# abiswas-odu/Disco

Hardware: AMD Instinct MI355X
Metric: overlaps/sec (BuildGraph stage), 150 bp reads (higher is better)
Workload: dtype u64; 1 GPU; 50000000 x 150 bp synthetic reads, 30x of 50 x 5000000 bp uniform-random contigs, both strands, error-free, min-overlap 40 (k=39), transitive reduction on, seed 42; reads=50000000, read_len=150, min_overlap=40, parallelism=1 GPU, e_pre=903537181, e_out=45314794, n_contained=4685156, cap_bind_sites=0, asymmetric_pairs=0, probes=5550000000, kmer_hits=2220071992

## Files before the change

### disco_amd/buildgraph.py

```python
from __future__ import annotations

import ctypes as C
import os

import numpy as np

_HERE = os.path.dirname(os.path.abspath(__file__))
_LIBPATH = os.environ.get("DISCO_LIB") or os.path.join(_HERE, "libdisco_hip.so")
_lib = None


class DiscoError(RuntimeError):
    pass


class Params(C.Structure):
    _fields_ = [("min_overlap", C.c_uint32), ("max_edges_per_kmer", C.c_uint32), ("flags", C.c_uint32), ("max_substitutions", C.c_uint32)]


class GenSpecABI(C.Structure):
    _fields_ = [("seed", C.c_uint64), ("n_reads", C.c_uint64), ("contig_len", C.c_uint64), ("n_contigs", C.c_uint32),
                ("len_min", C.c_uint32), ("len_max", C.c_uint32), ("skew", C.c_uint32)]


# ... 78 lines not shown
    ("disco_ingest_fasta", C.c_int, [_P, C.POINTER(C.c_char_p), C.c_int, C.c_uint32, _P, _P]),
    ("disco_ingest_fetch", C.c_int, [_P, _P, _P]),
    ("disco_inflate_bgzf", C.c_int64, [_P, _P, C.c_uint64, _P, C.c_uint64]),
    ("disco_dist_ingest_fasta", C.c_int, [_P, C.POINTER(C.c_char_p), C.c_int, C.c_uint32, _P, _P]),
    ("disco_dist_ingest_fetch", C.c_int, [_P, _P, _P]),
    ("disco_inflate_bgzf_window", C.c_int64, [_P, _P, C.c_uint64, C.c_uint64, C.c_uint64, _P]),
    ("disco_format_contained", C.c_int64, [_P, C.c_uint32, _P, _P]),
    ("disco_fetch_contained_text", C.c_int, [_P, _P, C.c_uint64]),
    ("disco_write_contained_text", C.c_int, [_P, _P, C.c_uint32, C.c_uint32]),
    ("disco_dist_format_contained", C.c_int64, [_P, C.c_uint32, _P, _P]),
    ("disco_dist_format_edges", C.c_int64, [_P, C.c_uint32, _P, _P]),
    ("disco_fetch_chain_residue", C.c_int64, [_P, _P, _P, C.c_uint64]),
    ("disco_fetch_chain_first_edges", C.c_int, [_P, _P]),
    ("disco_fetch_chain_end_links", C.c_int, [_P, _P, _P]),
    ("disco_format_par_simple", C.c_int64, [_P, C.c_uint32, _P, _P, C.c_uint64, _P, C.c_uint64, _P]),
    ("disco_fetch_par_simple_text", C.c_int, [_P, _P, C.c_uint64]),
    ("disco_write_par_simple_text", C.c_int, [_P, _P, C.c_uint32, C.c_uint32]),
    ("disco_prepare_edge_records", C.c_int64, [_P, C.c_uint32, _P, _P]),
    ("disco_fetch_edge_records", C.c_int, [_P, _P, C.c_uint64]),
    ("disco_write_edge_records", C.c_int, [_P, C.c_int, C.c_uint64, C.c_uint32]),
    ("disco_prepare_contained_records", C.c_int64, [_P, C.c_uint32, _P]),
    ("disco_fetch_contained_records", C.c_int, [_P, _P, C.c_uint64]),
    ("disco_write_contained_records", C.c_int, [_P, C.c_int, C.c_uint64, C.c_uint32]),
]

ABI_VERSION = 2
FLAG_TWO_PASS_VERIFY = 1
FLAG_SEEDED_KMER = 2
XCHG = ("reads", "index_records", "index_shards", "contain", "row_requests", "row_data", "push", "adjacency", "twins", "queries", "hits", "keys", "reads_dealt", "contain_keys")
UNIQUE_ID_BYTES = 128
DIST_GATHER_READS = 1
DIST_KEEP_INDEX_PARTITIONED = 2


CHAIN_EDGE_DTYPE = np.dtype([("a", "<u8"), ("b", "<u8"), ("offset", "<u8"), ("orient", "<u4"), ("n_links", "<u4"), ("first_link", "<u8")])
CHAIN_LINK_DTYPE = np.dtype([("to", "<u4"), ("offset", "<u4"), ("orient", "<u4")])


class PsEdge(C.Structure):
    _fields_ = [("src", C.c_uint64), ("dst", C.c_uint64), ("offset", C.c_uint64), ("orient", C.c_uint32), ("file", C.c_uint32),
                ("first_piece", C.c_uint64), ("n_pieces", C.c_uint32), ("pad", C.c_uint32)]


class PsPiece(C.Structure):
    _fields_ = [("kind", C.c_uint32), ("a", C.c_uint32), ("offset", C.c_uint32), ("orient", C.c_uint32)]


PS_EDGE_DTYPE = np.dtype([("src", "<u8"), ("dst", "<u8"), ("offset", "<u8"), ("orient", "<u4"), ("file", "<u4"), ("first_piece", "<u8"), ("n_pieces", "<u4"), ("pad", "<u4")])
PS_PIECE_DTYPE = np.dtype([("kind", "<u4"), ("a", "<u4"), ("offset", "<u4"), ("orient", "<u4")])
assert PS_EDGE_DTYPE.itemsize == C.sizeof(PsEdge) and PS_PIECE_DTYPE.itemsize == C.sizeof(PsPiece)


class IngestFile(C.Structure):
    _fields_ = [("first_index", C.c_uint64), ("last_index", C.c_uint64), ("good", C.c_uint64), ("bad", C.c_uint64)]


class IngestInfo(C.Structure):
    _fields_ = [("n_reads", C.c_uint64), ("total_records", C.c_uint64), ("too_long", C.c_uint64), ("stride_words", C.c_uint32), ("shortest", C.c_uint32),
                ("longest", C.c_uint32), ("read_s", C.c_float), ("device_s", C.c_float)]


class DistIngestInfo(C.Structure):
    _fields_ = [("n_reads", C.c_uint64), ("total_records", C.c_uint64), ("too_long", C.c_uint64), ("stride_words", C.c_uint32), ("shortest", C.c_uint32),
                ("longest", C.c_uint32), ("world", C.c_uint32), ("share_lo", C.c_uint64), ("share_hi", C.c_uint64), ("share_reads", C.c_uint64),
                ("kept_reads", C.c_uint64), ("home_lo", C.c_uint64), ("home_hi", C.c_uint64), ("read_s", C.c_float), ("device_s", C.c_float)]


class DistInfo(C.Structure):
    _fields_ = [("world", C.c_uint32), ("rank", C.c_uint32), ("n_reads", C.c_uint64), ("own_lo", C.c_uint64), ("own_hi", C.c_uint64),
                ("n_contained", C.c_uint64), ("e_pre", C.c_uint64), ("e_out", C.c_uint64), ("e_out_local", C.c_uint64),
                ("n_contained_local", C.c_uint64), ("cap_bind_sites", C.c_uint64), ("asymmetric_pairs", C.c_uint64),
                ("dropped_hits", C.c_uint64), ("probes", C.c_uint64), ("kmer_hits", C.c_uint64), ("regime", C.c_uint32),
                ("tr_rounds", C.c_uint32), ("tr_deferred", C.c_uint64), ("bytes_sent", C.c_uint64 * len(XCHG)),
                ("ms", C.c_float * len(XCHG)), ("ms_total", C.c_float), ("kernel_ms", C.c_float), ("comm_ops", C.c_uint32),
                ("host_syncs", C.c_uint32), ("device_allocs", C.c_uint32), ("device_frees", C.c_uint32), ("arena_bytes", C.c_uint64),
                ("arena_peak", C.c_uint64), ("hbm_peak", C.c_uint64), ("own_reads", C.c_uint64), ("placement", C.c_uint32), ("reserved_", C.c_uint32)]

PHASES = ("index", "probe_kernel", "verify", "contain", "select", "csr", "twin", "trmark", "emit", "order")

INSPECT_ABI = [
    ("disco_fetch_order", C.c_int, [_P, _P, _P, C.c_uint64, C.POINTER(C.c_uint64), C.POINTER(C.c_int)]),
    ("disco_fetch_survivor_layout", C.c_int, [_P, _P, C.c_uint64, C.POINTER(C.c_uint64), C.POINTER(C.c_int), C.POINTER(C.c_uint64)]),
    ("disco_set_record_piece", C.c_int, [_P, C.c_uint64]),
]
_inspect_bound = False


def _bind_inspect(L):
    global _inspect_bound
    if not _inspect_bound:
        for name, res, args in INSPECT_ABI:
            fn = getattr(L, name)
            fn.restype = res
            fn.argtypes = args
        _inspect_bound = True


def lib_path() -> str:
    return _LIBPATH


def load():
    global _lib
    if _lib is None:
        if not os.path.exists(_LIBPATH):
            raise DiscoError(f"{_LIBPATH} is missing: build it with `python -m disco_amd.build` (hipcc, gfx950). "
                             "There is no CPU fallback.")
        L = C.CDLL(_LIBPATH)
        L.disco_abi_version.restype = C.c_int
        if L.disco_abi_version() != ABI_VERSION:
            raise DiscoError(f"{_LIBPATH} speaks ABI version {L.disco_abi_version()}, this mirror was written against {ABI_VERSION}: rebuild "
                             "(`python -m disco_amd.build`)")
        for name, res, args in ABI:
            fn = getattr(L, name)
            fn.restype = res
            fn.argtypes = args
        _lib = L
    return _lib


class BuildGraph:

    def __init__(self, min_overlap: int = 40, device: int = 0, max_edges_per_kmer: int = 4, flags: int = 0, max_substitutions: int = 0):
        self.L = load()
        self.min_overlap = min_overlap
        self._h = _P()
        p = Params(min_overlap, max_edges_per_kmer, flags, max_substitutions)
        rc = self.L.disco_create(device, C.byref(p), C.byref(self._h))
        if rc != 0:
            raise DiscoError(f"disco_create failed ({rc}): {self.L.disco_last_error(None).decode()}")

    def _chk(self, rc):
        if rc < 0:
            raise DiscoError(f"libdisco_hip error {rc}: {self.L.disco_last_error(self._h).decode()}")
        return rc

    def close(self):
        if self._h:
            self.L.disco_destroy(self._h)
            self._h = _P()

    def __del__(self):
        try:
            self.close()
        except Exception:
            pass

    def __enter__(self):
        return self

    def __exit__(self, *a):
        self.close()

    def set_stream(self, stream_ptr: int | None):
        self._chk(self.L.disco_set_stream(self._h, _P(stream_ptr) if stream_ptr else None))

    def synchronize(self):
        self._chk(self.L.disco_synchronize(self._h))

    def upload_reads(self, packed: np.ndarray, lens: np.ndarray):
        packed = np.ascontiguousarray(packed, dtype=np.uint64)
        lens = np.ascontiguousarray(lens, dtype=np.uint16)
        assert packed.ndim == 2 and packed.shape[0] == lens.shape[0]
        self._keep = (packed, lens)
        self._chk(self.L.disco_upload_reads(self._h, packed.ctypes.data, packed.shape[1], lens.ctypes.data, packed.shape[0]))

# ... 238 lines not shown
        from .edgefile import EDGE

        out = np.zeros(n, dtype=EDGE)
        self._chk(self.L.disco_fetch_edge_records(self._h, out.ctypes.data if n else None, n))
        return out

    def write_edge_records(self, fd: int, file_offset: int = 32, threads: int = 8):
        self._chk(self.L.disco_write_edge_records(self._h, fd, file_offset, threads))

    def prepare_contained_records(self, n_files: int = 1, file_index=None) -> int:
        fi = None if file_index is None else np.ascontiguousarray(file_index, dtype=np.uint64)
        return self._chk(self.L.disco_prepare_contained_records(self._h, n_files, None if fi is None else fi.ctypes.data))

    def fetch_contained_records(self, n: int) -> np.ndarray:
        from .edgefile import CONTAINED

        out = np.zeros(n, dtype=CONTAINED)
        self._chk(self.L.disco_fetch_contained_records(self._h, out.ctypes.data if n else None, n))
        return out

    def write_contained_records(self, fd: int, file_offset: int = 32, threads: int = 8):
        self._chk(self.L.disco_write_contained_records(self._h, fd, file_offset, threads))

    def set_record_piece(self, records: int = 0):
        _bind_inspect(self.L)
        self._chk(self.L.disco_set_record_piece(self._h, records))

    def fetch_edge_substitutions(self) -> np.ndarray:
        n = self._chk(self.L.disco_fetch_edge_substitutions(self._h, None, 0))
        out = np.zeros(n, dtype=np.uint16)
        if n:
            self._chk(self.L.disco_fetch_edge_substitutions(self._h, out.ctypes.data, n))
        return out

    def phase_ms(self) -> dict:
        a = (C.c_float * len(PHASES))()
        self._chk(self.L.disco_phase_ms(self._h, a, len(PHASES)))
        return {n: float(a[i]) for i, n in enumerate(PHASES)}

    def fetch_edge_files(self, n_files: int):
        n = int(self.L.disco_fetch_edges(self._h, None, 0))
        out = np.zeros(max(n, 1), dtype=np.uint16)
        self._chk(self.L.disco_fetch_edge_files(self._h, n_files, out.ctypes.data, n))
        return out[:n]

    def partition_edges(self, edges: np.ndarray, n_nodes: int, n_files: int):
        edges = np.ascontiguousarray(edges, dtype=EDGE_DTYPE)
        out = np.zeros(max(len(edges), 1), dtype=np.uint16)
        self._chk(self.L.disco_partition_edges(self._h, edges.ctypes.data, len(edges), n_nodes, n_files, out.ctypes.data))
        return out[:len(edges)]

    def get_query_order(self) -> int:
        out = _P()
        self._chk(self.L.disco_get_query_order(self._h, C.byref(out)))
        return out.value or 0

    def set_query_order(self, d_order_ptr: int):
        self._chk(self.L.disco_set_query_order(self._h, _P(d_order_ptr)))

    def probe_run_words(self) -> int:
        return int(self.L.disco_probe_run_words(self._h))

    def fetch_order(self):
        _bind_inspect(self.L)
        n, bits = C.c_uint64(0), C.c_int(0)
        one = np.zeros(1, dtype=np.uint64)
        rc = self.L.disco_fetch_order(self._h, one.ctypes.data, one.ctypes.data, 0, C.byref(n), C.byref(bits))
        if n.value == 0:
            self._chk(rc)
        order, keys = np.zeros(max(n.value, 1), dtype=np.uint64), np.zeros(max(n.value, 1), dtype=np.uint32)
        self._chk(self.L.disco_fetch_order(self._h, order.ctypes.data, keys.ctypes.data, len(order), C.byref(n), C.byref(bits)))
        return order[:n.value], keys[:n.value], bits.value

    def fetch_survivor_layout(self, lengths: bool = True):
        _bind_inspect(self.L)
        n, dense, used = C.c_uint64(0), C.c_int(0), C.c_uint64(0)
        self._chk(self.L.disco_fetch_survivor_layout(self._h, None, 0, C.byref(n), C.byref(dense), C.byref(used)))
        lens = None
        if lengths:
            lens = np.zeros(max(n.value, 1), dtype=np.uint8)
            self._chk(self.L.disco_fetch_survivor_layout(self._h, lens.ctypes.data, len(lens), C.byref(n), C.byref(dense), C.byref(used)))
            lens = lens[:n.value]
        return lens, bool(dense.value), used.value

    def measure_hbm(self, nbytes: int = 4 << 30, reps: int = 5) -> float:
        out = C.c_double(0.0)
        self._chk(self.L.disco_measure_hbm(self._h, nbytes, reps, C.byref(out)))
        return out.value

    def measure_gather(self, nbytes: int = 3 << 30, reps: int = 3) -> float:
        out = C.c_double(0.0)
        self._chk(self.L.disco_measure_gather(self._h, nbytes, reps, C.byref(out)))
        return out.value

    def memcpy_d2d(self, dst_ptr: int, src_ptr: int, nbytes: int):
        self._chk(self.L.disco_memcpy_d2d(self._h, _P(dst_ptr), _P(src_ptr), nbytes))

    @staticmethod
    def comm_unique_id() -> bytes:
        buf = C.create_string_buffer(UNIQUE_ID_BYTES)
        rc = load().disco_comm_unique_id(buf, UNIQUE_ID_BYTES)
        if rc != 0:
            raise DiscoError(f"disco_comm_unique_id failed ({rc})")
        return buf.raw

    def comm_init(self, unique_id: bytes, world: int, rank: int):
        self._chk(self.L.disco_comm_init(self._h, C.c_char_p(unique_id), world, rank))

    @staticmethod
    def comm_init_local(graphs):
        arr = (_P * len(graphs))(*[g._h for g in graphs])
        rc = load().disco_comm_init_local(arr, len(graphs))
        if rc != 0:
            raise DiscoError(f"disco_comm_init_local failed ({rc})")

    @property
    def rank(self) -> int:
        return int(self.L.disco_comm_rank(self._h))

    @property
    def world(self) -> int:
        return int(self.L.disco_comm_world(self._h))

    @property
    def transport(self) -> str:
        return self.L.disco_comm_kind(self._h).decode()

    def dist_range(self, n_total: int):
        lo, hi = C.c_uint64(), C.c_uint64()
        self._chk(self.L.disco_dist_range(self._h, n_total, C.byref(lo), C.byref(hi)))
        return lo.value, hi.value

    def dist_upload_reads(self, packed_own: np.ndarray, lens_own: np.ndarray, n_total: int, stride_words: int | None = None):
        packed_own = np.ascontiguousarray(packed_own, dtype=np.uint64)
        lens_own = np.ascontiguousarray(lens_own, dtype=np.uint16)
        self._keep = (packed_own, lens_own)
        stride = int(stride_words if stride_words is not None else packed_own.shape[1])
        self._chk(self.L.disco_dist_upload_reads(self._h, packed_own.ctypes.data, stride, lens_own.ctypes.data, n_total))

    def dist_upload_ascii(self, reads):
        n = len(reads)
        lo, hi = self.dist_range(n)
        stride = int((max((len(r) for r in reads), default=1) + 31) // 32)
        packed = np.zeros((hi - lo, stride), dtype=np.uint64)
        lens = np.fromiter((len(r) for r in reads[lo:hi]), dtype=np.uint16, count=hi - lo)
        for i, r in enumerate(reads[lo:hi]):
            b = r.encode()
            if self.L.disco_pack_ascii(b, len(b), packed[i].ctypes.data) != 0:
                raise DiscoError(f"read {lo + i} contains a non-ACGT base")
        self.dist_upload_reads(packed, lens, n, stride)

    def dist_generate_reads(self, spec):
        s = GenSpecABI(spec.seed, spec.n_reads, spec.contig_len, spec.n_contigs, spec.len_min, spec.len_max, int(spec.skew_word if hasattr(spec, "skew_word") else getattr(spec, "skew", 0)))
        self._chk(self.L.disco_dist_generate_reads(self._h, C.byref(s)))

    def ingest_fasta(self, paths, threads: int = 16):
        arr = (C.c_char_p * len(paths))(*[os.fsencode(p) for p in paths])
        info, files = IngestInfo(), (IngestFile * len(paths))()
        rc = self.L.disco_ingest_fasta(self._h, arr, len(paths), threads, C.byref(info), files)
        if rc == -6:
            return None
        self._chk(rc)
        return ({n: getattr(info, n) for n, _ in IngestInfo._fields_}, [{n: getattr(f, n) for n, _ in IngestFile._fields_} for f in files])

    def inflate_bgzf(self, data: bytes):
        data = bytes(data)
# ... 110 lines not shown
```

### disco_amd/csrc/disco_hip.hip

```cpp
#include <hip/hip_runtime.h>
#include <rocprofiler-sdk-roctx/roctx.h>

#include <algorithm>
#include <atomic>
#include <chrono>
#include <cstdarg>
#include <cstdio>
#include <cstdlib>
#include <cstring>
#include <functional>
#include <fcntl.h>
#include <sys/mman.h>
#include <sys/stat.h>
#include <unistd.h>
#include <string>
#include <memory>
#include <thread>
#include <map>
#include <mutex>
#include <queue>
#include <vector>

#include "../../include/disco_hip.h"
#include "../../include/disco_hip_test.h"
// ... 79 lines not shown
                used += bytes;
                peak = std::max(peak, used);
                return base + off;
            }
        return nullptr;
    }
    void release(void *p)
    {
        const size_t off = (size_t)((char *)p - base);
        auto lv = live.find(off);
        if (lv == live.end()) return;
        size_t start = off, end = off + lv->second;
        used -= lv->second;
        live.erase(lv);
        auto nx = free_at.lower_bound(off);
        if (nx != free_at.end() && nx->first == end) {
            end += nx->second;
            nx = free_at.erase(nx);
        }
        if (nx != free_at.begin()) {
            auto pv = std::prev(nx);
            if (pv->first + pv->second == start) {
                start = pv->first;
                free_at.erase(pv);
            }
        }
        free_at[start] = end - start;
    }
    std::map<size_t, size_t> live;
};

template <typename T>
struct DevBuf {
    T *p = nullptr;
    u64 cap = 0;
    operator T *() const { return p; }
};

struct disco_ctx {
    int device = 0;
    disco_params prm{};
    DevArena arena;
    int k = 0;
    int ks = 0;
    hipStream_t own_stream = nullptr;
    hipStream_t stream = nullptr;
    int n_cu = 256;
    std::string err;
    size_t hbm_bytes = 0, hbm_peak = 0;

    u64 n = 0;
    int S = 0;
    u64 *d_reads = nullptr;
    u16 *d_len = nullptr;
    DevBuf<u64> reads_own;
    DevBuf<u16> len_own;
    bool reads_owned = false;
    std::vector<uint16_t> h_len;
    bool h_len_ok = false;
    std::mutex h_len_mu;
    u64 q_lo = 0, q_hi = 0;
    bool two_class = false;
    bool dist_two_class = false;
    u64 job_n_long = 0;
    u32 job_short_max = 0;
    int S_ext = 0;
    u64 n_long = 0;
    DevBuf<u64> d_full;
    DevBuf<u32> d_ovf, d_long_ids;
    u32 max_len_all = 0;
    int tailb = 0;
    DevBuf<u32> d_lpos, d_n_list;
    DevBuf<uint2> d_linfo;
    DevBuf<ulonglong2> d_lmeta;

    u64 T = 0;
    int bshift = 0;
    DevBuf<u32> d_bkt;
    DevBuf<u64> d_ent;
    DevBuf<ulonglong2> d_rec;
    bool binned_index = false;
    DevBuf<ulonglong2> d_rec2;
    DevBuf<u32> d_binx;

    DevBuf<u64> d_tile;
    u64 *d_total = nullptr;

    u64 *d_ctr = nullptr;
    u64 *d_wq = nullptr;
    u64 h_ctr[CTR_COUNT] = {0};

    DevBuf<u64> d_best;
    DevBuf<u64> d_hits;
    u64 hits_used = 0;
    u64 *d_bump = nullptr;
    DevBuf<u64> d_row_start;
    DevBuf<u32> d_row_cnt;
    DevBuf<u64> d_big_list;
    DevBuf<u32> d_big_cnt;
    u32 *d_n_big = nullptr;
    DevBuf<u32> d_runs;
    u64 runs_lo = 0, runs_n = 0;
    int runs_lpr = 0;
    DevBuf<u64> d_slow_list;
    u32 *d_n_slow = nullptr;
    u64 big_rows = 0, slow_rows = 0;
    const u64 *d_order = nullptr;
    const u64 *d_order_used = nullptr;
    bool order_external = false;
    DevBuf<u32> d_ocnt, d_okey, d_oslot;
    DevBuf<u64> d_order_own;
    bool order_counted = false;
    bool order_items = false;
    int order_id_bits = 0;
    bool es_big_counted = false, tr_big_counted = false;
    bool contained_count_pending = false;
    bool order_ready = false;
    hipStream_t aux_stream = nullptr;
    hipEvent_t ev_crows = nullptr;
    DevBuf<u32> d_cpos, d_crow_id;
    DevBuf<u64> d_crow_key;
    DevBuf<u64> d_tile2;
    u64 *d_total2 = nullptr;
    void *h_crows = nullptr;
    DevBuf<u32> d_crow_len;
    u64 crows_hcap = 0, crows_n = 0;
    bool crows_pending = false;
    bool crows_in_ring = false;
    DevBuf<u32> d_cgrp_cur, d_cgrp_id;
    DevBuf<u64> d_cgrp_key, d_cgrp_big;
    u64 h_cgrp_big = 0;
    bool cgrp_pending = false;
    DevBuf<u32> d_fetch_src;
    DevBuf<u64> d_fetch_ent;
    DevBuf<u32> d_rec_of_read;
    std::vector<u64> ingest_id_base, ingest_rec_base;
    u64 ingest_n = 0;
    void *h_ring = nullptr;
    std::vector<u64> text_off;
    DevBuf<char> d_ctext;
    std::vector<u64> ctext_off;
    u64 ctext_bytes = 0;
    DevBuf<u8> d_ingest;
    std::thread hits_prealloc;
    DevBuf<u64> prealloc;
    u64 prealloc_asked = 0;
    size_t ring_half = 0;
    hipEvent_t ev_ring[2] = {nullptr, nullptr};
    hipStream_t copy_stream = nullptr;
    hipEvent_t ev_copied[3] = {nullptr, nullptr, nullptr}, ev_unpacked[3] = {nullptr, nullptr, nullptr};
    bool index_counted = false;
    u64 order_counted_lo = 0, order_counted_hi = 0;
    int order_counted_bits = 0;
    DevBuf<u32> d_asked;
    u64 order_q_lo = 0, order_q_hi = 0;
    DevBuf<ulonglong2> d_meta_ord;
    u64 dropped_local = 0;
    ProbeRare h_probe_rare;
    DevBuf<ProbeRare> d_probe_rare;
    u32 max_len = 0, min_len = 0;
    bool two_pass_last = false;
    bool contained_done = false;

    DevBuf<u8> d_contained;
    DevBuf<u64> d_cbits;
    DevBuf<u64> d_dropbits;
    DevBuf<u64> d_drop_node, d_drop_key;
    u64 n_drop_items = 0;
    u64 drop_lo = 0, drop_hi = 0;
    u64 n_contained = 0;

    DevBuf<u64> d_adj_ref;
// ... 267 lines not shown
    v.long_ids = c->two_class ? c->d_long_ids : nullptr;
    v.n_long = c->two_class ? (u32)c->n_long : 0u;
    v.SL = c->two_class ? c->S_ext : 0;
    v.tailb = c->two_class ? c->tailb : 0;
    return v;
}

static OwnSet own_set(const disco_ctx *c)
{
    OwnSet o;
    o.otab = c->loci ? c->d_otab : nullptr;
    o.me = c->comm ? (u32)c->comm->rank : 0u;
    o.lo = c->q_lo;
    o.hi = c->q_hi;
    o.list = c->loci ? c->d_order_own : nullptr;
    o.n_own = c->loci ? c->n_own : 0;
    o.ids = c->loci ? c->d_own_ids : nullptr;
    return o;
}

static int settle_keys(disco_ctx *c)
{
    if (c->keys_pending) {
        c->keys_pending = false;
        HIPCHK(c, hipStreamWaitEvent(c->stream, c->ev_keys, 0));
    }
    return DISCO_OK;
}

static int env_int(const char *name, int dflt)
{
    const char *e = getenv(name);
    return e ? atoi(e) : dflt;
}

static int wave_grid(const disco_ctx *c, u64 items, int per_cu = 24)
{
    u64 g = (u64)c->n_cu * per_cu;
    if (items < g) g = items;
    return (int)std::max<u64>(g, 1);
}

template <typename K>
static int wq_grid(disco_ctx *c, K kernel, u64 items, const char *env, int cap = 32)
{
    (void)hipMemsetAsync(c->d_wq, 0, sizeof(u64) * WQ_WORDS, c->stream);
    int per_cu = 0;
    if (hipOccupancyMaxActiveBlocksPerMultiprocessor(&per_cu, kernel, 64, 0) != hipSuccess || per_cu <= 0) per_cu = 16;
    if (per_cu > cap) per_cu = cap;
    per_cu = env_int(env, per_cu);
    u64 g = (u64)c->n_cu * per_cu;
    const u64 chunks = (items + WQ_CHUNK - 1) / WQ_CHUNK;
    if (chunks < g) g = chunks;
    return (int)std::max<u64>(g, 1);
}

template <typename K, typename... A>
static void wq_launch(disco_ctx *c, K kernel, u64 items, const char *env, int cap, A... args)
{
    const int g = wq_grid(c, kernel, items, env, cap);
    hipLaunchKernelGGL(kernel, dim3(g), dim3(64), 0, c->stream, args...);
}

static int flat_grid(const disco_ctx *c, u64 items, int block = 256)
{
    u64 g = (items + block - 1) / block;
    u64 cap = (u64)c->n_cu * 16;
    return (int)std::max<u64>(std::min(g, cap), 1);
}

static int read_counters(disco_ctx *c)
{
    HIPCHK(c, hipMemcpyAsync(c->h_ctr, c->d_ctr, sizeof(c->h_ctr), hipMemcpyDeviceToHost, c->stream));
    HIPCHK(c, hipStreamSynchronize(c->stream));
    return DISCO_OK;
}

static int zero_counter(disco_ctx *c, int idx)
{
    HIPCHK(c, hipMemsetAsync(c->d_ctr + idx, 0, sizeof(u64), c->stream));
    return DISCO_OK;
}

template <typename InT, typename OutT>
static int scan_exclusive_on(disco_ctx *c, hipStream_t st, DevBuf<u64> &tile, u64 *total, const InT *in, u64 n, OutT *out, bool write_total, u64 *total_host)
{
    u64 nt = (n + SCAN_TILE - 1) / SCAN_TILE;
    if (nt == 0) nt = 1;
    CHK(ensure(c, tile, nt));
    hipLaunchKernelGGL((scan_tile_sums_kernel<InT>), dim3((unsigned)nt), dim3(SCAN_BLOCK), 0, st, in, n, tile.p);
    hipLaunchKernelGGL(scan_sums_kernel, dim3(1), dim3(1024), 0, st, tile.p, nt, total);
    hipLaunchKernelGGL((scan_apply_kernel<InT, OutT>), dim3((unsigned)nt), dim3(SCAN_BLOCK), 0, st, in, n, tile.p, out);
    if (write_total) hipLaunchKernelGGL((scan_write_total_kernel<OutT>), dim3(1), dim3(1), 0, st, total, out + n);
    HIPCHK(c, hipGetLastError());
    if (total_host) {
        HIPCHK(c, hipMemcpyAsync(total_host, total, sizeof(u64), hipMemcpyDeviceToHost, st));
        HIPCHK(c, hipStreamSynchronize(st));
    }
    return DISCO_OK;
}

template <typename InT, typename OutT>
static int scan_exclusive(disco_ctx *c, const InT *in, u64 n, OutT *out, bool write_total, u64 *total_host)
{
    return scan_exclusive_on<InT, OutT>(c, c->stream, c->d_tile, c->d_total, in, n, out, write_total, total_host);
}

static void drop_edge_records(disco_ctx *c)
{
    c->rec_e_ready = false;
    release(c, c->d_rec_efile);
    release(c, c->d_rec_subs);
    release(c, c->d_rec_efindex);
}
static void drop_contained_records(disco_ctx *c)
{
    c->rec_c_ready = false;
    c->rec_c_n = 0;
    release(c, c->d_rec_cword);
    release(c, c->d_rec_csup);
    release(c, c->d_rec_cfindex);
}

static void free_graph_state(disco_ctx *c)
{
    drop_edge_records(c);
    drop_contained_records(c);
    release(c, c->d_rec_piece[0]);
    release(c, c->d_rec_piece[1]);
    if (c->keys_pending) {
        c->keys_pending = false;
        if (c->ev_keys) (void)hipEventSynchronize(c->ev_keys);
    }
    release(c, c->d_bkt);
    release(c, c->d_ent);
    release(c, c->d_rec);
    release(c, c->d_rec2);
    release(c, c->d_binx);
    release(c, c->d_best);
    release(c, c->d_hits);
    release(c, c->d_row_start);
    release(c, c->d_row_cnt);
    release(c, c->d_big_list);
    release(c, c->d_big_cnt);
    release(c, c->d_slow_list);
    release(c, c->d_runs);
    c->runs_n = 0;
    c->runs_lpr = 0;
    release(c, c->d_contained);
    release(c, c->d_cbits);
    release(c, c->d_dropbits);
    release(c, c->d_drop_node);
    release(c, c->d_drop_key);
    release(c, c->d_adj_ref);
    release(c, c->d_adj_own);
    release(c, c->d_adj_spare);
    release(c, c->d_start_tmp);
    release(c, c->d_ocnt);
    release(c, c->d_okey);
    release(c, c->d_meta_ord);
    release(c, c->d_asked);
    release(c, c->d_oslot);
    release(c, c->d_order_own);
    c->d_order_used = nullptr;
    c->d_adj = nullptr;
    release(c, c->d_extra_cnt);
    release(c, c->d_extra_node);
    release(c, c->d_extra_key);
    release(c, c->d_half);
    release(c, c->d_hcnt);
    release(c, c->d_wide);
    release(c, c->d_n_wide);
    c->adj_total = 0;
    release(c, c->d_out_valid);
    release(c, c->d_ch_comp);
    release(c, c->d_ch_links);
    release(c, c->d_ch_dead);
    release(c, c->d_ch_first);
    release(c, c->d_ch_res_pos);
    release(c, c->d_ch_res_slot);
    c->ch_res_n = 0;
    release(c, c->d_ptext);
    c->ptext_bytes = 0;
    c->ptext_off.clear();
    release(c, c->d_text);
    c->text_bytes = 0;
    release(c, c->d_ctext);
    c->ctext_bytes = 0;
    c->ctext_off.clear();
    c->ch_ready = false;
    release(c, c->d_out_pos);
    release(c, c->d_out_src);
    release(c, c->d_out_ent);
    c->n_out = c->out_used = 0;
    c->flags_pending = false;
    c->adj_imported = false;
    c->T = 0;
    release(c, c->d_x16a);
    release(c, c->d_x16b);
    release(c, c->d_req_flat);
    release(c, c->d_req_s);
    release(c, c->d_req_r);
    release(c, c->d_rdeg_s);
    release(c, c->d_rdeg_r);
    release(c, c->d_rdata_s);
    release(c, c->d_rpos);
    release(c, c->d_nadj32_own);
    release(c, c->d_deg_tmp);
    release(c, c->d_dense);
    release(c, c->d_pq_start);
    c->nadj_used = 0;
    c->d_push_r = nullptr;
    c->n_push_r = 0;
    release(c, c->d_cb_all);
    release(c, c->d_otab);
    release(c, c->d_own_ids);
    c->n_own = 0;
    c->loci = c->runs_by_pos = false;
}

static void free_long_class(disco_ctx *c)
{
    release(c, c->d_full);
    release(c, c->d_ovf);
    release(c, c->d_long_ids);
    release(c, c->d_lpos);
    release(c, c->d_lmeta);
    release(c, c->d_linfo);
    release(c, c->d_n_list);
    c->two_class = false;
    c->n_long = 0;
    c->S_ext = 0;
    c->tailb = 0;
}

static void free_reads(disco_ctx *c)
{
    release(c, c->reads_own);
    release(c, c->len_own);
    free_long_class(c);
    c->d_reads = nullptr;
    c->d_len = nullptr;
    c->reads_owned = false;
    c->h_len.clear();
    c->n = 0;
}

static int alloc_reads(disco_ctx *c, u64 words, u64 n_len)
{
    CHK(ensure(c, c->reads_own, words));
    c->d_reads = c->reads_own;
    CHK(ensure(c, c->len_own, n_len));
    c->d_len = c->len_own;
    return DISCO_OK;
}

static u32 extra_cap(const disco_ctx *c) { return (u32)std::min<u64>(std::min(c->d_extra_node.cap, c->d_extra_key.cap), 0xFFFFFFFFull); }

static int grow_big_lists(disco_ctx *c, u64 need) { return ensure_group(c, need, need, c->d_big_list, c->d_big_cnt); }

static bool own_order_wanted(const disco_ctx *c, u64 nq, int *bits)
{
    const u64 order_min = getenv("DISCO_ORDER_MIN_READS") ? (u64)atoll(getenv("DISCO_ORDER_MIN_READS")) : 4096;
    int b = 16;
    while (b < 27 && (1ull << b) < nq) ++b;
    if (const char *e = getenv("DISCO_ORDER_BITS")) b = std::min(std::max(atoi(e), 16), 26);
    *bits = b;
    return !c->order_external && !getenv("DISCO_NO_ORDER") && nq >= order_min && nq > 0;
}

struct IndexCountPlan {
    u64 lo = 0, hi = 0;
    int lpr = 0, nf = 0;
    u32 *ocnt = nullptr, *oslot = nullptr;
    u64 *oitem = nullptr;
    u32 oidbits = 0;
    u32 oshift = 0;
    const u64 *list = nullptr;
};

static bool runs_nf_built(int nf, int m) { return (nf == 7 || nf == 12 || nf == 17 || nf == 22 || nf == 27) && m == RUNS_M; }

static int runs_lpr_for(const disco_ctx *c, int nf, u32 max_len, u64 nloc)
{
    int lpr = 0;
    const int m = view(c).m;
    const bool nf_built = runs_nf_built(nf, m);
    const bool nf_generic = nf >= 2 && nf <= 64 && m > 16 && m <= 31 && !getenv("DISCO_NO_GENERIC_RUNS");
    if ((nf_built || nf_generic) && max_len > (u32)c->ks && !getenv("DISCO_NO_RUNS")) {
        const u32 maxwin = max_len - (u32)c->ks;
        const u32 expect = 2u * maxwin / (u32)(nf + 1);
        lpr = maxwin <= 256 ? (maxwin <= 128 && expect <= 20 ? 16 : (expect <= 44 ? 32 : 0)) : 0;
        const double max_gb = getenv("DISCO_RUNS_MAX_GB") ? atof(getenv("DISCO_RUNS_MAX_GB")) : 16.0;
        if ((double)nloc * lpr * 4.0 > max_gb * 1e9) lpr = 0;
    }
    return lpr;
}

static bool two_class_ok(const disco_ctx *c, int S, u64 n, u64 n_long, u32 short_max, bool will_own = false)
{
    if (((c->comm || c->dist_reads) && !c->dist_two_class) || !(c->reads_owned || will_own) || c->prm.max_substitutions || getenv("DISCO_NO_TWO_CLASS")) return false;
    if (S <= VERIFY_SW || n_long == 0 || n_long * (u64)env_int("DISCO_TWO_CLASS_ONE_IN", 5) > n || n + n_long >= (1ull << 31)) return false;
    return runs_lpr_for(c, c->ks - view(c).m + 1, short_max, n) != 0;
}

static int two_class_alloc(disco_ctx *c, u64 n_long, int Sx, u32 short_max)
{
    c->n_long = n_long;
    c->S_ext = Sx;
    int rc = ensure(c, c->d_ovf, c->n_alloc);
    if (rc == DISCO_OK) rc = ensure(c, c->d_full, n_long * (u64)Sx);
    if (rc == DISCO_OK) rc = ensure(c, c->d_long_ids, n_long);
    if (rc == DISCO_OK) rc = ensure(c, c->d_lpos, n_long);
    if (rc == DISCO_OK) rc = ensure(c, c->d_lmeta, n_long);
    if (rc == DISCO_OK) rc = ensure(c, c->d_linfo, n_long);
    if (rc == DISCO_OK) rc = ensure(c, c->d_n_list, 1);
    if (rc != DISCO_OK) {
        free_long_class(c);
        return rc;
    }
    c->S = VERIFY_SW;
    c->tailb = short_max <= 160 ? 160 : 256;
    c->two_class = true;
    if (getenv("DISCO_VERBOSE"))
        fprintf(stderr, "[disco] two classes of rows: %llu of %llu reads are longer than 256 bases, the others up to %u: 64-byte rows + %d-word rows for those\n",
                (unsigned long long)n_long, (unsigned long long)c->n, short_max, Sx);
    return DISCO_OK;
}

static bool binned_order_wanted(disco_ctx *c, u64 n, int obits, int *id_bits)
{
    if (getenv("DISCO_NO_BINNED_ORDER") || getenv("DISCO_NO_ORDERED_FILL") || c->two_class || n != c->n || n >= 0xFFFF0000ull) return false;
    const u64 binned_min = getenv("DISCO_BINNED_ORDER_MIN_READS") ? (u64)atoll(getenv("DISCO_BINNED_ORDER_MIN_READS")) : (1ull << 21);
    if (n < binned_min) return false;
    int idb = 1, lenb = 1;
    while ((1ull << idb) < n) ++idb;
    while ((1u << lenb) <= c->max_len) ++lenb;
    if (obits + lenb + idb > 64) return false;
    if (ensure(c, c->d_rec2, n) != DISCO_OK) {
        (void)hipGetLastError();
        c->err.clear();
        return false;
    }
    *id_bits = idb;
    return true;
}

static int index_count_plan(disco_ctx *c, const DiscoView &v, u64 lo, u64 hi, IndexCountPlan *pl, const u64 *list = nullptr)
{
    const u64 nloc = hi - lo;
    *pl = IndexCountPlan();
    pl->lo = lo;
    pl->hi = hi;
    pl->list = list;
    if (!list) c->order_counted = c->order_ready = c->order_items = false;
    int obits = 0;
    if (!list && lo == c->q_lo && hi == c->q_hi && own_order_wanted(c, nloc, &obits) && !getenv("DISCO_NO_ORDER_FUSE")) {
        const u64 order_buckets = 1ull << obits;
        if (lo == 0 && binned_order_wanted(c, nloc, obits, &c->order_id_bits)) {
            pl->oitem = (u64 *)c->d_rec2.p;
            pl->oidbits = (u32)c->order_id_bits;
            c->order_items = true;
        } else {
            CHK(ensure(c, c->d_ocnt, order_buckets + 1));
            CHK(ensure(c, c->d_oslot, nloc));
            HIPCHK(c, hipMemsetAsync(c->d_ocnt, 0, (order_buckets + 1) * sizeof(u32), c->stream));
            pl->ocnt = c->d_ocnt;
            pl->oslot = c->d_oslot;
        }
        pl->oshift = 32u - (u32)obits;
        c->order_counted = true;
        c->order_counted_lo = lo;
        c->order_counted_hi = hi;
        c->order_counted_bits = obits;
    }
    c->runs_lpr = 0;
    c->runs_n = 0;
    c->runs_by_pos = false;
    const int nf = v.ks - v.m + 1;
    const int lpr = c->S == VERIFY_SW ? runs_lpr_for(c, nf, c->max_len, nloc) : 0;
    if (lpr && nloc) {
        CHK(ensure(c, c->d_runs, nloc * (u64)lpr));
        c->runs_lpr = lpr;
        c->runs_lo = lo;
        c->runs_n = nloc;
        c->runs_by_pos = list != nullptr;
        pl->lpr = lpr;
        pl->nf = nf;
    }
    return DISCO_OK;
}

typedef void (*IndexRunsFn)(DiscoView, u32 *, ulonglong2 *, u32 *, u64, u64, u32 *, u32 *, u32 *, u64 *, u32, u32, const u64 *);
typedef void (*IndexCountFn)(DiscoView, u32 *, ulonglong2 *, u32 *, u64, u64, u32 *, u32 *, u64 *, u32, u32, const u64 *);
struct IndexCountKernel {
    IndexRunsFn runs = nullptr;
    IndexCountFn plain = nullptr;
};
template <bool COUNT, int NF, int NFMAX, bool LONGK>
static IndexCountKernel index_runs_pick(int lpr)
{
    IndexCountKernel k;
    k.runs = lpr == 16 ? index_runs_kernel<COUNT, NF, 1, NFMAX, LONGK> : index_runs_kernel<COUNT, NF, 2, NFMAX, LONGK>;
    return k;
}
template <bool COUNT>
static IndexCountKernel index_count_pick(int nf, int m, int lpr, bool longk, bool long_class)
{
    if (long_class || !lpr) {
        IndexCountKernel k;
        if (long_class) k.plain = longk ? index_count_kernel<COUNT, true, true> : index_count_kernel<COUNT, false, true>;
        else k.plain = longk ? index_count_kernel<COUNT, true> : index_count_kernel<COUNT>;
        return k;
    }
    if (runs_nf_built(nf, m)) switch (nf) {
        case 7: return index_runs_pick<COUNT, 7, 7, false>(lpr);
        case 12: return index_runs_pick<COUNT, 12, 12, false>(lpr);
        case 17: return index_runs_pick<COUNT, 17, 17, false>(lpr);
        case 22: return index_runs_pick<COUNT, 22, 22, false>(lpr);
        default: return index_runs_pick<COUNT, 27, 27, false>(lpr);
        }
    if (longk) return nf <= 48 ? index_runs_pick<COUNT, 0, 48, true>(lpr) : index_runs_pick<COUNT, 0, 64, true>(lpr);
    if (nf <= 8) return index_runs_pick<COUNT, 0, 8, false>(lpr);
    if (nf <= 12) return index_runs_pick<COUNT, 0, 12, false>(lpr);
    if (nf <= 16) return index_runs_pick<COUNT, 0, 16, false>(lpr);
    if (nf <= 24) return index_runs_pick<COUNT, 0, 24, false>(lpr);
    if (nf <= 32) return index_runs_pick<COUNT, 0, 32, false>(lpr);
    if (nf <= 48) return index_runs_pick<COUNT, 0, 48, false>(lpr);
    return index_runs_pick<COUNT, 0, 64, false>(lpr);
}
static IndexCountKernel index_count_pick(bool count, int nf, int m, int lpr, bool longk, bool long_class)
{
    return count ? index_count_pick<true>(nf, m, lpr, longk, long_class) : index_count_pick<false>(nf, m, lpr, longk, long_class);
}

static int index_count_chunk(disco_ctx *c, const DiscoView &v, const IndexCountPlan &pl, bool count, ulonglong2 *rec_base, u64 a, u64 b)
{
    if (b <= a) return DISCO_OK;
    const dim3 grid((unsigned)((b - a + 255) / 256));
    ulonglong2 *rec = rec_base + 2 * (a - pl.lo);
    u32 *oslot = pl.oslot ? pl.oslot + (a - pl.lo) : nullptr;
    u64 *oitem = pl.oitem ? pl.oitem + (a - pl.lo) : nullptr;
    u32 *okey = pl.list ? nullptr : c->d_okey.p;
    const IndexCountKernel k = index_count_pick(count, pl.nf, v.m, pl.lpr, c->ks > 64, false);
    if (k.runs) hipLaunchKernelGGL(k.runs, grid, dim3(256), 0, c->stream, v, c->d_bkt, rec, okey, a, b, c->d_runs + (a - pl.lo) * (u64)pl.lpr, pl.ocnt, oslot, oitem, pl.oidbits, pl.oshift, pl.list);
    else hipLaunchKernelGGL(k.plain, grid, dim3(256), 0, c->stream, v, c->d_bkt, rec, okey, a, b, pl.ocnt, oslot, oitem, pl.oidbits, pl.oshift, pl.list);
    HIPCHK(c, hipGetLastError());
    return DISCO_OK;
}

static int index_count_long(disco_ctx *c, const DiscoView &v, const IndexCountPlan &pl, bool count, ulonglong2 *rec, u32 *oslot, u64 x_lo, u64 x_hi)
{
    const dim3 g((unsigned)((x_hi - x_lo + 255) / 256));
    hipLaunchKernelGGL(index_count_pick(count, 0, v.m, 0, c->ks > 64, true).plain, g, dim3(256), 0, c->stream, v, c->d_bkt, rec, c->d_okey, x_lo, x_hi, pl.ocnt, oslot, (u64 *)nullptr, 0u, pl.oshift,
                       (const u64 *)nullptr);
    HIPCHK(c, hipGetLastError());
    return DISCO_OK;
}

static bool binned_index_wanted(disco_ctx *c, int logT)
{
    if (getenv("DISCO_NO_BINNED_INDEX") || 2 * c->n >= 0xFFFF0000ull) return false;
    if (logT > BINX_SPAN_BITS && ensure(c, c->d_rec2, 2 * c->n) != DISCO_OK) {
        (void)hipGetLastError();
        c->err.clear();
        return false;
    }
    return true;
}

static int size_bucket_table(disco_ctx *c)
{
    u64 T = 1024;
    int logT = 10;
    double tscale = 2.0;
    if (const char *e = getenv("DISCO_BUCKET_SCALE")) tscale = atof(e);
    while ((double)T < tscale * (double)c->n && logT < 32) {
        T <<= 1;
        logT++;
    }
    c->T = T;
    c->bshift = 64 - logT;
    return logT;
}

static int index_begin(disco_ctx *c)
{
    const int logT = size_bucket_table(c);
    const u64 T = c->T;
    CHK(ensure(c, c->d_bkt, T + 1));
    CHK(ensure(c, c->d_ent, 2 * c->n));
    CHK(ensure(c, c->d_rec, 2 * c->n));
    CHK(ensure(c, c->d_okey, c->n));
    c->adj_imported = false;
    c->binned_index = binned_index_wanted(c, logT);
    if (!c->binned_index) HIPCHK(c, hipMemsetAsync(c->d_bkt, 0, (T + 1) * sizeof(u32), c->stream));
    return DISCO_OK;
}

struct BinxPlan {
    int span = 0, levels = 0, bits[3] = {0, 0, 0};
};
static BinxPlan binx_plan(int logT)
{
    BinxPlan b;
    b.span = std::min(logT, BINX_SPAN_BITS);
    const int prefix = logT - b.span;
    b.levels = (prefix + BINX_MAX_BITS - 1) / BINX_MAX_BITS;
    for (int l = 0; l < b.levels; l++) b.bits[l] = prefix / b.levels + (l < prefix % b.levels ? 1 : 0);
    return b;
}

template <typename R>
static int binx_partition(disco_ctx *c, const char *what, int bits, u32 kshift, u32 total, R *src, R *dst, const R **out, const u32 **part)
{
    const BinxPlan bp = binx_plan(bits);
    const u32 n_part = 1u << (bits - bp.span);
    const u32 tiles = (total + BINX_TILE - 1u) / BINX_TILE;
    u64 hist_len = 1;
    for (int l = 0, done = 0; l < bp.levels; done += bp.bits[l], l++) hist_len = std::max<u64>(hist_len, ((u64)tiles + (1ull << done)) * (1ull << bp.bits[l]) + 1);
    const u64 tab = ((u64)n_part + 1 + 63) & ~63ull;
    CHK(ensure(c, c->d_binx, 4 * tab + hist_len));
    u32 *seg[2] = {c->d_binx.p, c->d_binx.p + tab}, *tb[2] = {c->d_binx.p + 2 * tab, c->d_binx.p + 3 * tab}, *hist = c->d_binx.p + 4 * tab;
    if (getenv("DISCO_VERBOSE"))
        fprintf(stderr, "[disco] binned %s: 2^%d buckets, %u partitions of 2^%d, %d level(s) of %d / %d / %d bits\n", what, bits, n_part, bp.span, bp.levels, bp.bits[0], bp.bits[1], bp.bits[2]);
    u32 pseg = 1, pnb = 1;
    int cur = 0, done = 0;
    for (int l = 0; l < bp.levels; l++) {
        const u32 nseg = 1u << done, nb = 1u << bp.bits[l], shift = kshift + (u32)(bits - done - bp.bits[l]);
        const u32 grid = tiles + nseg;
        const u64 hlen = (u64)grid * nb + 1;
        hipLaunchKernelGGL(binx_segs_kernel, dim3(1), dim3(1024), 0, c->stream, l ? (const u32 *)hist : (const u32 *)nullptr, (const u32 *)tb[cur ^ 1], pseg, pnb, total, seg[cur], tb[cur]);
        HIPCHK(c, hipMemsetAsync(hist, 0, hlen * sizeof(u32), c->stream));
        hipLaunchKernelGGL(binx_hist_kernel<R>, dim3(grid), dim3(BINX_BLOCK), 0, c->stream, (const R *)src, (const u32 *)seg[cur], (const u32 *)tb[cur], nseg, shift, nb, hist);
        CHK((scan_exclusive<u32, u32>(c, hist, hlen, hist, false, nullptr)));
        hipLaunchKernelGGL(binx_scatter_kernel<R>, dim3(grid), dim3(BINX_BLOCK), 0, c->stream, (const R *)src, dst, (const u32 *)seg[cur], (const u32 *)tb[cur], nseg, shift, nb, (const u32 *)hist);
        HIPCHK(c, hipGetLastError());
        std::swap(src, dst);
        pseg = nseg;
        pnb = nb;
        done += bp.bits[l];
        cur ^= 1;
    }
    hipLaunchKernelGGL(binx_segs_kernel, dim3(1), dim3(1024), 0, c->stream, bp.levels ? (const u32 *)hist : (const u32 *)nullptr, (const u32 *)tb[cur ^ 1], pseg, pnb, total, seg[cur],
                       (u32 *)nullptr);
    HIPCHK(c, hipGetLastError());
    *out = src;
    *part = seg[cur];
    return DISCO_OK;
}

static int binned_build_index(disco_ctx *c)
{
    const int logT = 64 - c->bshift;
    const u32 total = (u32)(2 * c->n);
    const ulonglong2 *rec;
    const u32 *part;
    CHK(binx_partition(c, "index build", logT, 32u, total, c->d_rec.p, c->d_rec2.p, &rec, &part));
    const int span = std::min(logT, BINX_SPAN_BITS);
    hipLaunchKernelGGL(binx_build_kernel<ulonglong2>, dim3(1u << (logT - span)), dim3(BINX_BUILD_BLOCK), 0, c->stream, rec, part, (u32)span, 32u, 0u, total, c->T, c->d_bkt.p, c->d_ent.p);
    HIPCHK(c, hipGetLastError());
    return DISCO_OK;
}

static int binned_build_order(disco_ctx *c)
{
    const int bits = c->order_counted_bits;
    const u32 total = (u32)c->n, kshift = 64u - (u32)bits;
    u64 *items = (u64 *)c->d_rec2.p;
    const u64 *rec;
    const u32 *part;
    CHK(binx_partition(c, "grouping", bits, kshift, total, items, items + c->n, &rec, &part));
    const int span = std::min(bits, BINX_SPAN_BITS);
    hipLaunchKernelGGL(binx_build_kernel<u64>, dim3(1u << (bits - span)), dim3(BINX_BUILD_BLOCK), 0, c->stream, rec, part, (u32)span, kshift, (u32)c->order_id_bits, total, (u64)0,
                       (u32 *)nullptr, c->d_order_own.p);
    HIPCHK(c, hipGetLastError());
    return DISCO_OK;
}

static int start_contained_rows(disco_ctx *c, bool grouped)
{
    const u64 nc = c->n_contained;
    if (c->crows_pending && c->crows_n == nc && (!grouped || c->cgrp_pending)) return DISCO_OK;
    const bool have_rows = c->crows_pending && c->crows_n == nc;
    if (!have_rows) c->crows_pending = c->cgrp_pending = false;
    const u64 max_rows = getenv("DISCO_EAGER_ROWS_MAX") ? (u64)atoll(getenv("DISCO_EAGER_ROWS_MAX")) : (16ull << 20);
    if (c->comm || nc == 0 || nc > max_rows || c->n >= (1ull << 31)) return DISCO_OK;
    if (!c->aux_stream) {
        HIPCHK(c, hipStreamCreateWithFlags(&c->aux_stream, hipStreamNonBlocking));
        HIPCHK(c, hipEventCreateWithFlags(&c->ev_crows, hipEventDisableTiming));
        HIPCHK(c, hipMalloc((void **)&c->d_total2, sizeof(u64)));
    }
    CHK(ensure(c, c->d_cpos, c->n + 1));
    CHK(ensure_group(c, nc, nc + nc / 4 + 1024, c->d_crow_id, c->d_crow_key, c->d_crow_len));
    if (nc > c->crows_hcap && c->h_ring && !c->crows_in_ring && (u64)c->ring_half * 2 >= (nc + 1024) * 32) {
        if (c->h_crows) (void)hipHostFree(c->h_crows);
        c->h_crows = c->h_ring;
        c->crows_hcap = (u64)c->ring_half * 2 / 32;
        c->crows_in_ring = true;
    }
    if (nc > c->crows_hcap) {
        if (c->h_crows && !c->crows_in_ring) (void)hipHostFree(c->h_crows);
        c->crows_in_ring = false;
        c->h_crows = nullptr;
        c->crows_hcap = 0;
        const u64 want = nc + nc / 4 + 1024;
        if (hipHostMalloc(&c->h_crows, want * 32) != hipSuccess) {
            c->h_crows = nullptr;
            (void)hipGetLastError();
            return DISCO_OK;
        }
        c->crows_hcap = want;
    }
    if (!have_rows) {
    CHK((scan_exclusive_on<u8, u32>(c, c->aux_stream, c->d_tile2, c->d_total2, c->d_contained, c->n, c->d_cpos, false, nullptr)));
    hipLaunchKernelGGL(contain_rows32_kernel, dim3(flat_grid(c, c->n)), dim3(256), 0, c->aux_stream, c->d_best, c->d_contained, c->d_cpos, c->n, c->d_crow_id, c->d_crow_key);
    HIPCHK(c, hipGetLastError());
    u64 *hkey = (u64 *)c->h_crows;
    u32 *hid = (u32 *)(hkey + c->crows_hcap), *hln = hid + c->crows_hcap;
    hipLaunchKernelGGL(crow_lens_kernel, dim3(flat_grid(c, nc)), dim3(256), 0, c->aux_stream, (const u32 *)c->d_crow_id, (const u64 *)c->d_crow_key, nc, (const u16 *)c->d_len, c->d_crow_len);
    HIPCHK(c, hipGetLastError());
    HIPCHK(c, hipMemcpyAsync(hkey, c->d_crow_key, nc * 8, hipMemcpyDeviceToHost, c->aux_stream));
    HIPCHK(c, hipMemcpyAsync(hid, c->d_crow_id, nc * 4, hipMemcpyDeviceToHost, c->aux_stream));
    HIPCHK(c, hipMemcpyAsync(hln, c->d_crow_len, nc * 4, hipMemcpyDeviceToHost, c->aux_stream));
    HIPCHK(c, hipEventRecord(c->ev_crows, c->aux_stream));
    c->crows_n = nc;
    c->crows_pending = true;
    }
    if (grouped && !c->cgrp_pending) {
        CHK(ensure(c, c->d_cgrp_cur, c->n + 1));
        CHK(ensure_group(c, nc, nc + nc / 4 + 1024, c->d_cgrp_id, c->d_cgrp_key));
        CHK(ensure(c, c->d_cgrp_big, 1));
        HIPCHK(c, hipMemsetAsync(c->d_cpos, 0, (c->n + 1) * sizeof(u32), c->aux_stream));
        HIPCHK(c, hipMemsetAsync(c->d_cgrp_big, 0, sizeof(u64), c->aux_stream));
        hipLaunchKernelGGL(crow_count_kernel, dim3(flat_grid(c, nc)), dim3(256), 0, c->aux_stream, (const u64 *)c->d_crow_key, nc, c->d_cpos);
        CHK((scan_exclusive_on<u32, u32>(c, c->aux_stream, c->d_tile2, c->d_total2, c->d_cpos, c->n + 1, c->d_cgrp_cur, false, nullptr)));
        hipLaunchKernelGGL(crow_place_kernel, dim3(flat_grid(c, nc)), dim3(256), 0, c->aux_stream, (const u32 *)c->d_crow_id, (const u64 *)c->d_crow_key, nc, c->d_cgrp_cur, c->d_cgrp_id,
                           c->d_cgrp_key);
        hipLaunchKernelGGL(crow_sort_groups_kernel, dim3(flat_grid(c, nc)), dim3(256), 0, c->aux_stream, c->d_cgrp_id, c->d_cgrp_key, nc, c->d_cgrp_big);
        HIPCHK(c, hipGetLastError());
        u64 *gkey = (u64 *)((char *)c->h_crows + c->crows_hcap * 16);
        u32 *gid = (u32 *)(gkey + c->crows_hcap), *gln = gid + c->crows_hcap;
        hipLaunchKernelGGL(crow_lens_kernel, dim3(flat_grid(c, nc)), dim3(256), 0, c->aux_stream, (const u32 *)c->d_cgrp_id, (const u64 *)c->d_cgrp_key, nc, (const u16 *)c->d_len, c->d_crow_len);
        HIPCHK(c, hipMemcpyAsync(gkey, c->d_cgrp_key, nc * 8, hipMemcpyDeviceToHost, c->aux_stream));
        HIPCHK(c, hipMemcpyAsync(gid, c->d_cgrp_id, nc * 4, hipMemcpyDeviceToHost, c->aux_stream));
        HIPCHK(c, hipMemcpyAsync(gln, c->d_crow_len, nc * 4, hipMemcpyDeviceToHost, c->aux_stream));
        HIPCHK(c, hipMemcpyAsync(&c->h_cgrp_big, c->d_cgrp_big, sizeof(u64), hipMemcpyDeviceToHost, c->aux_stream));
        c->cgrp_pending = true;
    }
    return DISCO_OK;
}

static int settle_contained_rows(disco_ctx *c)
{
    if (c->crows_pending) HIPCHK(c, hipStreamSynchronize(c->aux_stream));
// ... 1483 lines not shown
    HIPCHK(c, hipGetLastError());
    HIPCHK(c, hipStreamSynchronize(c->stream));
    release(c, c->reads_own);
    c->reads_own = rows8;
    c->d_reads = c->reads_own;
    set_read_lengths(c, c->max_len, short_max, c->min_len);
    return DISCO_OK;
}

int disco_build_index(disco_ctx *c)
{
    DISCO_TRACE("disco_build_index");
    if (!c) return DISCO_E_ARG;
    if (c->phase < 1) return fail(c, DISCO_E_STATE, "disco_build_index: no reads");
    HIPCHK(c, hipSetDevice(c->device));
    ph_begin(c, DISCO_PH_INDEX);
    if (c->index_counted) {
        c->index_counted = false;
    } else {
        CHK(two_class_convert(c));
        CHK(index_begin(c));
        const DiscoView v = view(c);
        IndexCountPlan pl;
        CHK(index_count_plan(c, v, 0, c->n, &pl));
        CHK(index_count_chunk(c, v, pl, !c->binned_index, c->d_rec, 0, c->n));
        if (c->two_class) CHK(index_count_long(c, v, pl, !c->binned_index, c->d_rec, pl.oslot, 0, c->n_long));
    }
    const bool binned = c->binned_index;
    if (!binned) CHK((scan_exclusive<u32, u32>(c, c->d_bkt, c->T + 1, c->d_bkt, false, nullptr)));
    c->order_ready = false;
    if (c->order_counted && c->order_counted_lo == 0 && c->order_counted_hi == c->n && !c->two_class && !getenv("DISCO_NO_ORDERED_FILL")) {
        const u64 order_buckets = 1ull << c->order_counted_bits;
        CHK(ensure(c, c->d_order_own, c->n));
        ph_end(c, DISCO_PH_INDEX);
        ph_begin(c, DISCO_PH_ORDER);
        if (c->order_items) CHK(binned_build_order(c));
        else {
            CHK((scan_exclusive<u32, u32>(c, c->d_ocnt, order_buckets + 1, c->d_ocnt, false, nullptr)));
            hipLaunchKernelGGL(order_scatter_kernel, dim3(flat_grid(c, c->n)), dim3(256), 0, c->stream, c->d_okey, c->d_oslot, c->d_ocnt, 32u - (u32)c->order_counted_bits, (u64)0, c->n, c->d_len, c->d_order_own);
        }
        ph_end(c, DISCO_PH_ORDER);
        ph_begin(c, DISCO_PH_INDEX2);
        if (binned) CHK(binned_build_index(c));
        else hipLaunchKernelGGL(index_fill_ordered_kernel, dim3(flat_grid(c, c->n)), dim3(256), 0, c->stream, c->n, (const u64 *)c->d_order_own, (const ulonglong2 *)c->d_rec, (const u32 *)c->d_bkt, c->d_ent);
        ph_end(c, DISCO_PH_INDEX2);
        HIPCHK(c, hipGetLastError());
        c->order_ready = true;
        c->phase = 2;
        return DISCO_OK;
    }
    if (binned) CHK(binned_build_index(c));
    else if (c->n) hipLaunchKernelGGL(index_fill_kernel, dim3(flat_grid(c, 2 * c->n)), dim3(256), 0, c->stream, 2 * c->n, c->d_rec, c->d_bkt, c->d_ent);
    HIPCHK(c, hipGetLastError());
    ph_end(c, DISCO_PH_INDEX);
    c->phase = 2;
    return DISCO_OK;
}

int disco_probe(disco_ctx *c)
{
    DISCO_TRACE("disco_probe");
    if (!c) return DISCO_E_ARG;
    if (c->phase < 2) return fail(c, DISCO_E_STATE, "disco_probe: build the index first");
    HIPCHK(c, hipSetDevice(c->device));
    CHK(settle_contained_rows(c));
    CHK(settle_keys(c));
    drop_edge_records(c);
    drop_contained_records(c);
    settle_hits_prealloc(c);
    const u64 nq = c->q_hi - c->q_lo;
    CHK(ensure(c, c->d_best, c->n_alloc));
    CHK(ensure(c, c->d_row_start, c->n));
    CHK(ensure(c, c->d_row_cnt, c->n));
    if (c->n_alloc) hipLaunchKernelGGL(fill_u64_kernel, dim3(flat_grid(c, c->n_alloc)), dim3(256), 0, c->stream, c->d_best, c->n_alloc, DISCO_NOKEY);
    HIPCHK(c, hipMemsetAsync(c->d_row_cnt, 0, std::max<u64>(c->n, 1) * sizeof(u32), c->stream));
    const bool use_runs = c->runs_lpr != 0 && c->d_runs && c->q_lo >= c->runs_lo && c->q_hi <= c->runs_lo + c->runs_n;
    const ProbeKernel range_kernel = probe_pick(c, 0, use_runs);
    const int grid = range_kernel.runs ? wq_grid(c, range_kernel.runs, nq, "DISCO_PROBE_WAVES") : wq_grid(c, range_kernel.plain, nq, "DISCO_PROBE_WAVES");
    auto launch_probe = [&](const ProbeArgs &a, const ProbeKernel &k, int g) {
        if (k.runs) hipLaunchKernelGGL(k.runs, dim3(g), dim3(64), 0, c->stream, a, (const u32 *)c->d_runs, c->runs_by_pos ? ~0ull : c->runs_lo);
        else hipLaunchKernelGGL(k.plain, dim3(g), dim3(64), 0, c->stream, a);
    };
    const u64 chunk_slots = use_runs ? PR_CHUNK : PROBE_CHUNK;
    u64 want_hits = nq * 64 + (u64)grid * chunk_slots + (1u << 16);
    u32 want_slow = use_runs ? (u32)std::min<u64>(nq, nq / 64 + 1024 + (c->two_class ? c->n_long : 0)) : 1u;
    u32 want_big = (u32)std::min<u64>(nq, nq / 64 + 1024);
    for (int attempt = 0; attempt < 8; attempt++) {
        if (want_hits > c->d_hits.cap) {
            release(c, c->d_hits);
            size_t fr = 0, tot = 0;
            HIPCHK(c, hipMemGetInfo(&fr, &tot));
            if (want_hits * 8 > fr) {
                u64 can = fr / 8 / 10 * 9;
                if (can < (u64)grid * chunk_slots * 2) return fail(c, DISCO_E_NOMEM, "disco_probe: not enough HBM for the hit buffer (%llu entries wanted)", (unsigned long long)want_hits);
                want_hits = can;
            }
            CHK(ensure(c, c->d_hits, want_hits));
        }
        if (want_slow > c->d_slow_list.cap) CHK(ensure(c, c->d_slow_list, want_slow));
        CHK(grow_big_lists(c, want_big));
        HIPCHK(c, hipMemsetAsync(c->d_bump, 0, sizeof(u64), c->stream));
        HIPCHK(c, hipMemsetAsync(c->d_n_big, 0, sizeof(u32), c->stream));
        HIPCHK(c, hipMemsetAsync(c->d_n_slow, 0, sizeof(u32), c->stream));
        HIPCHK(c, hipMemsetAsync(c->d_ctr + CTR_KMER_HITS, 0, sizeof(u64) * 4, c->stream));
        CHK(zero_counter(c, CTR_MAX_ROW));
        CHK(zero_counter(c, CTR_ES_BIG));
        CHK(zero_counter(c, CTR_ES_MID));
        c->es_big_counted = c->tr_big_counted = false;
        ProbeArgs a;
        a.v = view(c);
        a.hits = c->d_hits;
        a.row_start = c->d_row_start;
        a.row_cnt = c->d_row_cnt;
        c->h_probe_rare.bump = c->d_bump;
        c->h_probe_rare.hits_cap = c->d_hits.cap;
        c->h_probe_rare.big_list = c->d_big_list;
        c->h_probe_rare.big_cnt = c->d_big_cnt;
        c->h_probe_rare.n_big = c->d_n_big;
        c->h_probe_rare.big_cap = c->d_big_list.cap;
        c->h_probe_rare.slow_cap = c->d_slow_list.cap;
        c->h_probe_rare.slow_list = c->d_slow_list;
        c->h_probe_rare.n_slow = c->d_n_slow;
        c->h_probe_rare.ctr = c->d_ctr;
        CHK(ensure(c, c->d_probe_rare, 1));
        HIPCHK(c, hipMemcpyAsync(c->d_probe_rare, &c->h_probe_rare, sizeof(ProbeRare), hipMemcpyHostToDevice, c->stream));
        a.rare = c->d_probe_rare;
        CHK(ensure(c, c->d_meta_ord, std::max<u64>(nq, 1)));
        a.meta_ord = c->d_meta_ord;
        int order_bits = 16;
        const bool own_order = own_order_wanted(c, nq, &order_bits);
        a.order = nullptr;
        const u64 order_buckets = 1ull << order_bits;
        const bool counted = c->order_counted && c->order_counted_lo == c->q_lo && c->order_counted_hi == c->q_hi && c->order_counted_bits == order_bits &&
                             (!c->order_items || c->order_ready);
        c->order_counted = false;
        if (c->loci) {
            c->d_order_used = c->d_order_own;
        } else if (own_order && c->order_ready && counted) {
            c->d_order_used = c->d_order_own;
        } else if (own_order) {
            CHK(ensure(c, c->d_ocnt, order_buckets + 1));
            CHK(ensure(c, c->d_oslot, nq));
            CHK(ensure(c, c->d_order_own, nq));
            const u32 oshift = 32u - (u32)order_bits;
            ph_begin(c, DISCO_PH_ORDER);
            if (!counted) {
                HIPCHK(c, hipMemsetAsync(c->d_ocnt, 0, (order_buckets + 1) * sizeof(u32), c->stream));
                hipLaunchKernelGGL(order_count_kernel, dim3(flat_grid(c, nq)), dim3(256), 0, c->stream, c->d_okey + c->q_lo, nq, oshift, c->d_ocnt, c->d_oslot);
            }
            CHK((scan_exclusive<u32, u32>(c, c->d_ocnt, order_buckets + 1, c->d_ocnt, false, nullptr)));
            hipLaunchKernelGGL(order_scatter_kernel, dim3(flat_grid(c, nq)), dim3(256), 0, c->stream, c->d_okey + c->q_lo, c->d_oslot, c->d_ocnt, oshift, c->q_lo, nq, c->d_len, c->d_order_own);
            ph_end(c, DISCO_PH_ORDER);
            HIPCHK(c, hipGetLastError());
            c->d_order_used = c->d_order_own;
        } else if (c->order_external && nq) {
            CHK(ensure(c, c->d_order_own, nq));
            hipLaunchKernelGGL(order_pack_kernel, dim3(flat_grid(c, nq)), dim3(256), 0, c->stream, c->d_order, nq, c->d_len, c->d_order_own);
            HIPCHK(c, hipGetLastError());
            c->d_order_used = c->d_order_own;
        } else
            c->d_order_used = nullptr;
        a.order = c->d_order_used;
        c->order_q_lo = c->q_lo;
        c->order_q_hi = c->q_hi;
        ph_begin(c, DISCO_PH_PROBE_KERNEL);
        HIPCHK(c, hipMemsetAsync(c->d_wq, 0, sizeof(u64) * WQ_WORDS, c->stream));
        const bool partitioned = c->dist_active && c->part_index;
        if (partitioned) CHK(dist_partitioned_probe(c));
        else if (nq) {
            launch_probe(a, range_kernel, grid);
        }
        ph_end(c, DISCO_PH_PROBE_KERNEL);
        HIPCHK(c, hipGetLastError());
        u32 n_big = 0, n_slow = 0;
        if (!partitioned) {
            HIPCHK(c, hipMemcpyAsync(&n_slow, c->d_n_slow, sizeof(u32), hipMemcpyDeviceToHost, c->stream));
            HIPCHK(c, hipMemcpyAsync(&n_big, c->d_n_big, sizeof(u32), hipMemcpyDeviceToHost, c->stream));
        }
        CHK(read_counters(c));
        if (partitioned) c->h_ctr[CTR_HITS_NEEDED] = c->hits_used;
        if (!c->h_ctr[CTR_OVERFLOW] && n_slow) {
            int g2 = wave_grid(c, (n_slow + WQ_CHUNK - 1) / WQ_CHUNK, 24);
            HIPCHK(c, hipMemsetAsync(c->d_wq, 0, sizeof(u64) * WQ_WORDS, c->stream));
            launch_probe(a, probe_pick(c, 2, false), g2);
            HIPCHK(c, hipGetLastError());
            HIPCHK(c, hipMemcpyAsync(&n_big, c->d_n_big, sizeof(u32), hipMemcpyDeviceToHost, c->stream));
            CHK(read_counters(c));
        }
        if (!partitioned) c->slow_rows = n_slow;
        if (!c->h_ctr[CTR_OVERFLOW] && n_big) {
            int g2 = wave_grid(c, (n_big + WQ_CHUNK - 1) / WQ_CHUNK, 8);
            HIPCHK(c, hipMemsetAsync(c->d_wq, 0, sizeof(u64) * WQ_WORDS, c->stream));
            launch_probe(a, probe_pick(c, 1, false), g2);
            HIPCHK(c, hipGetLastError());
            CHK(read_counters(c));
        }
        if (!c->h_ctr[CTR_OVERFLOW]) {
            c->big_rows = n_big;
            c->hits_used = c->h_ctr[CTR_HITS_NEEDED];
            VerifyArgs va;
            va.v = view(c);
            va.best = c->d_best;
            va.hits = c->d_hits;
            va.row_start = c->d_row_start;
            va.row_cnt = c->d_row_cnt;
            va.order = c->d_order_used;
            va.meta_ord = c->d_meta_ord;
            if (c->wait_bulk_before_verify) {
                HIPCHK(c, hipStreamWaitEvent(c->stream, c->ev_bulk, 0));
                c->wait_bulk_before_verify = false;
            }
            const bool inexact = c->prm.max_substitutions != 0;
            va.max_subs = c->prm.max_substitutions;
            const bool two_pass = !inexact && !c->two_class && (c->prm.flags & DISCO_FLAG_TWO_PASS_VERIFY) && c->S == VERIFY_SW && (nq || c->dist_active) &&
                                  (u64)c->min_len * 10 < (u64)c->max_len * 9 && !getenv("DISCO_NO_TWO_PASS");
            c->two_pass_last = two_pass;
            const bool flat = !inexact && c->S == VERIFY_SW && (c->two_class || !getenv("DISCO_NO_FLAT_VERIFY"));
            ph_begin(c, DISCO_PH_VERIFY);
            if (c->two_class && nq) {
                HIPCHK(c, hipMemsetAsync(c->d_n_list, 0, sizeof(u32), c->stream));
                hipLaunchKernelGGL(class_take_rows_kernel, dim3((unsigned)std::min<u64>((nq + TAKE_SPAN - 1) / TAKE_SPAN, (u64)c->n_cu * 8)), dim3(256), 0, c->stream, c->d_meta_ord,
                                   (const u64 *)c->d_order_used, c->q_lo, nq, (const u32 *)c->d_ovf, c->d_lpos, c->d_lmeta, c->d_linfo, c->d_n_list, (u32)c->n_long);
            }
            if (two_pass) {
                CHK(ensure(c, c->d_contained, c->n_alloc));
                CHK(ensure(c, c->d_cbits, c->n_alloc / 64 + 1));
                va.cbits = c->d_cbits;
                if (nq) verify_launch(c, va, nq, 1, flat, inexact);
                if (c->dist_active) {
                    CHK(dist_mark_contained(c));
                    c->contained_done = true;
                } else {
                    CHK(zero_counter(c, CTR_N_CONTAINED));
                    hipLaunchKernelGGL(contain_flags_kernel, dim3(flat_grid(c, c->n)), dim3(256), 0, c->stream, c->d_best, c->n, c->d_contained, c->d_cbits, c->d_ctr);
                }
                if (nq) verify_launch(c, va, nq, 2, flat, inexact);
            } else if (nq) {
                va.cbits = nullptr;
                verify_launch(c, va, nq, 0, flat, inexact);
            }
            if (c->two_class && nq)
                wq_launch(c, verify_long_kernel, c->n_long * 16, "DISCO_VL_WAVES", 32, va, (const u32 *)c->d_lpos, (const ulonglong2 *)c->d_lmeta, (const uint2 *)c->d_linfo, (const u32 *)c->d_n_list);
            ph_end(c, DISCO_PH_VERIFY);
            HIPCHK(c, hipGetLastError());
            CHK(read_counters(c));
            ph_collect(c);
            c->es_big_counted = true;
            c->phase = 3;
            return DISCO_OK;
        }
        if (getenv("DISCO_VERBOSE"))
            fprintf(stderr, "[disco] probe attempt %d overflowed: hits_cap=%llu needed=%llu n_big=%u big_cap=%u overflow=%llu\n", attempt,
                    (unsigned long long)c->d_hits.cap, (unsigned long long)c->h_ctr[CTR_HITS_NEEDED], n_big, (unsigned)c->d_big_list.cap, (unsigned long long)c->h_ctr[CTR_OVERFLOW]);
        if (n_big > c->d_big_list.cap) want_big = (u32)std::min<u64>(nq, (u64)n_big + n_big / 4 + 1024);
        if (n_slow > c->d_slow_list.cap) want_slow = (u32)std::min<u64>(nq, (u64)n_slow + n_slow / 4 + 1024);
        u64 needed = c->h_ctr[CTR_HITS_NEEDED];
        want_hits = std::max<u64>(c->d_hits.cap * 2, needed + needed / 4 + (u64)grid * chunk_slots);
    }
    return fail(c, DISCO_E_CAPACITY, "disco_probe: hit buffer could not be sized");
}


int disco_mark_contained(disco_ctx *c, uint64_t *n_contained)
{
    DISCO_TRACE("disco_mark_contained");
    if (!c) return DISCO_E_ARG;
    if (c->phase < 3) return fail(c, DISCO_E_STATE, "disco_mark_contained: run disco_probe first");
    HIPCHK(c, hipSetDevice(c->device));
    drop_contained_records(c);
    CHK(ensure(c, c->d_contained, c->n_alloc));
    CHK(ensure(c, c->d_cbits, c->n_alloc / 64 + 1));
    CHK(zero_counter(c, CTR_N_CONTAINED));
    ph_begin(c, DISCO_PH_CONTAIN);
    if (c->n) hipLaunchKernelGGL(contain_flags_kernel, dim3(flat_grid(c, c->n)), dim3(256), 0, c->stream, c->d_best, c->n, c->d_contained, c->d_cbits, c->d_ctr);
    HIPCHK(c, hipGetLastError());
    ph_end(c, DISCO_PH_CONTAIN);
    CHK(read_counters(c));
    ph_collect(c);
    c->n_contained = c->h_ctr[CTR_N_CONTAINED];
    if (n_contained) *n_contained = c->n_contained;
    c->phase = 4;
    c->crows_pending = c->cgrp_pending = false;
    return DISCO_OK;
}

static int ensure_big_cap(disco_ctx *c, const u32 *cnt, const u64 *ref, u32 thr)
{
    CHK(zero_counter(c, CTR_ES_BIG));
    const u64 ilo = c->loci ? 0 : c->q_lo, ihi = c->loci ? c->n : c->q_hi;
    if (ihi > ilo) hipLaunchKernelGGL(count_above_kernel, dim3(flat_grid(c, ihi - ilo)), dim3(256), 0, c->stream, cnt, ref, ilo, ihi, thr, c->d_ctr + CTR_ES_BIG);
    HIPCHK(c, hipGetLastError());
    CHK(read_counters(c));
    const u64 need = c->h_ctr[CTR_ES_BIG] + 1024;
    if (need > 0xFFFFFFFFull) return fail(c, DISCO_E_CAPACITY, "more than 2^32 big rows");
    return grow_big_lists(c, need);
}

static int select_edges(disco_ctx *c)
{
    DISCO_TRACE("select_edges");
    const u64 nq = c->q_hi - c->q_lo;
    CHK(ensure(c, c->d_adj_ref, c->n));
    HIPCHK(c, hipMemsetAsync(c->d_adj_ref, 0, std::max<u64>(c->n, 1) * sizeof(u64), c->stream));
    HIPCHK(c, hipMemsetAsync(c->d_n_big, 0, sizeof(u32), c->stream));
    CHK(zero_counter(c, CTR_CAP_SITES));
    CHK(zero_counter(c, CTR_DROPPED));
    CHK(zero_counter(c, CTR_ES_SLOW));
    CHK(zero_counter(c, CTR_ADJ_TOTAL));
    CHK(zero_counter(c, CTR_OVERFLOW));
    CHK(zero_counter(c, CTR_TR_BIG));
    CHK(zero_counter(c, CTR_TR_MID));
    const bool rows_counted = c->es_big_counted && !getenv("DISCO_COUNT_BIG_ROWS");
    const bool select_small = rows_counted && env_int("DISCO_SELECT_SMALL", c->h_ctr[CTR_ES_MID] * 100 <= nq ? 1 : 0) != 0;
    if (rows_counted) {
        const u64 need = c->h_ctr[select_small ? CTR_ES_MID : CTR_ES_BIG] + 1024;
        if (need > 0xFFFFFFFFull) return fail(c, DISCO_E_CAPACITY, "more than 2^32 big rows");
        CHK(grow_big_lists(c, need));
    } else
        CHK(ensure_big_cap(c, c->d_row_cnt, nullptr, ES_CAP));
    c->es_big_counted = false;
    EdgeSelArgs a;
    a.v = view(c);
    CHK(ensure(c, c->d_dropbits, c->n_alloc / 64 + 1));
    HIPCHK(c, hipMemsetAsync(c->d_dropbits, 0, (c->n_alloc / 64 + 1) * sizeof(u64), c->stream));
    c->drop_lo = c->loci ? 0 : c->q_lo;
    c->drop_hi = c->loci ? 0 : c->q_hi;
    a.dropbits = c->d_dropbits;
    a.hidden_flags = c->prm.max_substitutions != 0;
    a.drop_node = a.drop_key = nullptr;
    a.drop_cap = 0;
    CHK(zero_counter(c, CTR_DROP_ITEMS));
    if (c->prm.max_substitutions == 0 && !getenv("DISCO_NO_DROP_LIST")) {
        CHK(ensure(c, c->d_drop_node, DROP_LIST_CAP));
        CHK(ensure(c, c->d_drop_key, DROP_LIST_CAP));
        a.drop_node = c->d_drop_node;
        a.drop_key = c->d_drop_key;
        a.drop_cap = (u32)std::min<u64>(DROP_LIST_CAP, (u64)env_int("DISCO_DROP_LIST_CAP", (int)DROP_LIST_CAP));
    }
    a.contained = c->d_cbits;
    a.hits = c->d_hits;
    a.row_start = c->d_row_start;
    a.row_cnt = c->d_row_cnt;
    a.ref = c->d_adj_ref;
    a.max_per_kmer = c->prm.max_edges_per_kmer;
    a.big_list = c->d_big_list;
    a.n_big = c->d_n_big;
    a.big_cap = c->d_big_list.cap;
    a.scratch = nullptr;
    a.scratch_cap = 0;
    a.order = c->d_order_used;
    a.meta_ord = c->d_meta_ord;
    ph_begin(c, DISCO_PH_SELECT);
    const bool flat_select = c->S == VERIFY_SW && c->max_len <= 256 && !a.hidden_flags && a.max_per_kmer < 255u && !getenv("DISCO_NO_FLAT_SELECT");
    if (nq) wq_launch(c, edge_select_pick(false, flat_select, select_small), nq, "DISCO_SELECT_WAVES", 32, a);
    ph_end(c, DISCO_PH_SELECT);
    HIPCHK(c, hipGetLastError());
    u32 n_big = 0;
    HIPCHK(c, hipMemcpyAsync(&n_big, c->d_n_big, sizeof(u32), hipMemcpyDeviceToHost, c->stream));
    CHK(read_counters(c));
    ph_collect(c);
    if (c->h_ctr[CTR_OVERFLOW]) return fail(c, DISCO_E_CAPACITY, "edge selection: big-row list overflow (%u rows)", n_big);
    if (n_big) {
        if (select_small) {
            HIPCHK(c, hipMemsetAsync(c->d_wq, 0, sizeof(u64) * WQ_WORDS, c->stream));
            hipLaunchKernelGGL(edge_select_mid_kernel<ES_CAP>, dim3((int)std::min<u64>(n_big, (u64)c->n_cu * 32)), dim3(64), 0, c->stream, a, 0u);
        }
        if (!select_small || c->h_ctr[CTR_ES_BIG]) {
            HIPCHK(c, hipMemsetAsync(c->d_wq, 0, sizeof(u64) * WQ_WORDS, c->stream));
            hipLaunchKernelGGL(edge_select_mid_kernel<ES_MID>, dim3((int)std::min<u64>(n_big, (u64)c->n_cu * 8)), dim3(64), 0, c->stream, a, select_small ? (u32)ES_CAP : 0u);
        }
        HIPCHK(c, hipGetLastError());
        CHK(read_counters(c));
    }
    if (n_big && c->h_ctr[CTR_MAX_ROW] > ES_MID) {
        int g2 = (int)std::min<u64>(n_big, (u64)c->n_cu * 8);
        u64 cap = c->h_ctr[CTR_MAX_ROW] + 64;
        DevBuf<u64> scratch;
        CHK(ensure(c, scratch, (u64)g2 * 2 * cap));
        a.scratch = scratch;
        a.scratch_cap = cap;
        HIPCHK(c, hipMemsetAsync(c->d_wq, 0, sizeof(u64) * WQ_WORDS, c->stream));
        hipLaunchKernelGGL(edge_select_pick(true, false, false), dim3(g2), dim3(64), 0, c->stream, a);
        hipError_t e = hipGetLastError();
        int rc = read_counters(c);
        release(c, scratch);
        if (e != hipSuccess) return fail(c, DISCO_E_HIP, "edge_select_kernel (big rows): %s", hipGetErrorString(e));
        CHK(rc);
    }
    c->dropped = c->dropped_local = c->h_ctr[CTR_DROPPED];
    c->n_drop_items = a.drop_node ? c->h_ctr[CTR_DROP_ITEMS] : ~0ull;
    c->tr_big_counted = true;
    if (c->contained_count_pending) {
        c->n_contained = c->h_ctr[CTR_N_CONTAINED];
        c->contained_count_pending = false;
    }
    if (getenv("DISCO_VERBOSE"))
        fprintf(stderr, "[disco] edge selection%s: %llu rows in the sequential path, %u in the big-row list (%llu rows of more than 64 hits), dropped %llu\n",
                select_small ? " (five waves per SIMD)" : "", (unsigned long long)c->h_ctr[CTR_ES_SLOW], n_big, (unsigned long long)c->h_ctr[CTR_ES_MID], (unsigned long long)c->dropped);
    c->d_adj = c->d_hits;
    c->adj_total = c->h_ctr[CTR_ADJ_TOTAL];
    c->adj_imported = false;
    c->adj_span = 0;
    c->half_complete = true;
    c->ph_ms[DISCO_PH_CSR] = 0;
    c->phase = 5;
    return DISCO_OK;
}

static bool merge_is_sparse(const disco_ctx *c) { return c->d_adj == c->d_hits && c->n_extra <= 16384 && !getenv("DISCO_MERGE_REBUILD"); }

static int twin_check_search(disco_ctx *c, u64 lo, u64 hi);

static int twin_check(disco_ctx *c, u64 lo, u64 hi)
{
    CHK(twin_check_search(c, lo, hi));
    if (c->prm.max_substitutions != 0 && c->n && (c->n_extra == 0 || merge_is_sparse(c))) {
        hipLaunchKernelGGL(clear_adj_flags_kernel, dim3(flat_grid(c, c->n * 16)), dim3(256), 0, c->stream, c->d_adj_ref, c->d_adj, c->n);
        HIPCHK(c, hipGetLastError());
    }
    return DISCO_OK;
}

static int twin_check_search(disco_ctx *c, u64 lo, u64 hi)
{
    DISCO_TRACE("twin_check");
    CHK(ensure(c, c->d_extra_cnt, c->n));
    if (c->dropped == 0 && c->prm.max_substitutions == 0 && lo >= c->q_lo && hi <= c->q_hi && !getenv("DISCO_FORCE_TWIN_CHECK")) {
        c->n_extra = 0;
        c->asym_local = 0;
        c->ph_ms[DISCO_PH_TWIN] = 0;
        return DISCO_OK;
    }
    TwinArgs a;
    a.v = view(c);
    a.ref = c->d_adj_ref;
    a.adj = c->d_adj;
    a.lo = lo;
    a.hi = hi;
    a.otab = c->loci ? c->d_otab : nullptr;
    a.me = c->comm ? (u32)c->comm->rank : 0u;
    a.extra_cnt = c->d_extra_cnt;
    a.n_extra = c->d_n_extra;
    const bool by_list = c->prm.max_substitutions == 0 && c->d_drop_node && lo == 0 && hi == c->n && c->q_lo == 0 && c->q_hi == c->n && !c->adj_imported &&
                         c->n_drop_items == c->dropped && c->n_drop_items <= (u64)env_int("DISCO_DROP_LIST_CAP", (int)DROP_LIST_CAP) && !getenv("DISCO_FORCE_TWIN_CHECK");
    const bool by_bitmap = !by_list && c->d_dropbits && lo >= c->drop_lo && hi <= c->drop_hi && !getenv("DISCO_FORCE_TWIN_CHECK");
    a.dropbits = by_bitmap ? c->d_dropbits : nullptr;
    a.hidden_flags = by_bitmap && c->prm.max_substitutions != 0;
    if (!by_bitmap && !by_list && c->prm.max_substitutions == 0) {
        CHK(zero_counter(c, CTR_ASYM));
        CHK(zero_counter(c, CTR_TW_UP));
        CHK(zero_counter(c, CTR_TW_DOWN));
        a.extra_node = nullptr;
        a.extra_key = nullptr;
        a.extra_cap = 0;
// ... 150 lines not shown
    if (!c) return DISCO_E_ARG;
    CHK(disco_select_edges(c));
    CHK(disco_symmetrize(c, 1, nullptr));
    CHK(merge_extras(c));
    if (n_pre) *n_pre = c->adj_total / 2;
    return DISCO_OK;
}

int disco_adjacency_size(disco_ctx *c, uint64_t *n_entries)
{
    if (!c || !n_entries) return DISCO_E_ARG;
    if (c->phase < 5) return fail(c, DISCO_E_STATE, "disco_adjacency_size: select edges first");
    *n_entries = c->adj_total;
    return DISCO_OK;
}

int disco_export_adjacency(disco_ctx *c, void *d_deg_u32, void *d_entries_u64)
{
    if (!c || !d_deg_u32) return DISCO_E_ARG;
    if (c->phase < 5 || c->adj_imported) return fail(c, DISCO_E_STATE, "disco_export_adjacency: needs the locally selected edges");
    HIPCHK(c, hipSetDevice(c->device));
    const u64 nq = c->q_hi - c->q_lo;
    ph_begin(c, DISCO_PH_CSR);
    if (nq) hipLaunchKernelGGL(deg_from_ref_kernel, dim3(flat_grid(c, nq)), dim3(256), 0, c->stream, c->d_adj_ref, c->q_lo, c->q_hi, (u32 *)d_deg_u32);
    HIPCHK(c, hipGetLastError());
    if (nq && c->adj_total && d_entries_u64) {
        CHK(ensure(c, c->d_start_tmp, c->n + 1));
        u64 *start = c->d_start_tmp;
        u64 total = 0;
        int rc = scan_exclusive<u32, u64>(c, (const u32 *)d_deg_u32, nq, start, true, &total);
        if (rc == DISCO_OK && total != c->adj_total) rc = fail(c, DISCO_E_STATE, "disco_export_adjacency: degree sum %llu != %llu", (unsigned long long)total, (unsigned long long)c->adj_total);
        if (rc == DISCO_OK) hipLaunchKernelGGL(rows_gather_kernel, dim3(wave_grid(c, nq, 16)), dim3(64), 0, c->stream, c->d_adj, c->d_adj_ref, c->q_lo, c->q_hi, start, (u64 *)d_entries_u64,
                                              (c->phase == 5 && c->prm.max_substitutions != 0) ? 0ull : (u64)ADJ_FLAG);
        hipError_t e = hipStreamSynchronize(c->stream);
        CHK(rc);
        if (e != hipSuccess) return fail(c, DISCO_E_HIP, "disco_export_adjacency: %s", hipGetErrorString(e));
    }
    ph_end(c, DISCO_PH_CSR);
    HIPCHK(c, hipStreamSynchronize(c->stream));
    ph_collect(c);
    return DISCO_OK;
}





int disco_import_adjacency(disco_ctx *c, const void *d_deg_u32_all, const void *d_entries_u64_all, uint64_t n_entries_all)
{
    if (!c || !d_deg_u32_all) return DISCO_E_ARG;
    if (c->phase < 5) return fail(c, DISCO_E_STATE, "disco_import_adjacency: select edges first");
    HIPCHK(c, hipSetDevice(c->device));
    CHK(ensure(c, c->d_start_tmp, c->n + 1));
    u64 *start = c->d_start_tmp;
    u64 total = 0;
    CHK((scan_exclusive<u32, u64>(c, (const u32 *)d_deg_u32_all, c->n, start, true, &total)));
    if (total != n_entries_all)
        return fail(c, DISCO_E_ARG, "disco_import_adjacency: degrees sum to %llu but %llu entries were passed", (unsigned long long)total, (unsigned long long)n_entries_all);
    CHK(ensure(c, c->d_adj_own, total));
    c->d_adj = c->d_adj_own;
    c->adj_total = total;
    if (total) HIPCHK(c, hipMemcpyAsync(c->d_adj, d_entries_u64_all, total * 8, hipMemcpyDeviceToDevice, c->stream));
    if (c->n) hipLaunchKernelGGL(ref_from_start_kernel, dim3(flat_grid(c, c->n)), dim3(256), 0, c->stream, start, (const u32 *)d_deg_u32_all, c->n, c->d_adj_ref);
    HIPCHK(c, hipGetLastError());
    HIPCHK(c, hipStreamSynchronize(c->stream));
    c->adj_imported = true;
    c->tr_big_counted = false;
    c->adj_span = total;
    c->half_complete = false;
    c->phase = 5;
    return DISCO_OK;
}




int disco_transitive_mark(disco_ctx *c)
{
    DISCO_TRACE("disco_transitive_mark");
    if (!c) return DISCO_E_ARG;
    if (c->phase < 6) return fail(c, DISCO_E_STATE, "disco_transitive_mark: build edges first");
    HIPCHK(c, hipSetDevice(c->device));
    const u64 nq = c->q_hi - c->q_lo;
    HIPCHK(c, hipMemsetAsync(c->d_n_big, 0, sizeof(u32), c->stream));
    CHK(zero_counter(c, CTR_OVERFLOW));
    const bool counted_nodes = c->tr_big_counted && c->q_lo == 0 && c->q_hi == c->n && !getenv("DISCO_COUNT_BIG_ROWS");
    const bool tr_small = env_int("DISCO_TR_SMALL", counted_nodes && c->h_ctr[CTR_TR_MID] * 100 <= nq ? 1 : 0) != 0 && counted_nodes;
    if (counted_nodes) {
        const u64 need = c->h_ctr[tr_small ? CTR_TR_MID : CTR_TR_BIG] + 1024;
        if (need > 0xFFFFFFFFull) return fail(c, DISCO_E_CAPACITY, "more than 2^32 big nodes");
        CHK(grow_big_lists(c, need));
    } else
        CHK(ensure_big_cap(c, nullptr, c->d_adj_ref, TR_CAP));
    c->use_half = !getenv("DISCO_NO_HALF");
    const u32 all_flags = (c->adj_imported || !c->use_half || c->q_lo != 0 || c->q_hi != c->n) ? 1u : 0u;
    const bool lists = c->use_half && !all_flags;
    TrArgs a;
    CHK(tr_args_begin(c, &a, lists));
    a.order = (c->d_order_used && c->order_q_lo == c->q_lo && c->order_q_hi == c->q_hi && !c->adj_imported && !getenv("DISCO_TR_NO_ORDER")) ? c->d_order_used : nullptr;
    a.all_flags = all_flags;
    ph_begin(c, DISCO_PH_TRMARK);
    if (nq) wq_launch(c, tr_pick(false, false, tr_small, lists), nq, "DISCO_TR_WAVES", 32, a);
    ph_end(c, DISCO_PH_TRMARK);
    HIPCHK(c, hipGetLastError());
    u32 n_big = 0;
    HIPCHK(c, hipMemcpyAsync(&n_big, c->d_n_big, sizeof(u32), hipMemcpyDeviceToHost, c->stream));
    c->n_wide = 0;
    if (c->use_half) HIPCHK(c, hipMemcpyAsync(&c->n_wide, c->d_n_wide, sizeof(u32), hipMemcpyDeviceToHost, c->stream));
    CHK(read_counters(c));
    ph_collect(c);
    if (c->h_ctr[CTR_OVERFLOW]) return fail(c, DISCO_E_CAPACITY, "transitive marking: big-node list overflow (%u nodes)", n_big);
    if (n_big) {
        CHK(tr_big_nodes(c, &a, n_big, false, "big nodes"));
        if (c->h_ctr[CTR_OVERFLOW]) return fail(c, DISCO_E_CAPACITY, "transitive marking (big nodes): list overflow");
    }
    if (n_big && c->use_half) HIPCHK(c, hipMemcpy(&c->n_wide, c->d_n_wide, sizeof(u32), hipMemcpyDeviceToHost));
    c->flags_pending = false;
    c->phase = 7;
    return DISCO_OK;
}


int disco_emit_edges(disco_ctx *c, uint64_t *n_out)
{
    DISCO_TRACE("disco_emit_edges");
    if (!c) return DISCO_E_ARG;
    if (c->phase < 7) return fail(c, DISCO_E_STATE, "disco_emit_edges: run disco_transitive_mark first");
    HIPCHK(c, hipSetDevice(c->device));
    drop_edge_records(c);
    const u64 nq = c->q_hi - c->q_lo;
    ph_begin(c, DISCO_PH_EMIT);
    const int grid = wq_grid(c, emit_kernel<false>, nq, "DISCO_EMIT_WAVES");
    const u64 n_push = c->dist_active ? c->n_push_r : 0;
    const int grid_push = (int)std::max<u64>(std::min<u64>((n_push + 63) / 64, (u64)c->n_cu * 16), 1);
    const u64 nwaves = (u64)grid * 2 + (n_push ? (u64)grid_push : 0);
    u64 want = std::max<u64>(2 * nq, 1024) + n_push + nwaves * EMIT_CHUNK;
    for (int attempt = 0; attempt < 6; attempt++) {
        CHK(ensure_group(c, want, want, c->d_out_src, c->d_out_ent));
        HIPCHK(c, hipMemsetAsync(c->d_bump, 0, sizeof(u64), c->stream));
        const bool half_emit = c->use_half && c->half_complete;
        const bool dense = half_emit && c->half_selfdel && !c->dist_active;
        if (half_emit && c->half_selfdel && !dense) return fail(c, DISCO_E_STATE, "disco_emit_edges: self-delimiting lists under a communicator");
        c->out_dense = dense;
        if (half_emit && nq) {
            EmitHalfArgs h;
            h.v = view(c);
            h.ref = c->d_adj_ref;
            h.adj = c->d_adj;
            h.half = c->d_half;
            h.hcnt = dense ? nullptr : (const u32 *)c->d_hcnt;
            h.out_src = c->d_out_src;
            h.out_ent = c->d_out_ent;
            h.out_cap = c->d_out_src.cap;
            h.bump = c->d_bump;
            h.local_only = c->dist_active ? 1u : 0u;
            h.own = own_set(c);
            h.order = nullptr;
            if (dense) {
                const int gh = wq_grid(c, emit_half_lists_kernel, (nq + 63) / 64, "DISCO_EMIT_WAVES");
                hipLaunchKernelGGL(emit_half_lists_kernel, dim3(gh), dim3(64), 0, c->stream, h);
            } else {
                const int gh = wq_grid(c, emit_half_kernel, (nq + 63) / 64, "DISCO_EMIT_WAVES");
                hipLaunchKernelGGL(emit_half_kernel, dim3(gh), dim3(64), 0, c->stream, h);
            }
        }
        EmitArgs a;
        a.v = view(c);
        a.ref = c->d_adj_ref;
        a.adj = c->d_adj;
        a.hcnt = half_emit && !dense ? (const u32 *)c->d_hcnt : nullptr;
        a.half = half_emit ? c->d_half : nullptr;
        const bool listed = half_emit && c->n_wide <= c->d_wide.cap;
        a.list = listed ? c->d_wide : nullptr;
        a.n_list = listed ? c->n_wide : 0;
        a.out_src = c->d_out_src;
        a.out_ent = c->d_out_ent;
        a.out_cap = c->d_out_src.cap;
        a.bump = c->d_bump;
        a.local_only = c->dist_active ? 1u : 0u;
        a.own = own_set(c);
        HIPCHK(c, hipMemsetAsync(c->d_wq, 0, sizeof(u64) * WQ_WORDS, c->stream));
        if (nq && !(listed && c->n_wide == 0)) {
            if (dense) hipLaunchKernelGGL(emit_kernel<true>, dim3(grid), dim3(64), 0, c->stream, a);
            else hipLaunchKernelGGL(emit_kernel<false>, dim3(grid), dim3(64), 0, c->stream, a);
        }
        if (n_push) {
            EmitRecvArgs pr;
            pr.items = c->d_push_r;
            pr.n_items = n_push;
            pr.ref = c->d_adj_ref;
            pr.adj = c->d_adj;
            pr.half = c->d_half;
            pr.hcnt = c->d_hcnt;
            pr.out_src = c->d_out_src;
            pr.out_ent = c->d_out_ent;
            pr.out_cap = c->d_out_src.cap;
            pr.bump = c->d_bump;
            pr.wq = c->d_wq;
            HIPCHK(c, hipMemsetAsync(c->d_wq, 0, sizeof(u64) * WQ_WORDS, c->stream));
            hipLaunchKernelGGL(emit_push_recv_kernel, dim3(grid_push), dim3(64), 0, c->stream, pr);
        }
        HIPCHK(c, hipGetLastError());
        u64 used = 0;
        HIPCHK(c, hipMemcpyAsync(&used, c->d_bump, sizeof(u64), hipMemcpyDeviceToHost, c->stream));
        HIPCHK(c, hipStreamSynchronize(c->stream));
        if (used <= c->d_out_src.cap) {
            c->out_used = used;
            break;
        }
        want = used + used / 8 + nwaves * EMIT_CHUNK;
        if (attempt == 5) return fail(c, DISCO_E_CAPACITY, "disco_emit_edges: output buffer could not be sized");
    }
    u64 total = 0;
    if (c->out_dense) {
        total = c->out_used;
        release(c, c->d_out_valid);
        release(c, c->d_out_pos);
    } else if (c->out_used) {
        if (c->out_used > c->d_out_valid.cap || c->out_used + 1 > c->d_out_pos.cap) {
            release(c, c->d_out_valid);
            release(c, c->d_out_pos);
            int rc = ensure(c, c->d_out_valid, c->d_out_src.cap);
            if (rc == DISCO_OK) rc = ensure(c, c->d_out_pos, c->d_out_src.cap + 1);
            if (rc != DISCO_OK) {
                release(c, c->d_out_valid);
                return rc;
            }
        }
        hipLaunchKernelGGL(emit_valid_kernel, dim3(flat_grid(c, c->out_used)), dim3(256), 0, c->stream, c->d_out_src, c->out_used, c->d_out_valid);
        CHK((scan_exclusive<u8, u64>(c, c->d_out_valid, c->out_used, c->d_out_pos, true, nullptr)));
        HIPCHK(c, hipMemcpyAsync(&total, c->d_total, sizeof(u64), hipMemcpyDeviceToHost, c->stream));
    }
    ph_end(c, DISCO_PH_EMIT);
    HIPCHK(c, hipStreamSynchronize(c->stream));
    ph_collect(c);
    c->n_out = total;
    if (n_out) *n_out = total;
    c->phase = 8;
    return DISCO_OK;
}

int disco_transitive_reduce(disco_ctx *c, uint64_t *n_out)
{
    CHK(disco_transitive_mark(c));
    return disco_emit_edges(c, n_out);
}

int disco_run_graph(disco_ctx *c)
{
    DISCO_TRACE("disco_run_graph");
    const bool verbose = getenv("DISCO_VERBOSE") != nullptr;
    auto now = [] { return std::chrono::steady_clock::now(); };
    auto ms = [](std::chrono::steady_clock::time_point a, std::chrono::steady_clock::time_point b) { return std::chrono::duration<double, std::milli>(b - a).count(); };
    auto t0 = now();
    CHK(disco_build_index(c));
    auto t1 = now();
    CHK(disco_probe(c));
    auto t2 = now();
    {
        CHK(ensure(c, c->d_contained, c->n_alloc));
        CHK(ensure(c, c->d_cbits, c->n_alloc / 64 + 1));
        CHK(zero_counter(c, CTR_N_CONTAINED));
        ph_begin(c, DISCO_PH_CONTAIN);
        if (c->n) hipLaunchKernelGGL(contain_flags_kernel, dim3(flat_grid(c, c->n)), dim3(256), 0, c->stream, c->d_best, c->n, c->d_contained, c->d_cbits, c->d_ctr);
        HIPCHK(c, hipGetLastError());
        ph_end(c, DISCO_PH_CONTAIN);
        c->contained_count_pending = true;
        c->phase = 4;
        c->crows_pending = c->cgrp_pending = false;
    }
    auto t3 = now();
    CHK(disco_build_edges(c, nullptr));
    auto t4 = now();
    int rc = disco_transitive_reduce(c, nullptr);
    auto t5 = now();
    if (verbose)
        fprintf(stderr, "[disco] host wall ms: index %.1f probe %.1f contain %.1f edges %.1f reduce %.1f\n", ms(t0, t1), ms(t1, t2), ms(t2, t3), ms(t3, t4), ms(t4, t5));
    return rc;
}

static int ensure_host_len(disco_ctx *c)
{
    std::lock_guard<std::mutex> lk(c->h_len_mu);
    if (c->h_len_ok && c->h_len.size() == c->n) return DISCO_OK;
    c->h_len.resize(c->n);
    if (c->n) HIPCHK(c, hipMemcpy(c->h_len.data(), c->d_len, c->n * 2, hipMemcpyDeviceToHost));
    c->h_len_ok = true;
    return DISCO_OK;
}

int64_t disco_fetch_contained(disco_ctx *c, disco_contained_row *out, uint64_t cap)
{
    DISCO_TRACE("disco_fetch_contained");
    if (!c) return DISCO_E_ARG;
    if (c->phase < 4) return fail(c, DISCO_E_STATE, "disco_fetch_contained: run disco_mark_contained first");
    HIPCHK(c, hipSetDevice(c->device));
    const u64 nc = c->n_contained;
    if (!out) return (int64_t)nc;
    if (cap < nc) return fail(c, DISCO_E_ARG, "disco_fetch_contained: need room for %llu rows", (unsigned long long)nc);
    if (nc == 0) return 0;
    auto decode = [&](auto id_of, const u64 *keys_h, const u32 *lens_h) {
        const u16 *hlen = lens_h ? nullptr : c->h_len.data();
        const u32 kk = (u32)c->k;
        parallel_for(nc, [&, hlen, kk, lens_h](u64 b, u64 e_) {
            for (u64 i = b; i < e_; i++) {
                const u64 key = keys_h[i];
                disco_contained_row &r = out[i];
                r.contained = id_of(i);
                r.super = CKEY_SUPER(key);
                r.j = CKEY_J(key);
                r.type = disco_hit_type(CKEY_SUFFIX(key), CKEY_REV(key));
                r.len2 = lens_h ? (lens_h[i] & 0xFFFFu) : hlen[r.contained];
                r.len1 = lens_h ? (lens_h[i] >> 16) : hlen[r.super];
                u32 orient, off;
                disco_map_type(r.type, r.len1, kk, r.j, &orient, &off);
                r.orient = orient;
                r.start = off;
            }
        });
    };
    CHK(start_contained_rows(c, false));
    if (c->crows_pending && c->crows_n == nc) {
        HIPCHK(c, hipEventSynchronize(c->ev_crows));
        const u64 *hkey = (const u64 *)c->h_crows;
        const u32 *hid = (const u32 *)(hkey + c->crows_hcap);
        decode([hid](u64 i) { return (u64)hid[i]; }, hkey, hid + c->crows_hcap);
        return (int64_t)nc;
    }
    CHK(ensure_host_len(c));
    CHK(settle_keys(c));
    DevBuf<u64> pos, ids, keys;
    std::vector<u64> hid(nc), hkey(nc);
    auto gather = [&]() -> int {
        CHK(ensure(c, pos, c->n + 1));
        CHK(ensure(c, ids, nc));
        CHK(ensure(c, keys, nc));
        CHK((scan_exclusive<u8, u64>(c, c->d_contained, c->n, pos, false, nullptr)));
// ... 2203 lines not shown
            unsigned long long mine = (msg.ok && bulk_ready) ? 1ull : 0ull, all[DIST_MAX_WORLD];
            rc = cm->host_all_gather(&mine, 1, all, c->stream);
            bool everybody = rc == DISCO_OK;
            for (int p = 0; everybody && p < nranks; p++) everybody = all[p] != 0ull;
            if (rc == DISCO_OK && everybody) {
                const int rb = bulk->join(&msg.id);
                mine = rb == DISCO_OK ? 1ull : 0ull;
                rc = cm->host_all_gather(&mine, 1, all, c->stream);
                for (int p = 0; rc == DISCO_OK && everybody && p < nranks; p++) everybody = all[p] != 0ull;
            }
            if (rc == DISCO_OK && !everybody) {
                if (rank == 0) fprintf(stderr, "[disco] no second communicator on every rank: the reads are gathered on the first one\n");
                delete bulk;
                bulk = nullptr;
            }
        }
    }
    if (one_comm) {
        delete bulk;
        bulk = nullptr;
    }
    if (rc == DISCO_OK && bulk) {
        cm->sibling = bulk;
        bulk->sibling = cm;
    }
    if (rc != DISCO_OK) {
        fail(c, rc, "disco_comm_init: %s %s", cm->err.c_str(), bulk ? bulk->err.c_str() : "");
        delete cm;
        delete bulk;
        return rc;
    }
    return comm_attach(c, cm, bulk);
}

int disco_comm_init_local(disco_ctx *const *ctxs, int nranks)
{
    if (!ctxs || nranks < 1 || nranks > DIST_MAX_WORLD) return DISCO_E_ARG;
    for (int r = 0; r < nranks; r++)
        if (!ctxs[r]) return DISCO_E_ARG;
    auto grp = std::make_shared<LoopGroup>(nranks), grp2 = std::make_shared<LoopGroup>(nranks);
    for (int r = 0; r < nranks; r++) {
        const int rc = comm_attach(ctxs[r], new LoopComm(grp, r), new LoopComm(grp2, r));
        if (rc != DISCO_OK) return rc;
    }
    return DISCO_OK;
}

int disco_probe_run_words(const disco_ctx *c) { return c ? c->runs_lpr : 0; }

int disco_fetch_order(disco_ctx *c, uint64_t *order_words, uint32_t *keys, uint64_t cap, uint64_t *n, int *order_bits)
{
    if (!c || !order_words || !keys || !n || !order_bits) return DISCO_E_ARG;
    if (!c->order_ready || !c->d_order_own || !c->d_okey) return fail(c, DISCO_E_STATE, "disco_fetch_order: disco_build_index made no order");
    *n = c->n;
    *order_bits = c->order_counted_bits;
    if (cap < c->n) return fail(c, DISCO_E_ARG, "disco_fetch_order: room for %llu reads, %llu needed", (unsigned long long)cap, (unsigned long long)c->n);
    HIPCHK(c, hipSetDevice(c->device));
    HIPCHK(c, hipMemcpyAsync(order_words, c->d_order_own, c->n * sizeof(u64), hipMemcpyDeviceToHost, c->stream));
    HIPCHK(c, hipMemcpyAsync(keys, c->d_okey, c->n * sizeof(u32), hipMemcpyDeviceToHost, c->stream));
    HIPCHK(c, hipStreamSynchronize(c->stream));
    return DISCO_OK;
}
int disco_fetch_survivor_layout(disco_ctx *c, uint8_t *list_len, uint64_t cap, uint64_t *n, int *dense, uint64_t *out_used)
{
    if (!c || !n || !dense || !out_used) return DISCO_E_ARG;
    if (c->phase < 8) return fail(c, DISCO_E_STATE, "disco_fetch_survivor_layout: run disco_transitive_reduce first");
    *n = c->n;
    *dense = c->out_dense ? 1 : 0;
    *out_used = c->out_used;
    if (!list_len) return DISCO_OK;
    if (cap < c->n) return fail(c, DISCO_E_ARG, "disco_fetch_survivor_layout: room for %llu nodes, %llu needed", (unsigned long long)cap, (unsigned long long)c->n);
    if (!c->half_selfdel || !c->d_half) return fail(c, DISCO_E_STATE, "disco_fetch_survivor_layout: the last marking kept counts, not self-delimiting lists");
    HIPCHK(c, hipSetDevice(c->device));
    std::vector<u64> half(c->n * HALF_CAP), ref(c->n);
    if (c->n) {
        HIPCHK(c, hipMemcpyAsync(half.data(), c->d_half, c->n * HALF_CAP * sizeof(u64), hipMemcpyDeviceToHost, c->stream));
        HIPCHK(c, hipMemcpyAsync(ref.data(), c->d_adj_ref, c->n * sizeof(u64), hipMemcpyDeviceToHost, c->stream));
        HIPCHK(c, hipStreamSynchronize(c->stream));
    }
    for (u64 v = 0; v < c->n; v++)
        list_len[v] = REF_DEG(ref[v]) ? (uint8_t)surv_len(half[4 * v], half[4 * v + 1], half[4 * v + 2], half[4 * v + 3]) : 0xFFu;
    return DISCO_OK;
}
int disco_comm_rank(const disco_ctx *c) { return (c && c->comm) ? c->comm->rank : 0; }
int disco_comm_world(const disco_ctx *c) { return (c && c->comm) ? c->comm->world : 1; }
const char *disco_comm_kind(const disco_ctx *c) { return (c && c->comm) ? c->comm->kind() : "none"; }

int disco_dist_range(const disco_ctx *c, uint64_t n_total, uint64_t *lo, uint64_t *hi)
{
    if (!c || !lo || !hi) return DISCO_E_ARG;
    u64 per, l, h;
    dist_range(c, n_total, &per, &l, &h);
    *lo = l;
    *hi = h;
    return DISCO_OK;
}

static int dist_set_reads(disco_ctx *c, u64 n_total, uint32_t dstride)
{
    if (!c->comm) return fail(c, DISCO_E_STATE, "no communicator: call disco_comm_init / disco_comm_init_local first");
    u64 per, lo, hi;
    dist_range(c, n_total, &per, &lo, &hi);
    CHK(begin_rows(c, n_total, per * (u64)c->comm->world, 0, dstride, false));
    c->per = per;
    c->q_lo = c->home_lo = lo;
    c->q_hi = c->home_hi = hi;
    HIPCHK(c, hipMemsetAsync(c->d_reads, 0, c->n_alloc * (u64)dstride * 8, c->stream));
    c->dist_reads = true;
    c->ingest_n = 0;
    return DISCO_OK;
}

static int dist_validate(disco_ctx *c)
{
    const u64 nloc = c->q_hi - c->q_lo;
    CHK(count_lengths(c, c->q_lo, c->q_hi));
    u64 bad = c->h_ctr[CTR_BAD_LEN], ext[2] = {c->h_ctr[CTR_MAX_LEN], c->h_ctr[CTR_MIN_LEN]};
    CHK(host_reduce(c, &bad, 1));
    CHK(host_reduce(c, ext, 2, true));
    if (bad) return fail(c, DISCO_E_ARG, "%llu reads have a length outside (min_overlap=%u, min(32767, 32*stride)]", (unsigned long long)bad, c->prm.min_overlap);
    c->max_len = (u32)ext[0];
    c->min_len = 0xFFFFu - (u32)ext[1];
    CHK(ensure(c, c->d_list_n, 1));
    HIPCHK(c, hipMemsetAsync(c->d_list_n, 0, sizeof(u64), c->stream));
    if (nloc) hipLaunchKernelGGL(probes_sum_kernel, dim3(flat_grid(c, nloc)), dim3(256), 0, c->stream, c->d_len, c->q_lo, c->q_hi, (u32)c->k, c->d_list_n);
    HIPCHK(c, hipMemcpyAsync(&c->home_probes, c->d_list_n, sizeof(u64), hipMemcpyDeviceToHost, c->stream));
    HIPCHK(c, hipStreamSynchronize(c->stream));
    c->job_n_long = 0;
    c->job_short_max = c->max_len;
    if (c->max_len > (u32)DISCO_SHORT_MAX) {
        DevBuf<u64> d_ls;
        u64 hls[2] = {0, 0};
        CHK(ensure(c, d_ls, 2));
        HIPCHK(c, hipMemsetAsync(d_ls, 0, 2 * sizeof(u64), c->stream));
        if (nloc) hipLaunchKernelGGL(long_stats_kernel, dim3(flat_grid(c, nloc)), dim3(256), 0, c->stream, (const u16 *)c->d_len, c->q_lo, c->q_hi, d_ls);
        HIPCHK(c, hipMemcpyAsync(hls, d_ls, sizeof hls, hipMemcpyDeviceToHost, c->stream));
        HIPCHK(c, hipStreamSynchronize(c->stream));
        release(c, d_ls);
        CHK(host_reduce(c, &hls[0], 1));
        CHK(host_reduce(c, &hls[1], 1, true));
        c->job_n_long = hls[0];
        c->job_short_max = (u32)hls[1];
    }
    c->phase = 1;
    return DISCO_OK;
}

int disco_dist_upload_reads(disco_ctx *c, const uint64_t *packed_own, uint32_t stride_words, const uint16_t *len_own, uint64_t n_total)
{
    DISCO_TRACE("disco_dist_upload_reads");
    if (!c) return DISCO_E_ARG;
    HIPCHK(c, hipSetDevice(c->device));
    const uint32_t dstride = (stride_words + 7u) & ~7u;
    CHK(dist_set_reads(c, n_total, dstride));
    const u64 nloc = c->q_hi - c->q_lo;
    if (nloc && (!packed_own || !len_own)) return fail(c, DISCO_E_ARG, "disco_dist_upload_reads: null argument");
    if (nloc) {
        u64 *dst = c->d_reads + c->q_lo * (u64)dstride;
        if (dstride != stride_words) HIPCHK(c, hipMemsetAsync(dst, 0, nloc * (u64)dstride * 8, c->stream));
        HIPCHK(c, hipMemcpy2DAsync(dst, (size_t)dstride * 8, packed_own, (size_t)stride_words * 8, (size_t)stride_words * 8, nloc, hipMemcpyHostToDevice, c->stream));
        HIPCHK(c, hipMemcpyAsync(c->d_len + c->q_lo, len_own, nloc * 2, hipMemcpyHostToDevice, c->stream));
    }
    return dist_validate(c);
}

int disco_dist_generate_reads(disco_ctx *c, const disco_genspec_abi *s)
// ... 760 lines not shown
```

### disco_amd/csrc/disco_kernels.h

```cpp
#ifndef DISCO_KERNELS_H_
#define DISCO_KERNELS_H_

#include "disco_device.h"
#include "readgen.h"

#define PROBE_ROWCAP 512
#define PROBE_SEGW 128
#define PROBE_SEGP (PROBE_SEGW + 64)
#define PROBE_ACAP 32
#define PROBE_CHUNK 4096
#define ES_MID 1024
#define ES_DUPBITS 11
#define ES_DUPTAB (1 << ES_DUPBITS)
#ifndef ES_CAP
#define ES_CAP 256
#endif
#ifndef TR_CAP
#define TR_CAP 256
#endif
#define TR_CAP_SMALL 128
#define VERIFY_SW 8
#define ORDER_BUCKET(key, shift) (((key) * 0x9E3779B1u) >> (shift))
#define SCAN_ITEMS 16
#define SCAN_BLOCK 256
#define SCAN_TILE (SCAN_ITEMS * SCAN_BLOCK)

#define REF_MAKE(pos, deg) (((u64)(deg) << 40) | (u64)(pos))
#define REF_POS(r) ((r)&0xFFFFFFFFFFull)
#define REF_DEG(r) ((u32)((r) >> 40))
#define ADJ_FLAG (1ull << 15)
#define ADJ_HIDDEN_OF(hit) ((u64)HIT_HIDDEN(hit) << 15)
#define EXTRA_NODE_MAKE(w, slot) ((u64)(w) | ((u64)(slot) << 32))
#define EXTRA_NODE(e) ((e)&0xFFFFFFFFull)
#define EXTRA_SLOT(e) ((u32)((e) >> 32))

enum {
    CTR_KMER_HITS = 0,
    CTR_RAW_HITS,
    CTR_HITS_NEEDED,
    CTR_OVERFLOW,
    CTR_CAP_SITES,
    CTR_ASYM,
    CTR_N_CONTAINED,
    CTR_BAD_LEN,
    CTR_BIG_ROWS,
    CTR_ES_BIG,
    CTR_TR_BIG,
    CTR_MAX_DEG,
    CTR_MAX_ROW,
    CTR_TW_UP,
    CTR_TW_DOWN,
    CTR_ES_SLOW,
    CTR_ADJ_TOTAL,
    CTR_MAX_LEN,
    CTR_DROPPED,
    CTR_MIN_LEN,
    CTR_DROP_ITEMS,
    CTR_SHORT_MAX,
    CTR_TR_MID,
    CTR_ES_MID,
    CTR_COUNT
};

#define WQ_CHUNK 64
#define ORDER_MAKE(id, l) ((u64)(id) | ((u64)(l) << 32))
#define ORDER_ID(o) ((o) & 0xFFFFFFFFull)
#define ORDER_LEN(o) ((int)((o) >> 32))
#define ORDER_ITEM(key, shift, id, l, idbits) (((u64)ORDER_BUCKET(key, shift) << (32u + (shift))) | ((u64)(l) << (idbits)) | (u64)(id))
__device__ __forceinline__ u32 uniform_u32(u32 x) { return (u32)__builtin_amdgcn_readfirstlane((int)x); }
__device__ __forceinline__ u64 uniform_u64(u64 x)
{
    return ((u64)uniform_u32((u32)(x >> 32)) << 32) | uniform_u32((u32)x);
}

template <u32 CHUNK = WQ_CHUNK>
__device__ __forceinline__ bool wq_grab(u64 *counter, u64 n, u64 &beg, u64 &end)
{
    u64 b = 0;
    if ((threadIdx.x & 63) == 0) b = atomicAdd(counter, (u64)CHUNK);
#ifdef WQ_EXP_SHFL
    b = __shfl(b, 0);
#else
    b = uniform_u64(b);
#endif
    beg = b;
    end = (b + CHUNK < n) ? b + CHUNK : n;
    return b < n;
}

template <u32 CHUNK = WQ_CHUNK, u32 MULT = 4>
__device__ __forceinline__ bool wq_grab_multi(u64 *counter, u64 n, u64 &beg, u64 &end, u64 &gnext, u64 &gend)
{
    if (gnext >= gend) {
        if (!wq_grab<CHUNK * MULT>(counter, n, gnext, gend)) return false;
    }
    beg = gnext;
    end = beg + CHUNK < gend ? beg + CHUNK : gend;
    gnext = end;
    return true;
}

#define WQ_NQ 8u
#define WQ_WORDS (16u * WQ_NQ)
struct WqSplit {
    u32 qi = 0;
};
template <u32 CHUNK = WQ_CHUNK>
__device__ __forceinline__ bool wq_grab_split(u64 *counters, u64 n, u64 &beg, u64 &end, WqSplit &st)
{
    const u32 nchunks = (u32)((n + CHUNK - 1u) / CHUNK);
    const u32 per = (nchunks + WQ_NQ - 1u) / WQ_NQ;
    while (st.qi < WQ_NQ) {
        const u32 q = ((u32)blockIdx.x + st.qi) % WQ_NQ;
        const u32 first = q * per;
        const u32 mine = first < nchunks ? (nchunks - first < per ? nchunks - first : per) : 0u;
        u32 b = mine;
        if (mine) {
            u32 t = 0;
            if ((threadIdx.x & 63) == 0) t = atomicAdd((u32 *)&counters[16u * q], 1u);
            b = uniform_u32(t);
        }
        if (b < mine) {
            beg = (u64)(first + b) * CHUNK;
            end = beg + CHUNK < n ? beg + CHUNK : n;
            return true;
        }
        st.qi++;
    }
    return false;
}

struct DiscoView {
    const u64 *reads;
    const u16 *len;
    u64 n;
    int S;
    int k;
    int ks;
    int m;
    const u32 *bkt;
    const u64 *ent;
    int bshift;
    u64 q_lo, q_hi;
    u64 *ctr;
    u64 *wq;
    const u64 *full;
    const u32 *ovf;
    const u32 *long_ids;
    u32 n_long;
    int SL;
    int tailb;
};

struct OwnSet {
    const u8 *otab;
    u32 me;
    u64 lo, hi;
    const u64 *list;
    u64 n_own;
    const u32 *ids;
    __device__ __forceinline__ bool mine(u64 v) const { return otab ? otab[v] == (u8)me : (v >= lo && v < hi); }
    __device__ __forceinline__ u64 count() const { return otab ? n_own : hi - lo; }
    __device__ __forceinline__ u64 node(u64 i) const { return otab ? ORDER_ID(list[i]) : lo + i; }
    __device__ __forceinline__ u64 node_by_id(u64 i) const { return otab ? (u64)ids[i] : lo + i; }
};
__host__ __device__ __forceinline__ u32 disco_key_owner(u32 key, u32 G) { return (u32)(((u64)(key * 0x9E3779B1u) * (u64)G) >> 32); }

__global__ void generate_reads_kernel(disco_genspec spec, u64 *__restrict__ reads, u16 *__restrict__ len, int S, u64 r_lo, u64 r_hi)
{
    u64 gid = r_lo * (u64)S + (u64)blockIdx.x * blockDim.x + threadIdx.x;
    u64 total = r_hi * (u64)S;
    for (; gid < total; gid += (u64)gridDim.x * blockDim.x) {
        u64 r = gid / S;
        int w = (int)(gid % S);
        disco_readloc loc = disco_read_location(&spec, r);
        u64 word = 0;
        int base0 = w * 32;
        for (int i = 0; i < 32; i++) {
            int p = base0 + i;
            if (p < (int)loc.len) word |= (u64)disco_read_base(&spec, &loc, (u32)p) << (62 - 2 * i);
        }
        reads[gid] = word;
        if (w == 0) len[r] = (u16)loc.len;
    }
}

__global__ void substitute_bases_kernel(u64 seed, u32 rate_ppm, u64 *__restrict__ reads, const u16 *__restrict__ len, int S, u64 r_lo, u64 r_hi)
{
    u64 gid = r_lo * (u64)S + (u64)blockIdx.x * blockDim.x + threadIdx.x;
    const u64 total = r_hi * (u64)S;
    for (; gid < total; gid += (u64)gridDim.x * blockDim.x) {
        const u64 r = gid / S;
        const int base0 = (int)(gid % S) * 32, L = (int)len[r];
        if (base0 >= L) continue;
        const u64 word = reads[gid];
        u64 out = 0;
        for (int i = 0; i < 32; i++) {
            u32 b = (u32)(word >> (62 - 2 * i)) & 3u;
            if (base0 + i < L) b = disco_substituted_base(seed, rate_ppm, r, (u32)(base0 + i), b);
            else b = 0;
            out |= (u64)b << (62 - 2 * i);
        }
        reads[gid] = out;
    }
}

__global__ void validate_len_kernel(const u16 *__restrict__ len, u64 n, int S, int min_overlap, u64 *ctr)
{
    u64 i = (u64)blockIdx.x * blockDim.x + threadIdx.x;
    u32 bad = 0, mx = 0, mn = 0xFFFFu;
    for (; i < n; i += (u64)gridDim.x * blockDim.x) {
        u32 L = len[i];
        if (L <= (u32)min_overlap || L > 32767u || L > (u32)S * 32u) bad++;
        mx = L > mx ? L : mx;
        mn = L < mn ? L : mn;
    }
    if (bad) atomicAdd(&ctr[CTR_BAD_LEN], (u64)bad);
    for (int o = 32; o > 0; o >>= 1) {
        mx = max(mx, (u32)__shfl_down(mx, o));
        mn = min(mn, (u32)__shfl_down(mn, o));
    }
    if ((threadIdx.x & 63) == 0) {
        atomicMax(&ctr[CTR_MAX_LEN], (u64)mx);
        atomicMax(&ctr[CTR_MIN_LEN], (u64)(0xFFFFu - mn));
    }
}

template <bool COUNT, bool LONGK = false, bool LONGCLASS = false>
__global__ void __launch_bounds__(256) index_count_kernel(DiscoView v, u32 *__restrict__ bkt, ulonglong2 *__restrict__ rec, u32 *__restrict__ okey, u64 lo, u64 hi,
                                                          u32 *__restrict__ ocnt, u32 *__restrict__ oslot, u64 *__restrict__ oitem, u32 oidbits, u32 oshift,
                                                          const u64 *__restrict__ list = nullptr)
{
    const u64 x = lo + (u64)blockIdx.x * 256u + threadIdx.x;
    if (x >= hi) return;
    const u64 i = LONGCLASS ? (u64)v.long_ids[x] : x;
    const u64 lw = (!LONGCLASS && list) ? list[x] : 0ull;
    const u64 rid = (!LONGCLASS && list) ? ORDER_ID(lw) : i;
    if (LONGCLASS) lo = 0;
    const int S = LONGCLASS ? v.SL : v.S;
    const u64 *__restrict__ p = LONGCLASS ? v.full + x * (u64)S : v.reads + rid * (u64)S;
    if (!LONGCLASS && v.full && v.len[rid] > DISCO_SHORT_MAX) return;
    const int L = (!LONGCLASS && list) ? ORDER_LEN(lw) : (int)v.len[rid], k = v.ks, m = v.m, nf = k - m + 1;
    const int nmm = L - m + 1;
    const int sfx0 = nmm - nf;
    const u64 mask = (1ull << (2 * m)) - 1ull;
    const int rsh = 2 * (m - 1);
    u64 f = 0, r = 0, word = 0;
    int pos = 0;
    auto next = [&]() {
        if ((pos & 31) == 0) word = p[pos >> 5];
        const u32 b = (u32)(word >> 62);
        word <<= 2;
        ++pos;
        f = ((f << 2) | b) & mask;
        r = (r >> 2) | ((u64)(3u - b) << rsh);
    };
    u32 best = 0xFFFFFFFFu;
    auto order_word = [&]() {
        next();
        const bool st = r < f;
        const u32 h = order_hash32(st ? r : f);
        best = min(best, h);
        return (h & ~0x1FFu) | (u32)st;
    };
    for (int q = 0; q < m - 1; ++q) next();
    u32 k1p = 0xFFFFFFFFu, k2p = 0xFFFFFFFFu, k1s = 0xFFFFFFFFu, k2s = 0xFFFFFFFFu;
    int q = 0;
    for (; q < nf; ++q) {
        const u32 o = order_word();
        k1p = min(k1p, o + ((u32)q << 1));
        k2p = min(k2p, o + ((u32)(63 - q) << 1));
        if (q >= sfx0) {
            k1s = min(k1s, o + ((u32)(q - sfx0) << 1));
            k2s = min(k2s, o + ((u32)(63 - (q - sfx0)) << 1));
        }
    }
    for (; q < sfx0; ++q) order_word();
    for (; q < nmm; ++q) {
        const u32 o = order_word();
        k1s = min(k1s, o + ((u32)(q - sfx0) << 1));
        k2s = min(k2s, o + ((u32)(63 - (q - sfx0)) << 1));
    }
    if (okey) okey[i] = best;
    if (oitem) oitem[i - lo] = ORDER_ITEM(best, oshift, rid, L, oidbits);
    else if (ocnt) oslot[i - lo] = atomicAdd(&ocnt[ORDER_BUCKET(best, oshift)], 1u);
    auto resolve = [&](u32 k1, u32 k2, int j0, u32 &t, u32 &rev) {
        const int ffirst = (int)((k1 >> 1) & 63u), flast = 63 - (int)((k2 >> 1) & 63u);
        int fsel = ffirst;
        if (ffirst == flast)
            rev = k1 & 1u;
        else {
            rev = kmer_is_rev<false, LONGK>(p, S, j0, k);
            fsel = rev ? flast : ffirst;
        }
        t = rev ? (u32)(nf - 1 - fsel) : (u32)fsel;
        return mmer_key(p, S, j0 + fsel, m);
    };
    u32 tp, rp, ts, rs;
    const u64 kp = resolve(k1p, k2p, 0, tp, rp);
    const u64 ks = resolve(k1s, k2s, sfx0, ts, rs);
    const u64 bp = kp >> v.bshift, bs = ks >> v.bshift;
    const u32 sp = COUNT ? atomicAdd(&bkt[bp], 1u) : 0u;
    const u32 ss = COUNT ? atomicAdd(&bkt[bs], 1u) : 0u;
    rec[2 * (i - lo)] = make_ulonglong2((bp << 32) | sp, PAY_MAKE(kp, rid, tp, rp, 0, L));
    rec[2 * (i - lo) + 1] = make_ulonglong2((bs << 32) | ss, PAY_MAKE(ks, LONGCLASS ? v.n + x : rid, ts, rs, 1, L));
}

#define RUNS_M 23
template <bool B>
struct FlagConst {
    static constexpr bool value = B;
};
template <int M>
struct MmerRoll {
    static_assert(M == 0 || (M > 16 && M <= 24 && (M & 1)), "two dwords, the high one partly used; a 24-bit fold in order_hash32<false>");
    const u64 *__restrict__ p;
    int last_word;
    u32 himask, rsh;
    int pos = 0;
    u64 word = 0;
    u32 cw = 0;
    u32 flo = 0, fhi = 0, rlo = 0, rhi = 0;
    bool st = false;
    u32 clo = 0, chi = 0;
    __device__ __forceinline__ MmerRoll(const u64 *row, int S, int m = M) : p(row), last_word(S - 1), himask((1u << (2 * m - 32)) - 1u), rsh((u32)(2 * m - 34)) {}
    __device__ __forceinline__ void step()
    {
        if ((pos & 15) == 0) {
            if ((pos & 31) == 0) word = p[min(pos >> 5, last_word)];
            cw = (pos & 16) ? (u32)word : (u32)(word >> 32);
        }
        const u32 b = __builtin_amdgcn_ubfe(cw, (u32)(30 - 2 * (pos & 15)), 2u);
        ++pos;
        fhi = __builtin_amdgcn_alignbit(fhi, flo, 30u) & (M ? ((1u << (2 * (M ? M : 17) - 32)) - 1u) : himask);
        flo = (flo << 2) | b;
        rlo = __builtin_amdgcn_alignbit(rhi, rlo, 2u);
        rhi = (rhi >> 2) | ((b ^ 3u) << (M ? (u32)(2 * (M ? M : 17) - 34) : rsh));
        st = (((u64)rhi << 32) | rlo) < (((u64)fhi << 32) | flo);
        clo = st ? rlo : flo;
        chi = st ? rhi : fhi;
    }
    __device__ __forceinline__ u32 hash() const { return order_hash32<M == 0>(((u64)chi << 32) | clo); }
    __device__ __forceinline__ u32 strand() const { return st ? 1u : 0u; }
};
#define RUN_W(e) ((u32)(e) >> 7)
#define RUN_DELTA(e) (((u32)(e) >> 1) & 63u)
#define RUN_STRAND(e) ((u32)(e)&1u)
#define OCC_MAKE(slot, e, wend) (((u32)(slot) << 29) | (RUN_STRAND(e) << 23) | (RUN_DELTA(e) << 17) | ((u32)(wend) << 8) | RUN_W(e))
#define OCC_SLOT(d) ((u32)(d) >> 29)
#define OCC_STRAND(d) (((u32)(d) >> 23) & 1u)
#define OCC_DELTA(d) (((u32)(d) >> 17) & 63u)
#define OCC_END(d) (((u32)(d) >> 8) & 0x1FFu)
#define OCC_FIRST(d) ((u32)(d)&0xFFu)

template <bool COUNT, int NF, int NL, int NFMAX = NF, bool LONGK = false>
__global__ void __launch_bounds__(256) index_runs_kernel(DiscoView v, u32 *__restrict__ bkt, ulonglong2 *__restrict__ rec, u32 *__restrict__ okey, u64 lo, u64 hi,
                                                         u32 *__restrict__ runs, u32 *__restrict__ ocnt, u32 *__restrict__ oslot, u64 *__restrict__ oitem, u32 oidbits,
                                                         u32 oshift,
                                                         const u64 *__restrict__ list = nullptr)
{
    static_assert(NF == 0 || NF == NFMAX, "a specialised instantiation holds exactly its window");
    constexpr int CAP = 32 * NL;
    __shared__ u16 s_runs[256 * CAP];
    __shared__ u32 s_x[3 * 256];
    const u32 tid = threadIdx.x;
    for (u32 x = tid; x < 256u * CAP / 2u; x += 256u) ((u32 *)s_runs)[x] = 0xFFFFFFFFu;
    __syncthreads();
    const u64 i = lo + (u64)blockIdx.x * 256u + tid;
    const u64 lw = (list && i < hi) ? list[i] : 0ull;
    const u64 rid = list ? ORDER_ID(lw) : i;
    const bool other_class = i < hi && v.full && v.len[rid] > DISCO_SHORT_MAX;
    if (other_class) s_runs[tid * CAP] = 0xFFFEu;
    const bool mine = i < hi && !other_class;
    const int L = mine ? (list ? ORDER_LEN(lw) : (int)v.len[rid]) : 0;
    int npos_lo = mine ? L - v.ks : 0x7FFFFFFF;
    for (int o = 32; o; o >>= 1) npos_lo = min(npos_lo, __shfl_xor(npos_lo, o));
    npos_lo = __builtin_amdgcn_readfirstlane(npos_lo);
    if (mine) {
        const u64 *__restrict__ p = v.reads + rid * v.S;
        const int k = v.ks;
        const int m = NF ? RUNS_M : v.m;
        const int nf = NF ? NF : k - m + 1;
        const int nmm = L - m + 1;
        const int npos = nmm - nf;
        MmerRoll<NF ? RUNS_M : 0> roll(p, v.S, m);
        u32 best = 0xFFFFFFFFu;
        for (int q = 0; q < m - 1; ++q) roll.step();
        u32 s1[NFMAX], s2[NFMAX];
#pragma clang loop unroll(full)
        for (int t = 0; t < NFMAX; ++t) s1[t] = s2[t] = 0xFFFFFFFFu;
        u16 *my = s_runs + tid * CAP;
        u32 cnt = 0, lastm = 0xFFFFFFFFu, tie = 0;
        u32 P1 = 0, P2 = 0;
        u32 *sx = s_x + tid;
        auto window = [&](auto inner, int w, u32 m1, u32 m2, int base, int tw) __attribute__((always_inline)) {
            if (decltype(inner)::value || w <= npos) {
                if (!decltype(inner)::value && w == npos) {
                    sx[0] = m1;
                    sx[256] = m2;
                    sx[512] = (u32)base;
                } else {
                    tie |= (m1 ^ m2) ^ 0xFEu;
                    if (((m1 ^ lastm) >> 1) != 0u) {
                        lastm = m1;
                        my[cnt < (u32)CAP ? cnt : (u32)CAP - 1u] = (u16)((m1 & 0xFFu) + (((u32)w << 7) - 2u * (u32)tw));
                        ++cnt;
                    }
                }
            }
        };
        const int nblk = npos / nf + 2;
        int q = 0;
        auto block = [&](auto inner, int b) __attribute__((always_inline)) {
            const int base = (b - 1) * nf;
            lastm -= (u32)nf << 1;
            if (b >= 1) window(inner, base, s1[0], s2[0], base, 0);
            if (b == 1) {
                P1 = s1[0];
                P2 = s2[0];
            }
            u32 p1 = 0xFFFFFFFFu, p2 = 0xFFFFFFFFu;
            u32 hc[NFMAX];
#pragma clang loop unroll(full)
            for (int t = 0; t < NFMAX; ++t) {
                if (NF != 0 || t < nf) {
                    roll.step();
                    const u32 h = roll.hash();
                    best = min(best, decltype(inner)::value || q < nmm ? h : 0xFFFFFFFFu);
                    const u32 o = (h & ~0x1FFu) | roll.strand();
                    ++q;
                    hc[t] = o;
                    p1 = min(p1, o | ((u32)(nf + t) << 1));
                    p2 = min(p2, o | ((u32)(127 - (nf + t)) << 1));
                    if (t + 1 < nf && b >= 1) window(inner, base + t + 1, min(s1[t + 1 < NFMAX ? t + 1 : 0], p1), min(s2[t + 1 < NFMAX ? t + 1 : 0], p2), base, t + 1);
                }
            }
            u32 a1 = 0xFFFFFFFFu, a2 = 0xFFFFFFFFu;
#pragma clang loop unroll(full)
            for (int t = NFMAX - 1; t >= 0; --t) {
                if (NF == 0 && t >= nf) continue;
                a1 = min(a1, hc[t] | ((u32)t << 1));
                a2 = min(a2, hc[t] | ((u32)(127 - t) << 1));
                s1[t] = a1;
                s2[t] = a2;
            }
        };
        int b = 0;
        for (const int inner_end = npos_lo / nf; b <= inner_end; ++b) block(FlagConst<true>(), b);
        for (; b < nblk; ++b) block(FlagConst<false>(), b);
        if (okey) okey[i] = best;
        if (oitem) oitem[i - lo] = ORDER_ITEM(best, oshift, rid, L, oidbits);
        else if (ocnt) oslot[i - lo] = atomicAdd(&ocnt[ORDER_BUCKET(best, oshift)], 1u);
        if ((tie & ~1u) != 0 || cnt > (u32)CAP) my[0] = 0xFFFEu;
        auto resolve = [&](u32 k1, u32 k2, int wbase, int j0, u32 &t, u32 &rev) {
            const int ffirst = wbase + (int)((k1 >> 1) & 0x7Fu) - j0, flast = wbase + 127 - (int)((k2 >> 1) & 0x7Fu) - j0;
            int fsel = ffirst;
            if (ffirst == flast)
                rev = k1 & 1u;
            else {
                rev = kmer_is_rev<false, LONGK>(p, v.S, j0, k);
                fsel = rev ? flast : ffirst;
            }
            t = rev ? (u32)(nf - 1 - fsel) : (u32)fsel;
            return mmer_key(p, v.S, j0 + fsel, m);
        };
        u32 tp, rp, ts, rs;
        const u64 kp = resolve(P1, P2, 0, 0, tp, rp);
        const u64 ks = resolve(sx[0], sx[256], (int)sx[512], npos, ts, rs);
        const u64 bp = kp >> v.bshift, bs = ks >> v.bshift;
        const u32 sp = COUNT ? atomicAdd(&bkt[bp], 1u) : 0u;
        const u32 ss = COUNT ? atomicAdd(&bkt[bs], 1u) : 0u;
        rec[2 * (i - lo)] = make_ulonglong2((bp << 32) | sp, PAY_MAKE(kp, rid, tp, rp, 0, L));
        rec[2 * (i - lo) + 1] = make_ulonglong2((bs << 32) | ss, PAY_MAKE(ks, rid, ts, rs, 1, L));
    }
    __syncthreads();
#if defined(INDEX_EXP_NORUNS)
    if (tid != 9999u) return;
#endif
    const u64 r0 = (u64)blockIdx.x * 256u;
    const u64 nr = (hi - lo) - r0 < 256u ? (hi - lo) - r0 : 256u;
    u32 *__restrict__ dst = runs + r0 * (CAP / 2);
    for (u32 x = tid; x < (u32)nr * (CAP / 2); x += 256u) dst[x] = ((const u32 *)s_runs)[x];
}

__global__ void index_fill_kernel(u64 n2, const ulonglong2 *__restrict__ rec, const u32 *__restrict__ bkt, u64 *__restrict__ ent)
{
    u64 i = (u64)blockIdx.x * blockDim.x + threadIdx.x;
    for (; i < n2; i += (u64)gridDim.x * blockDim.x) {
        const ulonglong2 r = rec[i];
        ent[(u64)bkt[r.x >> 32] + (u32)r.x] = r.y;
    }
}

__global__ void index_fill_ordered_kernel(u64 nq, const u64 *__restrict__ order, const ulonglong2 *__restrict__ rec, const u32 *__restrict__ bkt, u64 *__restrict__ ent)
{
    u64 i = (u64)blockIdx.x * blockDim.x + threadIdx.x;
    for (; i < nq; i += (u64)gridDim.x * blockDim.x) {
        const u64 id = ORDER_ID(order[i]);
        const ulonglong2 r0 = rec[2 * id], r1 = rec[2 * id + 1];
        ent[(u64)bkt[r0.x >> 32] + (u32)r0.x] = r0.y;
        ent[(u64)bkt[r1.x >> 32] + (u32)r1.x] = r1.y;
    }
}

#define BINX_SPAN_BITS 14
#define BINX_MAX_BITS 8
#define BINX_TILE 2048u
#define BINX_BLOCK 256u
#define BINX_BUILD_BLOCK 1024u

__device__ __forceinline__ u32 binx_block_scan1024(u32 x, u32 *s_w, u32 *total)
{
    u32 incl = x;
    for (int o = 1; o < 64; o <<= 1) {
        const u32 y = __shfl_up(incl, o);
        if ((int)(threadIdx.x & 63) >= o) incl += y;
    }
    __syncthreads();
    if ((threadIdx.x & 63) == 63) s_w[threadIdx.x >> 6] = incl;
    __syncthreads();
    u32 off = 0, sum = 0;
    for (u32 w = 0; w < 16u; w++) {
        const u32 t = s_w[w];
        off += w < (threadIdx.x >> 6) ? t : 0u;
        sum += t;
    }
    *total = sum;
    return off + incl - x;
}

__global__ void __launch_bounds__(1024) binx_segs_kernel(const u32 *__restrict__ prev_scan, const u32 *__restrict__ ptb, u32 pseg, u32 pnb, u32 total, u32 *__restrict__ seg,
                                                         u32 *__restrict__ tb)
{
    __shared__ u32 s_w[16];
    const u32 nseg = prev_scan ? pseg * pnb : 1u;
    for (u32 x = threadIdx.x; x < nseg; x += 1024u) {
        u32 st = 0;
        if (prev_scan) {
            const u32 s = x / pnb, d = x % pnb;
            const u32 t0 = ptb[s], nt = ptb[s + 1] - t0;
            st = prev_scan[(u64)pnb * t0 + (u64)d * nt];
        }
        seg[x] = st;
    }
    if (threadIdx.x == 0) seg[nseg] = total;
    if (!tb) return;
    __syncthreads();
    u32 carry = 0;
    for (u32 base = 0; base < nseg; base += 1024u) {
        const u32 x = base + threadIdx.x;
        const u32 nt = x < nseg ? (seg[x + 1] - seg[x] + BINX_TILE - 1u) / BINX_TILE : 0u;
        u32 sum;
        const u32 ex = binx_block_scan1024(nt, s_w, &sum);
        if (x < nseg) tb[x] = carry + ex;
        carry += sum;
    }
    if (threadIdx.x == 0) tb[nseg] = carry;
}

__device__ __forceinline__ bool binx_tile(const u32 *__restrict__ seg, const u32 *__restrict__ tb, u32 nseg, u32 &t0, u32 &nt, u32 &ti, u32 &lo, u32 &hi)
{
    const u32 t = blockIdx.x;
    if (t >= tb[nseg]) return false;
    u32 a = 0, b = nseg;
    while (b - a > 1u) {
        const u32 mid = (a + b) >> 1;
        if (tb[mid] <= t) a = mid;
        else b = mid;
    }
    t0 = tb[a];
    nt = tb[a + 1] - t0;
    ti = t - t0;
    const u32 end = seg[a + 1];
    lo = seg[a] + ti * BINX_TILE;
    hi = end - lo > BINX_TILE ? lo + BINX_TILE : end;
    return true;
}

__device__ __forceinline__ u64 binx_key(const ulonglong2 &r) { return r.x; }
__device__ __forceinline__ u64 binx_key(u64 r) { return r; }
#define BINX_DIGIT(key, shift, nb) ((u32)((key) >> (shift)) & ((nb)-1u))

template <typename R>
__global__ void __launch_bounds__(BINX_BLOCK) binx_hist_kernel(const R *__restrict__ rec, const u32 *__restrict__ seg, const u32 *__restrict__ tb, u32 nseg, u32 shift, u32 nb,
                                                               u32 *__restrict__ hist)
{
    __shared__ u32 s_h[1u << BINX_MAX_BITS];
    u32 t0, nt, ti, lo, hi;
    if (!binx_tile(seg, tb, nseg, t0, nt, ti, lo, hi)) return;
    s_h[threadIdx.x] = 0;
    __syncthreads();
    for (u32 i = lo + threadIdx.x; i < hi; i += BINX_BLOCK) atomicAdd(&s_h[BINX_DIGIT(binx_key(rec[i]), shift, nb)], 1u);
    __syncthreads();
    if (threadIdx.x < nb) hist[(u64)nb * t0 + (u64)threadIdx.x * nt + ti] = s_h[threadIdx.x];
}

template <typename R>
__global__ void __launch_bounds__(BINX_BLOCK) binx_scatter_kernel(const R *__restrict__ src, R *__restrict__ dst, const u32 *__restrict__ seg, const u32 *__restrict__ tb,
                                                                  u32 nseg, u32 shift, u32 nb, const u32 *__restrict__ scan)
{
    static_assert(BINX_BLOCK == (1u << BINX_MAX_BITS) && BINX_TILE % BINX_BLOCK == 0, "a thread per bin; whole rounds per tile");
    constexpr u32 PER = BINX_TILE / BINX_BLOCK;
    __shared__ R s_rec[BINX_TILE];
    __shared__ u32 s_cnt[BINX_BLOCK], s_base[BINX_BLOCK], s_w[BINX_BLOCK / 64u];
    const u32 tid = threadIdx.x;
    u32 t0, nt, ti, lo, hi;
    if (!binx_tile(seg, tb, nseg, t0, nt, ti, lo, hi)) return;
    s_cnt[tid] = 0;
    __syncthreads();
    R r[PER];
    u32 rank[PER];
#pragma unroll
    for (u32 j = 0; j < PER; j++) {
        const u32 i = lo + j * BINX_BLOCK + tid;
        if (i < hi) {
            r[j] = src[i];
            rank[j] = atomicAdd(&s_cnt[BINX_DIGIT(binx_key(r[j]), shift, nb)], 1u);
        }
    }
    __syncthreads();
    const u32 cnt = s_cnt[tid];
    u32 incl = cnt;
    for (int o = 1; o < 64; o <<= 1) {
        const u32 y = __shfl_up(incl, o);
        if ((int)(tid & 63u) >= o) incl += y;
    }
    if ((tid & 63u) == 63u) s_w[tid >> 6] = incl;
    __syncthreads();
    u32 start = incl - cnt;
    for (u32 w = 0; w < (tid >> 6); w++) start += s_w[w];
    __syncthreads();
    s_cnt[tid] = start;
    if (tid < nb) s_base[tid] = scan[(u64)nb * t0 + (u64)tid * nt + ti] - start;
    __syncthreads();
#pragma unroll
    for (u32 j = 0; j < PER; j++) {
        const u32 i = lo + j * BINX_BLOCK + tid;
        if (i < hi) s_rec[s_cnt[BINX_DIGIT(binx_key(r[j]), shift, nb)] + rank[j]] = r[j];
    }
    __syncthreads();
    for (u32 j = tid; j < hi - lo; j += BINX_BLOCK) {
        const R x = s_rec[j];
        dst[s_base[BINX_DIGIT(binx_key(x), shift, nb)] + j] = x;
    }
}

__device__ __forceinline__ u64 binx_payload(const ulonglong2 &r, u32, u32) { return r.y; }
__device__ __forceinline__ u64 binx_payload(u64 r, u32 kshift, u32 idbits) { return ORDER_MAKE(r & ((1ull << idbits) - 1ull), (r << (64u - kshift)) >> (64u - kshift + idbits)); }
template <typename R>
__global__ void __launch_bounds__(BINX_BUILD_BLOCK) binx_build_kernel(const R *__restrict__ rec, const u32 *__restrict__ part, u32 span, u32 kshift, u32 idbits, u32 total, u64 T,
                                                                      u32 *__restrict__ bkt, u64 *__restrict__ ent)
{
    constexpr bool TABLE = sizeof(R) == sizeof(ulonglong2);
    __shared__ u32 s_c[1u << BINX_SPAN_BITS];
    __shared__ u32 s_w[16];
    const u32 tid = threadIdx.x, p = blockIdx.x;
    const u32 nbk = 1u << span, mask = nbk - 1u;
    const u32 beg = part[p], end = part[p + 1];
    for (u32 x = tid; x < nbk; x += BINX_BUILD_BLOCK) s_c[x] = 0;
    __syncthreads();
    for (u32 i = beg + tid; i < end; i += BINX_BUILD_BLOCK) atomicAdd(&s_c[(u32)(binx_key(rec[i]) >> kshift) & mask], 1u);
    __syncthreads();
    u32 carry = beg;
    for (u32 base = 0; base < nbk; base += BINX_BUILD_BLOCK) {
        const u32 x = s_c[base + tid];
        u32 sum;
        const u32 ex = binx_block_scan1024(x, s_w, &sum);
        s_c[base + tid] = carry + ex;
        if (TABLE) bkt[(u64)p * nbk + base + tid] = carry + ex;
        carry += sum;
    }
    if (TABLE && (u64)(p + 1u) * nbk == T && tid == 0) bkt[T] = total;
    __syncthreads();
    for (u32 i = beg + tid; i < end; i += BINX_BUILD_BLOCK) {
        const R x = rec[i];
        ent[atomicAdd(&s_c[(u32)(binx_key(x) >> kshift) & mask], 1u)] = binx_payload(x, kshift, idbits);
    }
}

template <typename InT>
__global__ void __launch_bounds__(SCAN_BLOCK) scan_tile_sums_kernel(const InT *__restrict__ in, u64 n, u64 *__restrict__ tile_sums)
{
    __shared__ u64 s_part[SCAN_BLOCK / DISCO_WAVE];
    u64 base = (u64)blockIdx.x * SCAN_TILE;
    u64 sum = 0;
    for (int i = 0; i < SCAN_ITEMS; i++) {
        u64 idx = base + (u64)i * SCAN_BLOCK + threadIdx.x;
        if (idx < n) sum += (u64)in[idx];
    }
    for (int o = 32; o > 0; o >>= 1) sum += __shfl_down(sum, o);
    if ((threadIdx.x & 63) == 0) s_part[threadIdx.x >> 6] = sum;
    __syncthreads();
    if (threadIdx.x == 0) {
        u64 t = 0;
        for (int w = 0; w < SCAN_BLOCK / DISCO_WAVE; w++) t += s_part[w];
        tile_sums[blockIdx.x] = t;
    }
}

__global__ void __launch_bounds__(1024) scan_sums_kernel(u64 *__restrict__ tile_sums, u64 nt, u64 *__restrict__ total)
{
    __shared__ u64 s_w[16];
    __shared__ u64 s_carry;
    if (threadIdx.x == 0) s_carry = 0;
    __syncthreads();
    for (u64 base = 0; base < nt; base += 1024) {
        u64 idx = base + threadIdx.x;
        u64 x = idx < nt ? tile_sums[idx] : 0;
        u64 incl = x;
        for (int o = 1; o < 64; o <<= 1) {
            u64 y = __shfl_up(incl, o);
            if ((int)(threadIdx.x & 63) >= o) incl += y;
        }
        if ((threadIdx.x & 63) == 63) s_w[threadIdx.x >> 6] = incl;
        __syncthreads();
        u64 woff = 0;
        for (int w = 0; w < (int)(threadIdx.x >> 6); w++) woff += s_w[w];
        u64 carry = s_carry;
        if (idx < nt) tile_sums[idx] = carry + woff + incl - x;
        __syncthreads();
        if (threadIdx.x == 1023) s_carry = carry + woff + incl;
        __syncthreads();
    }
    if (threadIdx.x == 0) *total = s_carry;
}

template <typename InT, typename OutT>
__global__ void __launch_bounds__(SCAN_BLOCK) scan_apply_kernel(const InT *in, u64 n, const u64 *__restrict__ tile_sums, OutT *out)
{
    __shared__ u64 s_w[SCAN_BLOCK / DISCO_WAVE];
    u64 base = (u64)blockIdx.x * SCAN_TILE + (u64)threadIdx.x * SCAN_ITEMS;
    u64 vals[SCAN_ITEMS];
    u64 sum = 0;
#pragma unroll
    for (int i = 0; i < SCAN_ITEMS; i++) {
        u64 idx = base + i;
        vals[i] = idx < n ? (u64)in[idx] : 0;
        sum += vals[i];
    }
    u64 incl = sum;
    for (int o = 1; o < 64; o <<= 1) {
        u64 y = __shfl_up(incl, o);
        if ((int)(threadIdx.x & 63) >= o) incl += y;
    }
    if ((threadIdx.x & 63) == 63) s_w[threadIdx.x >> 6] = incl;
    __syncthreads();
    u64 off = tile_sums[blockIdx.x] + incl - sum;
    for (int w = 0; w < (int)(threadIdx.x >> 6); w++) off += s_w[w];
#pragma unroll
    for (int i = 0; i < SCAN_ITEMS; i++) {
        u64 idx = base + i;
        if (idx < n) out[idx] = (OutT)off;
        off += vals[i];
    }
}

template <typename OutT>
__global__ void scan_write_total_kernel(const u64 *total, OutT *out_n) { *out_n = (OutT)*total; }

struct ProbeRare {
    u64 *bump;
    u64 hits_cap;
    u64 *big_list;
    u32 *big_cnt;
    u32 *n_big;
    u32 big_cap;
    u32 slow_cap;
    u64 *ctr;
    u64 *slow_list;
    u32 *n_slow;
};
struct ProbeArgs {
    DiscoView v;
    u64 *hits;
    u64 *row_start;
    u32 *row_cnt;
    ulonglong2 *meta_ord;
    const ProbeRare *rare;
    const u64 *order;
};

#ifndef PROBE_WAVES_PER_SIMD
#define PROBE_WAVES_PER_SIMD 8
#endif
template <int PMODE, bool LDSROW, bool ROW17, bool LONGK = false, bool LONGCLASS = false>
__global__ void __launch_bounds__(64, (LONGK || LONGCLASS) ? PROBE_WAVES_PER_SIMD - 2 : (ROW17 ? PROBE_WAVES_PER_SIMD - 1 : PROBE_WAVES_PER_SIMD)) probe_kernel(ProbeArgs a)
{
    static_assert(!LONGCLASS || (PMODE != 0 && !LDSROW), "the long class is only ever met in the lists");
    constexpr bool BIG = PMODE == 1, LISTED = PMODE != 0;
    __shared__ u32 s_k1[PROBE_SEGP + 32];
    __shared__ u32 s_k2[PROBE_SEGP + 32];
    __shared__ u8 s_strand[PROBE_SEGP];
    __shared__ u32 s_first[PROBE_SEGP];
    __shared__ u16 s_wp[PROBE_SEGW];
    __shared__ u16 s_lead[PROBE_SEGW];
    __shared__ u32 s_occ_fp[64];
    __shared__ u32 s_occ_start[64];
    __shared__ u32 s_occ_excl[64];
    __shared__ u16 s_occ_prel[64];
    __shared__ u8 s_mark[64];
    __shared__ u64 s_a[PROBE_ACAP + 2];
    const u32 lane = threadIdx.x;
    const int S = a.v.S, k = a.v.ks;
    const int m = a.v.m, nf = k - m + 1;
    const int dl = LONGK ? a.v.k - k : 0;
    u64 chunk_base = 0;
    u32 chunk_used = PROBE_CHUNK;
    u32 my_maxrow = 0;
    const u64 n_items = BIG ? (u64)min(*a.rare->n_big, a.rare->big_cap) : (PMODE == 2 ? (u64)min(*a.rare->n_slow, a.rare->slow_cap) : (a.v.q_hi - a.v.q_lo));

    u64 pre_w = 0;
    int pre_len = 0;
    u64 cbeg = 0, cend = 0;
    u64 ord_chunk = 0;
    auto rid = [&](u64 it) { return readlane_u64(ord_chunk, (u32)(it - cbeg)); };
    while (wq_grab(a.v.wq, n_items, cbeg, cend)) {
    if (!LISTED) {
        const u64 i = min(cbeg + lane, cend - 1);
        ord_chunk = a.order ? a.order[i] : ORDER_MAKE(a.v.q_lo + i, a.v.len[a.v.q_lo + i]);
    }
    if (!LISTED && LDSROW) {
        const u64 o0 = rid(cbeg);
        const u64 A0 = ORDER_ID(o0);
        pre_len = ORDER_LEN(o0);
        if ((int)lane < S) pre_w = a.v.reads[A0 * S + lane];
    }
    for (u64 it = cbeg; it < cend; it++) {
        const u64 bl = BIG ? a.rare->big_list[it] : (PMODE == 2 ? a.rare->slow_list[it] : 0ull);
        const u64 oe = LISTED ? 0ull : rid(it);
        const u64 A = LISTED ? (bl & 0xFFFFFFFFull) : ORDER_ID(oe);
        const u64 opos = LISTED ? (bl >> 32) : it;
        const u64 *ga = a.v.reads + A * S;
        int LA;
        int Sx = S;
        u64 A2 = A;
        if (LISTED && (LDSROW || LONGCLASS) && a.v.full && (int)a.v.len[A] > DISCO_SHORT_MAX) {
            const u32 x = a.v.ovf[A];
            Sx = a.v.SL;
            ga = a.v.full + (u64)x * Sx;
            A2 = a.v.n + x;
        }
        __syncthreads();
        if (!LISTED && LDSROW) {
            LA = pre_len;
            if ((int)lane < PROBE_ACAP + 2) s_a[lane] = ((int)lane < S) ? pre_w : 0ull;
            const u64 itn = it + 1;
            if (itn < cend) {
                const u64 on = rid(itn);
                const u64 An = ORDER_ID(on);
                pre_len = ORDER_LEN(on);
                if ((int)lane < S) pre_w = a.v.reads[An * S + lane];
            }
        } else {
            LA = LISTED ? (int)a.v.len[A] : ORDER_LEN(oe);
            if (LDSROW && (int)lane < PROBE_ACAP + 2) s_a[lane] = ((int)lane < Sx) ? ga[lane] : 0ull;
        }
        const int npos = LA - k;
        const u32 nref = (u32)(npos - dl);
        const u64 *pa = LDSROW ? (const u64 *)s_a : ga;
        u32 nrow = 0;
        u64 *grow = nullptr;
        u32 want = 0;
        if (BIG) {
            u64 base = 0;
            want = a.rare->big_cnt[it];
            if (lane == 0) {
                base = atomicAdd(a.rare->bump, (u64)want);
                atomicMax(&a.rare->ctr[CTR_HITS_NEEDED], base + want);
                a.row_start[A] = base;
            }
            base = __shfl(base, 0);
            if (base + want <= a.rare->hits_cap) grow = a.hits + base;
            else {
                want = 0;
                if (lane == 0) atomicAdd(&a.rare->ctr[CTR_OVERFLOW], 1ull);
            }
        } else {
            if (PROBE_CHUNK - chunk_used < PROBE_ROWCAP) {
                u64 base = 0;
                if (lane == 0) {
                    base = atomicAdd(a.rare->bump, (u64)PROBE_CHUNK);
                    atomicMax(&a.rare->ctr[CTR_HITS_NEEDED], base + PROBE_CHUNK);
                    if (base + PROBE_CHUNK > a.rare->hits_cap) {
                        atomicAdd(&a.rare->ctr[CTR_OVERFLOW], 1ull);
                        base = ~0ull;
                    }
                }
                chunk_base = __shfl(base, 0);
                chunk_used = 0;
            }
            if (chunk_base != ~0ull) {
                grow = a.hits + chunk_base + chunk_used;
                want = PROBE_CHUNK - chunk_used;
            }
        }

        auto push = [&](bool take, u64 pay, u32 rev, int jj) {
            if (LONGK) {
                if (PAY_SUFFIX(pay) != rev) jj -= dl;
// ... 2380 lines not shown
                    const u32 cnt = go ? (s_bins[rl * 64u + (off >> 2)] >> (8u * (off & 3u))) & 0xFFu : 0u;
                    if (go) s_ent[rl * 64u + st + ((segm[i] >> 8) & 0xFFu)] = ent[i];
                    segm[i] = (segm[i] & 0xFF3Fu) | (go ? 64u : 0u) | (cnt << 16) | (st << 24);
                }
            }
            __syncthreads();
#pragma unroll
            for (int i = 0; i < NB; i++) {
                if ((u32)i < nbat) {
                    const u32 seg = segm[i] & 63u, rl = seg - r0;
                    const u32 st = segm[i] >> 24, cnt = (segm[i] >> 16) & 0xFFu, rk = (segm[i] >> 8) & 0xFFu;
                    const u64 other = s_ent[rl * 64u + st + (cnt == 2u ? (rk ^ 1u) : rk)];
                    u32 below = other < ent[i] ? 1u : 0u;
                    if (__any(cnt > 2u)) {
                        if (cnt > 2u) {
                            below = 0;
                            for (u32 t = 0; t < cnt; t++) below += s_ent[rl * 64u + st + t] < ent[i] ? 1u : 0u;
                        }
                    }
                    if (segm[i] & 64u) a.hits[s_hdr[seg].x + st + below] = ent[i];
                }
            }
        }
        if (lane < n && !((slowmask >> lane) & 1ull)) a.ref[A] = c ? REF_MAKE(meta.x, nacc_me) : 0ull;
        {
            u32 t = ((slowmask >> lane) & 1ull) ? 0u : nacc_me;
            t = wave_inclusive_add(t);
            n_edges += (u32)__builtin_amdgcn_readlane((int)t, 63);
        }
#ifdef SEL_EXP_NOSLOW
        slowmask = 0;
#endif
        while (slowmask) {
            const u32 i = (u32)__ffsll((long long)slowmask) - 1u;
            slowmask &= slowmask - 1ull;
            const u64 Ai = (u32)__builtin_amdgcn_readlane((int)A, (int)i);
            const u64 rs = readlane_u64(meta.x, i);
            const u32 c0 = (u32)__builtin_amdgcn_readlane((int)craw, (int)i);
            const u32 L0 = (u32)__builtin_amdgcn_readlane((int)LAme, (int)i);
            __syncthreads();
            if (c0 > SEQ_CAP) {
                if (lane == 0) {
                    const u32 idx = atomicAdd(a.n_big, 1u);
                    if (idx < a.big_cap) a.big_list[idx] = Ai;
                    else atomicAdd(&a.v.ctr[CTR_OVERFLOW], 1ull);
                    a.ref[Ai] = 0;
                }
                continue;
            }
            bool done = false;
            if (c0 <= 64u) {
                u64 g = ~0ull;
                if (lane < c0) {
                    g = a.hits[rs + lane];
                    if (is_contained(a.contained, HIT_ID(g))) g = ~0ull;
                }
                done = edge_select_row_fast(a, Ai, rs, L0, g, lane, dropped, n_edges);
            }
            if (!done) {
                n_slow++;
                edge_select_row<(int)SEQ_CAP>(a, Ai, rs, s_ent, s_ent + SEQ_CAP, c0, lane, s_jc, cap_sites, dropped, n_edges, tr_wide);
            }
        }
    }
    if (lane == 0 && n_edges) atomicAdd(&a.v.ctr[CTR_ADJ_TOTAL], n_edges);
    if (lane == 0 && n_slow) atomicAdd(&a.v.ctr[CTR_ES_SLOW], (u64)n_slow);
    if (lane == 0 && cap_sites) atomicAdd(&a.v.ctr[CTR_CAP_SITES], (u64)cap_sites);
    tr_wide_flush(a, tr_wide, lane);
    if (lane == 0 && dropped) atomicAdd(&a.v.ctr[CTR_DROPPED], (u64)dropped);
}

template <int CAP>
__global__ void __launch_bounds__(64) edge_select_mid_kernel(EdgeSelArgs a, u32 above)
{
    __shared__ u64 s_h[CAP];
    __shared__ u64 s_t[CAP];
    __shared__ u32 s_jcnt[128];
    const u32 lane = threadIdx.x;
    u32 cap_sites = 0, dropped = 0, n_slow = 0;
    u64 n_edges = 0, tr_wide = 0;
    const u64 n_items = (u64)min(*a.n_big, a.big_cap);
    u64 cbeg = 0, cend = 0;
    u64 gnext = 0, gend = 0;
    while (wq_grab_multi<1, 8>(a.v.wq, n_items, cbeg, cend, gnext, gend)) {
        const u64 A = a.big_list[cbeg];
        const u32 c = a.row_cnt[A];
        if (c > (u32)CAP || c <= above) continue;
        n_slow++;
        edge_select_row<CAP>(a, A, a.row_start[A], s_h, s_t, c, lane, s_jcnt, cap_sites, dropped, n_edges, tr_wide);
    }
    if (lane == 0 && n_edges) atomicAdd(&a.v.ctr[CTR_ADJ_TOTAL], n_edges);
    if (lane == 0 && n_slow) atomicAdd(&a.v.ctr[CTR_ES_SLOW], (u64)n_slow);
    if (lane == 0 && cap_sites) atomicAdd(&a.v.ctr[CTR_CAP_SITES], (u64)cap_sites);
    tr_wide_flush(a, tr_wide, lane);
    if (lane == 0 && dropped) atomicAdd(&a.v.ctr[CTR_DROPPED], (u64)dropped);
}


__global__ void deg_from_ref_kernel(const u64 *__restrict__ ref, u64 lo, u64 hi, u32 *__restrict__ out)
{
    u64 i = lo + (u64)blockIdx.x * blockDim.x + threadIdx.x;
    for (; i < hi; i += (u64)gridDim.x * blockDim.x) out[i - lo] = REF_DEG(ref[i]);
}

__global__ void ref_from_start_kernel(const u64 *__restrict__ start, const u32 *__restrict__ deg, u64 n, u64 *__restrict__ ref)
{
    u64 i = (u64)blockIdx.x * blockDim.x + threadIdx.x;
    for (; i < n; i += (u64)gridDim.x * blockDim.x) ref[i] = REF_MAKE(start[i], deg[i]);
}

__global__ void __launch_bounds__(64) rows_gather_kernel(const u64 *__restrict__ adj, const u64 *__restrict__ ref, u64 lo, u64 hi,
                                                         const u64 *__restrict__ dst_start, u64 *__restrict__ dst, u64 strip)
{
    for (u64 v = lo + blockIdx.x; v < hi; v += gridDim.x) {
        const u64 r = ref[v];
        const u32 d = REF_DEG(r);
        const u64 *src = adj + REF_POS(r);
        u64 *o = dst + dst_start[v - lo];
        for (u32 i = threadIdx.x; i < d; i += 64) o[i] = src[i] & ~strip;
    }
}

#define NBR32_MAKE(e) ((u32)ADJ_DST(e) | (ADJ_ORI(e) << 30))
#define NBR32_ENTRY(x) ADJ_MAKE(0u, (u64)((x)&0x3FFFFFFFu), (x) >> 30, 0u)
__global__ void __launch_bounds__(64) rows_gather32_kernel(const u64 *__restrict__ adj, const u64 *__restrict__ ref, u64 lo, u64 hi,
                                                           const u64 *__restrict__ dst_start, u32 *__restrict__ dst)
{
    for (u64 v = lo + blockIdx.x; v < hi; v += gridDim.x) {
        const u64 r = ref[v];
        const u32 d = REF_DEG(r);
        const u64 *src = adj + REF_POS(r);
        u32 *o = dst + dst_start[v - lo];
        for (u32 i = threadIdx.x; i < d; i += 64) o[i] = NBR32_MAKE(src[i]);
    }
}

__device__ __forceinline__ int adj_find(const u64 *__restrict__ r, u32 d, u64 key)
{
    u32 lo = 0, hi = d;
    while (lo < hi) {
        u32 mid = (lo + hi) >> 1;
        u64 x = r[mid] & ~ADJ_FLAG;
        if (x < key) lo = mid + 1;
        else hi = mid;
    }
    return (lo < d && (r[lo] & ~ADJ_FLAG) == key) ? (int)lo : -1;
}

struct TwinArgs {
    DiscoView v;
    const u64 *ref;
    const u64 *adj;
    u64 lo, hi;
    const u8 *otab;
    u32 me;
    u32 *extra_cnt;
    u64 *extra_node;
    u64 *extra_key;
    u32 *n_extra;
    u32 extra_cap;
    const u64 *dropbits;
    int up_only;
    int hidden_flags;
};

#ifndef TW_PEND
// ... 1013 lines not shown
{
    u64 i = (u64)blockIdx.x * blockDim.x + threadIdx.x;
    for (; i < nq; i += (u64)gridDim.x * blockDim.x) oslot[i] = atomicAdd(&cnt[ORDER_BUCKET(okey[i], shift)], 1u);
}

__global__ void order_scatter_kernel(const u32 *__restrict__ okey, const u32 *__restrict__ oslot, const u32 *__restrict__ start, u32 shift, u64 lo, u64 nq,
                                     const u16 *__restrict__ len, u64 *__restrict__ order)
{
    u64 i = (u64)blockIdx.x * blockDim.x + threadIdx.x;
    for (; i < nq; i += (u64)gridDim.x * blockDim.x) order[(u64)start[ORDER_BUCKET(okey[i], shift)] + oslot[i]] = ORDER_MAKE(lo + i, len[lo + i]);
}

__global__ void order_pack_kernel(const u64 *__restrict__ ids, u64 nq, const u16 *__restrict__ len, u64 *__restrict__ order)
{
    u64 i = (u64)blockIdx.x * blockDim.x + threadIdx.x;
    for (; i < nq; i += (u64)gridDim.x * blockDim.x) order[i] = ORDER_MAKE(ids[i], len[ids[i]]);
}

__global__ void count_above_kernel(const u32 *__restrict__ cnt, const u64 *__restrict__ ref, u64 lo, u64 hi, u32 thr, u64 *out)
{
    u64 i = lo + (u64)blockIdx.x * blockDim.x + threadIdx.x;
    u32 c = 0;
    for (; i < hi; i += (u64)gridDim.x * blockDim.x) c += (ref ? REF_DEG(ref[i]) : cnt[i]) > thr;
    for (int o = 32; o > 0; o >>= 1) c += __shfl_down(c, o);
    if ((threadIdx.x & 63) == 0 && c) atomicAdd(out, (u64)c);
}

__global__ void __launch_bounds__(256) stream_copy_kernel(const ulonglong2 *__restrict__ src, ulonglong2 *__restrict__ dst, u64 n)
{
    u64 i = (u64)blockIdx.x * blockDim.x + threadIdx.x;
    const u64 step = (u64)gridDim.x * blockDim.x;
    for (; i + 3 * step < n; i += 4 * step) {
        const ulonglong2 x0 = src[i], x1 = src[i + step], x2 = src[i + 2 * step], x3 = src[i + 3 * step];
        dst[i] = x0;
        dst[i + step] = x1;
        dst[i + 2 * step] = x2;
        dst[i + 3 * step] = x3;
    }
    for (; i < n; i += step) dst[i] = src[i];
}

__global__ void __launch_bounds__(256) gather_rows_kernel(const ulonglong2 *__restrict__ tab, u64 nrows, u32 per_lane, u64 *__restrict__ sink)
{
    const u64 tid = (u64)blockIdx.x * blockDim.x + threadIdx.x;
    u64 acc = 0;
    for (u32 it = 0; it < per_lane; it += 4) {
        ulonglong2 v[4][4];
#pragma unroll
        for (int u = 0; u < 4; u++) {
            const u64 r = disco_hash64(tid * per_lane + it + u) % nrows;
            const ulonglong2 *g = tab + r * 4;
            v[u][0] = g[0];
            v[u][1] = g[1];
            v[u][2] = g[2];
            v[u][3] = g[3];
        }
#pragma unroll
        for (int u = 0; u < 4; u++) acc ^= v[u][0].x ^ v[u][1].y ^ v[u][2].x ^ v[u][3].y;
    }
    if (acc == 0x1234567ull) sink[0] = acc;
}

__global__ void max_u32_kernel(const u32 *__restrict__ p, u64 n, u64 *__restrict__ out)
{
    u64 i = (u64)blockIdx.x * blockDim.x + threadIdx.x;
    u32 m = 0;
    for (; i < n; i += (u64)gridDim.x * blockDim.x) m = max(m, p[i]);
    for (int o = 32; o > 0; o >>= 1) m = max(m, (u32)__shfl_down(m, o));
    if ((threadIdx.x & 63) == 0 && m) atomicMax(out, (u64)m);
}

__global__ void iota_u64_kernel(u64 *p, u64 n)
{
    u64 i = (u64)blockIdx.x * blockDim.x + threadIdx.x;
    for (; i < n; i += (u64)gridDim.x * blockDim.x) p[i] = i;
}

__global__ void fill_u64_kernel(u64 *p, u64 n, u64 val)
{
    u64 i = (u64)blockIdx.x * blockDim.x + threadIdx.x;
    for (; i < n; i += (u64)gridDim.x * blockDim.x) p[i] = val;
}

#endif
```

### include/disco_hip_inspect.h

```cpp
#ifndef DISCO_HIP_INSPECT_H_
#define DISCO_HIP_INSPECT_H_

#include "disco_hip.h"

#ifdef __cplusplus
extern "C" {
#endif

int disco_fetch_order(disco_ctx *ctx, uint64_t *order_words, uint32_t *keys, uint64_t cap, uint64_t *n, int *order_bits);

int disco_fetch_survivor_layout(disco_ctx *ctx, uint8_t *list_len, uint64_t cap, uint64_t *n, int *dense, uint64_t *out_used);

int disco_set_record_piece(disco_ctx *ctx, uint64_t records);

#ifdef __cplusplus
}
#endif
#endif
```

Measured before the change: 11.28 billion overlaps/s.

## Fuse level-0 binning histogram into count pass, batch counter zeroing, chain slow probe

The index count kernels now build the first-level radix histogram of the binned partition in shared memory as they write records, so binx_partition skips its first memset and histogram pass. Multiple memsets of counters are replaced by one small zeroing kernel. The slow-list probe is launched right after the main probe without a host readback in between. List-grab chunk sizes are adapted, early-exit guards are added for idle blocks, and the build-kernel prefix scan is vectorised per thread. The cost is extra shared memory and atomics in the count kernels, plus a larger hit buffer reservation.

Result: no change. 11.39 billion overlaps/s, median of 6 (+0.9%).

```diff
diff --git a/disco_amd/buildgraph.py b/disco_amd/buildgraph.py
--- a/disco_amd/buildgraph.py
+++ b/disco_amd/buildgraph.py
@@ -184,6 +184,7 @@
     ("disco_fetch_order", C.c_int, [_P, _P, _P, C.c_uint64, C.POINTER(C.c_uint64), C.POINTER(C.c_int)]),
     ("disco_fetch_survivor_layout", C.c_int, [_P, _P, C.c_uint64, C.POINTER(C.c_uint64), C.POINTER(C.c_int), C.POINTER(C.c_uint64)]),
     ("disco_set_record_piece", C.c_int, [_P, C.c_uint64]),
+    ("disco_last_pass_waits", C.c_int, [_P, C.POINTER(C.c_uint32)]),
 ]
 _inspect_bound = False
 
@@ -588,6 +589,12 @@
             self._chk(self.L.disco_fetch_survivor_layout(self._h, lens.ctypes.data, len(lens), C.byref(n), C.byref(dense), C.byref(used)))
             lens = lens[:n.value]
         return lens, bool(dense.value), used.value
+
+    def last_pass_waits(self) -> int:
+        _bind_inspect(self.L)
+        w = C.c_uint32(0)
+        self._chk(self.L.disco_last_pass_waits(self._h, C.byref(w)))
+        return w.value
 
     def measure_hbm(self, nbytes: int = 4 << 30, reps: int = 5) -> float:
         out = C.c_double(0.0)
diff --git a/disco_amd/csrc/disco_hip.hip b/disco_amd/csrc/disco_hip.hip
--- a/disco_amd/csrc/disco_hip.hip
+++ b/disco_amd/csrc/disco_hip.hip
@@ -185,12 +185,15 @@
     bool binned_index = false;
     DevBuf<ulonglong2> d_rec2;
     DevBuf<u32> d_binx;
+    DevBuf<u32> d_hist0;
+    u32 *hist0_rec = nullptr, *hist0_item = nullptr;
 
     DevBuf<u64> d_tile;
     u64 *d_total = nullptr;
 
     u64 *d_ctr = nullptr;
     u64 *d_wq = nullptr;
+    u32 last_pass_waits = ~0u;
     u64 h_ctr[CTR_COUNT] = {0};
 
     DevBuf<u64> d_best;
@@ -624,6 +627,14 @@
     return DISCO_OK;
 }
 
+#define CTR_BIT(i) (1ull << (i))
+static int zero_words(disco_ctx *c, u64 ctr_mask, u64 *w64 = nullptr, u32 *w32a = nullptr, u32 *w32b = nullptr)
+{
+    hipLaunchKernelGGL(zero_words_kernel, dim3(1), dim3(64), 0, c->stream, c->d_ctr, ctr_mask, w64, w32a, w32b);
+    HIPCHK(c, hipGetLastError());
+    return DISCO_OK;
+}
+
 template <typename InT, typename OutT>
 static int scan_exclusive_on(disco_ctx *c, hipStream_t st, DevBuf<u64> &tile, u64 *total, const InT *in, u64 n, OutT *out, bool write_total, u64 *total_host)
 {
@@ -679,6 +690,8 @@
     release(c, c->d_rec);
     release(c, c->d_rec2);
     release(c, c->d_binx);
+    release(c, c->d_hist0);
+    c->hist0_rec = c->hist0_item = nullptr;
     release(c, c->d_best);
     release(c, c->d_hits);
     release(c, c->d_row_start);
@@ -819,6 +832,7 @@
     u32 oidbits = 0;
     u32 oshift = 0;
     const u64 *list = nullptr;
+    BinxCount0 c0;
 };
 
 static bool runs_nf_built(int nf, int m) { return (nf == 7 || nf == 12 || nf == 17 || nf == 22 || nf == 27) && m == RUNS_M; }
@@ -888,6 +902,7 @@
     return true;
 }
 
+static int binx_count0_begin(disco_ctx *c, IndexCountPlan *pl);
 static int index_count_plan(disco_ctx *c, const DiscoView &v, u64 lo, u64 hi, IndexCountPlan *pl, const u64 *list = nullptr)
 {
     const u64 nloc = hi - lo;
@@ -930,11 +945,12 @@
         pl->lpr = lpr;
         pl->nf = nf;
     }
-    return DISCO_OK;
-}
-
-typedef void (*IndexRunsFn)(DiscoView, u32 *, ulonglong2 *, u32 *, u64, u64, u32 *, u32 *, u32 *, u64 *, u32, u32, const u64 *);
-typedef void (*IndexCountFn)(DiscoView, u32 *, ulonglong2 *, u32 *, u64, u64, u32 *, u32 *, u64 *, u32, u32, const u64 *);
+    if (!list) CHK(binx_count0_begin(c, pl));
+    return DISCO_OK;
+}
+
+typedef void (*IndexRunsFn)(DiscoView, u32 *, ulonglong2 *, u32 *, u64, u64, u32 *, u32 *, u32 *, u64 *, u32, u32, const u64 *, BinxCount0);
+typedef void (*IndexCountFn)(DiscoView, u32 *, ulonglong2 *, u32 *, u64, u64, u32 *, u32 *, u64 *, u32, u32, const u64 *, BinxCount0);
 struct IndexCountKernel {
     IndexRunsFn runs = nullptr;
     IndexCountFn plain = nullptr;
@@ -985,8 +1001,8 @@
     u64 *oitem = pl.oitem ? pl.oitem + (a - pl.lo) : nullptr;
     u32 *okey = pl.list ? nullptr : c->d_okey.p;
     const IndexCountKernel k = index_count_pick(count, pl.nf, v.m, pl.lpr, c->ks > 64, false);
-    if (k.runs) hipLaunchKernelGGL(k.runs, grid, dim3(256), 0, c->stream, v, c->d_bkt, rec, okey, a, b, c->d_runs + (a - pl.lo) * (u64)pl.lpr, pl.ocnt, oslot, oitem, pl.oidbits, pl.oshift, pl.list);
-    else hipLaunchKernelGGL(k.plain, grid, dim3(256), 0, c->stream, v, c->d_bkt, rec, okey, a, b, pl.ocnt, oslot, oitem, pl.oidbits, pl.oshift, pl.list);
+    if (k.runs) hipLaunchKernelGGL(k.runs, grid, dim3(256), 0, c->stream, v, c->d_bkt, rec, okey, a, b, c->d_runs + (a - pl.lo) * (u64)pl.lpr, pl.ocnt, oslot, oitem, pl.oidbits, pl.oshift, pl.list, pl.c0);
+    else hipLaunchKernelGGL(k.plain, grid, dim3(256), 0, c->stream, v, c->d_bkt, rec, okey, a, b, pl.ocnt, oslot, oitem, pl.oidbits, pl.oshift, pl.list, pl.c0);
     HIPCHK(c, hipGetLastError());
     return DISCO_OK;
 }
@@ -995,7 +1011,7 @@
 {
     const dim3 g((unsigned)((x_hi - x_lo + 255) / 256));
     hipLaunchKernelGGL(index_count_pick(count, 0, v.m, 0, c->ks > 64, true).plain, g, dim3(256), 0, c->stream, v, c->d_bkt, rec, c->d_okey, x_lo, x_hi, pl.ocnt, oslot, (u64 *)nullptr, 0u, pl.oshift,
-                       (const u64 *)nullptr);
+                       (const u64 *)nullptr, BinxCount0());
     HIPCHK(c, hipGetLastError());
     return DISCO_OK;
 }
@@ -1053,8 +1069,35 @@
     return b;
 }
 
+static u64 binx_hist0_len(u32 total, int bits0) { return ((u64)(total + BINX_TILE - 1u) / BINX_TILE + 1) * (1ull << bits0) + 1; }
+
+static int binx_count0_begin(disco_ctx *c, IndexCountPlan *pl)
+{
+    c->hist0_rec = c->hist0_item = nullptr;
+    if (!c->binned_index || c->comm || c->two_class || pl->lo != 0 || pl->hi != c->n || !c->n || getenv("DISCO_NO_COUNTED_LEVEL0")) return DISCO_OK;
+    const int logT = 64 - c->bshift, obits = 32 - (int)pl->oshift;
+    const BinxPlan br = binx_plan(logT), bo = pl->oitem ? binx_plan(obits) : BinxPlan();
+    const u64 rec_len = br.levels ? binx_hist0_len((u32)(2 * c->n), br.bits[0]) : 0, item_len = bo.levels ? binx_hist0_len((u32)c->n, bo.bits[0]) : 0;
+    if (!rec_len && !item_len) return DISCO_OK;
+    CHK(ensure(c, c->d_hist0, rec_len + item_len));
+    HIPCHK(c, hipMemsetAsync(c->d_hist0, 0, (rec_len + item_len) * sizeof(u32), c->stream));
+    if (rec_len) {
+        pl->c0.rec_hist = c->hist0_rec = c->d_hist0.p;
+        pl->c0.rec_shift = 32u + (u32)(logT - br.bits[0]);
+        pl->c0.rec_nb = 1u << br.bits[0];
+        pl->c0.rec_tiles = (u32)((2 * c->n + BINX_TILE - 1u) / BINX_TILE);
+    }
+    if (item_len) {
+        pl->c0.item_hist = c->hist0_item = c->d_hist0.p + rec_len;
+        pl->c0.item_shift = 64u - (u32)bo.bits[0];
+        pl->c0.item_nb = 1u << bo.bits[0];
+        pl->c0.item_tiles = (u32)((c->n + BINX_TILE - 1u) / BINX_TILE);
+    }
+    return DISCO_OK;
+}
+
 template <typename R>
-static int binx_partition(disco_ctx *c, const char *what, int bits, u32 kshift, u32 total, R *src, R *dst, const R **out, const u32 **part)
+static int binx_partition(disco_ctx *c, const char *what, int bits, u32 kshift, u32 total, R *src, R *dst, const R **out, const u32 **part, u32 *counted0 = nullptr)
 {
     const BinxPlan bp = binx_plan(bits);
     const u32 n_part = 1u << (bits - bp.span);
@@ -1065,27 +1108,32 @@
     CHK(ensure(c, c->d_binx, 4 * tab + hist_len));
     u32 *seg[2] = {c->d_binx.p, c->d_binx.p + tab}, *tb[2] = {c->d_binx.p + 2 * tab, c->d_binx.p + 3 * tab}, *hist = c->d_binx.p + 4 * tab;
     if (getenv("DISCO_VERBOSE"))
-        fprintf(stderr, "[disco] binned %s: 2^%d buckets, %u partitions of 2^%d, %d level(s) of %d / %d / %d bits\n", what, bits, n_part, bp.span, bp.levels, bp.bits[0], bp.bits[1], bp.bits[2]);
+        fprintf(stderr, "[disco] binned %s: 2^%d buckets, %u partitions of 2^%d, %d level(s) of %d / %d / %d bits%s\n", what, bits, n_part, bp.span, bp.levels, bp.bits[0], bp.bits[1], bp.bits[2],
+                counted0 && bp.levels ? ", the first counted by the count pass" : "");
     u32 pseg = 1, pnb = 1;
     int cur = 0, done = 0;
+    const u32 *prev_scan = nullptr;
     for (int l = 0; l < bp.levels; l++) {
         const u32 nseg = 1u << done, nb = 1u << bp.bits[l], shift = kshift + (u32)(bits - done - bp.bits[l]);
         const u32 grid = tiles + nseg;
         const u64 hlen = (u64)grid * nb + 1;
-        hipLaunchKernelGGL(binx_segs_kernel, dim3(1), dim3(1024), 0, c->stream, l ? (const u32 *)hist : (const u32 *)nullptr, (const u32 *)tb[cur ^ 1], pseg, pnb, total, seg[cur], tb[cur]);
-        HIPCHK(c, hipMemsetAsync(hist, 0, hlen * sizeof(u32), c->stream));
-        hipLaunchKernelGGL(binx_hist_kernel<R>, dim3(grid), dim3(BINX_BLOCK), 0, c->stream, (const R *)src, (const u32 *)seg[cur], (const u32 *)tb[cur], nseg, shift, nb, hist);
-        CHK((scan_exclusive<u32, u32>(c, hist, hlen, hist, false, nullptr)));
-        hipLaunchKernelGGL(binx_scatter_kernel<R>, dim3(grid), dim3(BINX_BLOCK), 0, c->stream, (const R *)src, dst, (const u32 *)seg[cur], (const u32 *)tb[cur], nseg, shift, nb, (const u32 *)hist);
+        u32 *const lh = (l == 0 && counted0) ? counted0 : hist;
+        hipLaunchKernelGGL(binx_segs_kernel, dim3(1), dim3(1024), 0, c->stream, prev_scan, (const u32 *)tb[cur ^ 1], pseg, pnb, total, seg[cur], tb[cur]);
+        if (lh == hist) {
+            HIPCHK(c, hipMemsetAsync(hist, 0, hlen * sizeof(u32), c->stream));
+            hipLaunchKernelGGL(binx_hist_kernel<R>, dim3(grid), dim3(BINX_BLOCK), 0, c->stream, (const R *)src, (const u32 *)seg[cur], (const u32 *)tb[cur], nseg, shift, nb, hist);
+        }
+        CHK((scan_exclusive<u32, u32>(c, lh, hlen, lh, false, nullptr)));
+        hipLaunchKernelGGL(binx_scatter_kernel<R>, dim3(grid), dim3(BINX_BLOCK), 0, c->stream, (const R *)src, dst, (const u32 *)seg[cur], (const u32 *)tb[cur], nseg, shift, nb, (const u32 *)lh);
         HIPCHK(c, hipGetLastError());
+        prev_scan = lh;
         std::swap(src, dst);
         pseg = nseg;
         pnb = nb;
         done += bp.bits[l];
         cur ^= 1;
     }
-    hipLaunchKernelGGL(binx_segs_kernel, dim3(1), dim3(1024), 0, c->stream, bp.levels ? (const u32 *)hist : (const u32 *)nullptr, (const u32 *)tb[cur ^ 1], pseg, pnb, total, seg[cur],
-                       (u32 *)nullptr);
+    hipLaunchKernelGGL(binx_segs_kernel, dim3(1), dim3(1024), 0, c->stream, prev_scan, (const u32 *)tb[cur ^ 1], pseg, pnb, total, seg[cur], (u32 *)nullptr);
     HIPCHK(c, hipGetLastError());
     *out = src;
     *part = seg[cur];
@@ -1098,7 +1146,9 @@
     const u32 total = (u32)(2 * c->n);
     const ulonglong2 *rec;
     const u32 *part;
-    CHK(binx_partition(c, "index build", logT, 32u, total, c->d_rec.p, c->d_rec2.p, &rec, &part));
+    u32 *const counted0 = c->hist0_rec;
+    c->hist0_rec = nullptr;
+    CHK(binx_partition(c, "index build", logT, 32u, total, c->d_rec.p, c->d_rec2.p, &rec, &part, counted0));
     const int span = std::min(logT, BINX_SPAN_BITS);
     hipLaunchKernelGGL(binx_build_kernel<ulonglong2>, dim3(1u << (logT - span)), dim3(BINX_BUILD_BLOCK), 0, c->stream, rec, part, (u32)span, 32u, 0u, total, c->T, c->d_bkt.p, c->d_ent.p);
     HIPCHK(c, hipGetLastError());
@@ -1112,7 +1162,9 @@
     u64 *items = (u64 *)c->d_rec2.p;
     const u64 *rec;
     const u32 *part;
-    CHK(binx_partition(c, "grouping", bits, kshift, total, items, items + c->n, &rec, &part));
+    u32 *const counted0 = c->hist0_item;
+    c->hist0_item = nullptr;
+    CHK(binx_partition(c, "grouping", bits, kshift, total, items, items + c->n, &rec, &part, counted0));
     const int span = std::min(bits, BINX_SPAN_BITS);
     hipLaunchKernelGGL(binx_build_kernel<u64>, dim3(1u << (bits - span)), dim3(BINX_BUILD_BLOCK), 0, c->stream, rec, part, (u32)span, kshift, (u32)c->order_id_bits, total, (u64)0,
                        (u32 *)nullptr, c->d_order_own.p);
@@ -2762,7 +2814,7 @@
         else hipLaunchKernelGGL(k.plain, dim3(g), dim3(64), 0, c->stream, a);
     };
     const u64 chunk_slots = use_runs ? PR_CHUNK : PROBE_CHUNK;
-    u64 want_hits = nq * 64 + (u64)grid * chunk_slots + (1u << 16);
+    u64 want_hits = nq * 64 + (u64)grid * chunk_slots + (1u << 16) + 256u * (u64)PROBE_CHUNK;
     u32 want_slow = use_runs ? (u32)std::min<u64>(nq, nq / 64 + 1024 + (c->two_class ? c->n_long : 0)) : 1u;
     u32 want_big = (u32)std::min<u64>(nq, nq / 64 + 1024);
     for (int attempt = 0; attempt < 8; attempt++) {
@@ -2779,13 +2831,8 @@
         }
         if (want_slow > c->d_slow_list.cap) CHK(ensure(c, c->d_slow_list, want_slow));
         CHK(grow_big_lists(c, want_big));
-        HIPCHK(c, hipMemsetAsync(c->d_bump, 0, sizeof(u64), c->stream));
-        HIPCHK(c, hipMemsetAsync(c->d_n_big, 0, sizeof(u32), c->stream));
-        HIPCHK(c, hipMemsetAsync(c->d_n_slow, 0, sizeof(u32), c->stream));
-        HIPCHK(c, hipMemsetAsync(c->d_ctr + CTR_KMER_HITS, 0, sizeof(u64) * 4, c->stream));
-        CHK(zero_counter(c, CTR_MAX_ROW));
-        CHK(zero_counter(c, CTR_ES_BIG));
-        CHK(zero_counter(c, CTR_ES_MID));
+        CHK(zero_words(c, CTR_BIT(CTR_KMER_HITS) | CTR_BIT(CTR_RAW_HITS) | CTR_BIT(CTR_HITS_NEEDED) | CTR_BIT(CTR_OVERFLOW) | CTR_BIT(CTR_MAX_ROW) | CTR_BIT(CTR_ES_BIG) | CTR_BIT(CTR_ES_MID),
+                       c->d_bump, c->d_n_big, c->d_n_slow));
         c->es_big_counted = c->tr_big_counted = false;
         ProbeArgs a;
         a.v = view(c);
@@ -2844,11 +2891,17 @@
         c->order_q_lo = c->q_lo;
         c->order_q_hi = c->q_hi;
         ph_begin(c, DISCO_PH_PROBE_KERNEL);
-        HIPCHK(c, hipMemsetAsync(c->d_wq, 0, sizeof(u64) * WQ_WORDS, c->stream));
         const bool partitioned = c->dist_active && c->part_index;
+        if (attempt || partitioned) HIPCHK(c, hipMemsetAsync(c->d_wq, 0, sizeof(u64) * WQ_WORDS, c->stream));
         if (partitioned) CHK(dist_partitioned_probe(c));
         else if (nq) {
             launch_probe(a, range_kernel, grid);
+        }
+        const bool chain_slow = use_runs && !partitioned && nq && !c->comm;
+        if (chain_slow) {
+            const int g2 = wave_grid(c, (c->d_slow_list.cap + LIST_GRAB_MIN - 1) / LIST_GRAB_MIN, 24);
+            HIPCHK(c, hipMemsetAsync(c->d_wq, 0, sizeof(u64) * WQ_WORDS, c->stream));
+            launch_probe(a, probe_pick(c, 2, false), g2);
         }
         ph_end(c, DISCO_PH_PROBE_KERNEL);
         HIPCHK(c, hipGetLastError());
@@ -2859,8 +2912,8 @@
         }
         CHK(read_counters(c));
         if (partitioned) c->h_ctr[CTR_HITS_NEEDED] = c->hits_used;
-        if (!c->h_ctr[CTR_OVERFLOW] && n_slow) {
-            int g2 = wave_grid(c, (n_slow + WQ_CHUNK - 1) / WQ_CHUNK, 24);
+        if (!chain_slow && !c->h_ctr[CTR_OVERFLOW] && n_slow) {
+            int g2 = wave_grid(c, (n_slow + LIST_GRAB_MIN - 1) / LIST_GRAB_MIN, 24);
             HIPCHK(c, hipMemsetAsync(c->d_wq, 0, sizeof(u64) * WQ_WORDS, c->stream));
             launch_probe(a, probe_pick(c, 2, false), g2);
             HIPCHK(c, hipGetLastError());
@@ -2869,13 +2922,14 @@
         }
         if (!partitioned) c->slow_rows = n_slow;
         if (!c->h_ctr[CTR_OVERFLOW] && n_big) {
-            int g2 = wave_grid(c, (n_big + WQ_CHUNK - 1) / WQ_CHUNK, 8);
+            int g2 = wave_grid(c, (n_big + LIST_GRAB_MIN - 1) / LIST_GRAB_MIN, 8);
             HIPCHK(c, hipMemsetAsync(c->d_wq, 0, sizeof(u64) * WQ_WORDS, c->stream));
             launch_probe(a, probe_pick(c, 1, false), g2);
             HIPCHK(c, hipGetLastError());
             CHK(read_counters(c));
         }
         if (!c->h_ctr[CTR_OVERFLOW]) {
+            if (getenv("DISCO_VERBOSE")) fprintf(stderr, "[disco] probe: %u reads on the slow list, %u rows on the big-row list, of %llu reads\n", n_slow, n_big, (unsigned long long)nq);
             c->big_rows = n_big;
             c->hits_used = c->h_ctr[CTR_HITS_NEEDED];
             VerifyArgs va;
@@ -2982,14 +3036,8 @@
     const u64 nq = c->q_hi - c->q_lo;
     CHK(ensure(c, c->d_adj_ref, c->n));
     HIPCHK(c, hipMemsetAsync(c->d_adj_ref, 0, std::max<u64>(c->n, 1) * sizeof(u64), c->stream));
-    HIPCHK(c, hipMemsetAsync(c->d_n_big, 0, sizeof(u32), c->stream));
-    CHK(zero_counter(c, CTR_CAP_SITES));
-    CHK(zero_counter(c, CTR_DROPPED));
-    CHK(zero_counter(c, CTR_ES_SLOW));
-    CHK(zero_counter(c, CTR_ADJ_TOTAL));
-    CHK(zero_counter(c, CTR_OVERFLOW));
-    CHK(zero_counter(c, CTR_TR_BIG));
-    CHK(zero_counter(c, CTR_TR_MID));
+    CHK(zero_words(c, CTR_BIT(CTR_CAP_SITES) | CTR_BIT(CTR_DROPPED) | CTR_BIT(CTR_ES_SLOW) | CTR_BIT(CTR_ADJ_TOTAL) | CTR_BIT(CTR_OVERFLOW) | CTR_BIT(CTR_TR_BIG) | CTR_BIT(CTR_TR_MID) |
+                       CTR_BIT(CTR_DROP_ITEMS), nullptr, c->d_n_big));
     const bool rows_counted = c->es_big_counted && !getenv("DISCO_COUNT_BIG_ROWS");
     const bool select_small = rows_counted && env_int("DISCO_SELECT_SMALL", c->h_ctr[CTR_ES_MID] * 100 <= nq ? 1 : 0) != 0;
     if (rows_counted) {
@@ -3009,7 +3057,6 @@
     a.hidden_flags = c->prm.max_substitutions != 0;
     a.drop_node = a.drop_key = nullptr;
     a.drop_cap = 0;
-    CHK(zero_counter(c, CTR_DROP_ITEMS));
     if (c->prm.max_substitutions == 0 && !getenv("DISCO_NO_DROP_LIST")) {
         CHK(ensure(c, c->d_drop_node, DROP_LIST_CAP));
         CHK(ensure(c, c->d_drop_key, DROP_LIST_CAP));
@@ -3035,21 +3082,28 @@
     if (nq) wq_launch(c, edge_select_pick(false, flat_select, select_small), nq, "DISCO_SELECT_WAVES", 32, a);
     ph_end(c, DISCO_PH_SELECT);
     HIPCHK(c, hipGetLastError());
+    const bool es_big_rows = !select_small || c->h_ctr[CTR_ES_BIG];
+    auto launch_mid = [&](u64 rows) -> int {
+        if (select_small) {
+            HIPCHK(c, hipMemsetAsync(c->d_wq, 0, sizeof(u64) * WQ_WORDS, c->stream));
+            hipLaunchKernelGGL(edge_select_mid_kernel<ES_CAP>, dim3((int)std::min<u64>(rows, (u64)c->n_cu * 32)), dim3(64), 0, c->stream, a, 0u);
+        }
+        if (es_big_rows) {
+            HIPCHK(c, hipMemsetAsync(c->d_wq, 0, sizeof(u64) * WQ_WORDS, c->stream));
+            hipLaunchKernelGGL(edge_select_mid_kernel<ES_MID>, dim3((int)std::min<u64>(rows, (u64)c->n_cu * 8)), dim3(64), 0, c->stream, a, select_small ? (u32)ES_CAP : 0u);
+        }
+        HIPCHK(c, hipGetLastError());
+        return DISCO_OK;
+    };
+    const bool chain_mid = nq && !c->comm;
+    if (chain_mid) CHK(launch_mid(std::max<u64>(a.big_cap, 1)));
     u32 n_big = 0;
     HIPCHK(c, hipMemcpyAsync(&n_big, c->d_n_big, sizeof(u32), hipMemcpyDeviceToHost, c->stream));
     CHK(read_counters(c));
     ph_collect(c);
     if (c->h_ctr[CTR_OVERFLOW]) return fail(c, DISCO_E_CAPACITY, "edge selection: big-row list overflow (%u rows)", n_big);
-    if (n_big) {
-        if (select_small) {
-            HIPCHK(c, hipMemsetAsync(c->d_wq, 0, sizeof(u64) * WQ_WORDS, c->stream));
-            hipLaunchKernelGGL(edge_select_mid_kernel<ES_CAP>, dim3((int)std::min<u64>(n_big, (u64)c->n_cu * 32)), dim3(64), 0, c->stream, a, 0u);
-        }
-        if (!select_small || c->h_ctr[CTR_ES_BIG]) {
-            HIPCHK(c, hipMemsetAsync(c->d_wq, 0, sizeof(u64) * WQ_WORDS, c->stream));
-            hipLaunchKernelGGL(edge_select_mid_kernel<ES_MID>, dim3((int)std::min<u64>(n_big, (u64)c->n_cu * 8)), dim3(64), 0, c->stream, a, select_small ? (u32)ES_CAP : 0u);
-        }
-        HIPCHK(c, hipGetLastError());
+    if (n_big && !chain_mid) {
+        CHK(launch_mid(n_big));
         CHK(read_counters(c));
     }
     if (n_big && c->h_ctr[CTR_MAX_ROW] > ES_MID) {
@@ -3366,8 +3420,7 @@
     if (c->phase < 6) return fail(c, DISCO_E_STATE, "disco_transitive_mark: build edges first");
     HIPCHK(c, hipSetDevice(c->device));
     const u64 nq = c->q_hi - c->q_lo;
-    HIPCHK(c, hipMemsetAsync(c->d_n_big, 0, sizeof(u32), c->stream));
-    CHK(zero_counter(c, CTR_OVERFLOW));
+    CHK(zero_words(c, CTR_BIT(CTR_OVERFLOW), nullptr, c->d_n_big));
     const bool counted_nodes = c->tr_big_counted && c->q_lo == 0 && c->q_hi == c->n && !getenv("DISCO_COUNT_BIG_ROWS");
     const bool tr_small = env_int("DISCO_TR_SMALL", counted_nodes && c->h_ctr[CTR_TR_MID] * 100 <= nq ? 1 : 0) != 0 && counted_nodes;
     if (counted_nodes) {
@@ -3485,6 +3538,7 @@
             hipLaunchKernelGGL(emit_push_recv_kernel, dim3(grid_push), dim3(64), 0, c->stream, pr);
         }
         HIPCHK(c, hipGetLastError());
+        if (dense) ph_end(c, DISCO_PH_EMIT);
         u64 used = 0;
         HIPCHK(c, hipMemcpyAsync(&used, c->d_bump, sizeof(u64), hipMemcpyDeviceToHost, c->stream));
         HIPCHK(c, hipStreamSynchronize(c->stream));
@@ -3515,8 +3569,10 @@
         CHK((scan_exclusive<u8, u64>(c, c->d_out_valid, c->out_used, c->d_out_pos, true, nullptr)));
         HIPCHK(c, hipMemcpyAsync(&total, c->d_total, sizeof(u64), hipMemcpyDeviceToHost, c->stream));
     }
-    ph_end(c, DISCO_PH_EMIT);
-    HIPCHK(c, hipStreamSynchronize(c->stream));
+    if (!c->out_dense) {
+        ph_end(c, DISCO_PH_EMIT);
+        HIPCHK(c, hipStreamSynchronize(c->stream));
+    }
     ph_collect(c);
     c->n_out = total;
     if (n_out) *n_out = total;
@@ -3537,6 +3593,13 @@
     auto now = [] { return std::chrono::steady_clock::now(); };
     auto ms = [](std::chrono::steady_clock::time_point a, std::chrono::steady_clock::time_point b) { return std::chrono::duration<double, std::milli>(b - a).count(); };
     auto t0 = now();
+    if (!c) return DISCO_E_ARG;
+    const u32 waits0 = tl_pass.host_syncs;
+    struct WaitsOut {
+        disco_ctx *c;
+        u32 w0;
+        ~WaitsOut() { c->last_pass_waits = tl_pass.host_syncs - w0; }
+    } waits_out{c, waits0};
     CHK(disco_build_index(c));
     auto t1 = now();
     CHK(disco_probe(c));
@@ -5906,6 +5969,13 @@
         list_len[v] = REF_DEG(ref[v]) ? (uint8_t)surv_len(half[4 * v], half[4 * v + 1], half[4 * v + 2], half[4 * v + 3]) : 0xFFu;
     return DISCO_OK;
 }
+int disco_last_pass_waits(disco_ctx *c, uint32_t *waits)
+{
+    if (!c || !waits) return DISCO_E_ARG;
+    if (c->last_pass_waits == ~0u) return fail(c, DISCO_E_STATE, "disco_last_pass_waits: no disco_run_graph yet");
+    *waits = c->last_pass_waits;
+    return DISCO_OK;
+}
 int disco_comm_rank(const disco_ctx *c) { return (c && c->comm) ? c->comm->rank : 0; }
 int disco_comm_world(const disco_ctx *c) { return (c && c->comm) ? c->comm->world : 1; }
 const char *disco_comm_kind(const disco_ctx *c) { return (c && c->comm) ? c->comm->kind() : "none"; }
diff --git a/disco_amd/csrc/disco_kernels.h b/disco_amd/csrc/disco_kernels.h
--- a/disco_amd/csrc/disco_kernels.h
+++ b/disco_amd/csrc/disco_kernels.h
@@ -88,6 +88,23 @@
     return b < n;
 }
 
+#define LIST_GRAB_MIN 4u
+__device__ __forceinline__ u32 wq_list_chunk(u64 n)
+{
+    u32 g = LIST_GRAB_MIN;
+    while (g < (u32)WQ_CHUNK && (u64)g * g * 256u < n) g <<= 1;
+    return g;
+}
+__device__ __forceinline__ bool wq_grab_n(u64 *counter, u64 n, u32 chunk, u64 &beg, u64 &end)
+{
+    u64 b = 0;
+    if ((threadIdx.x & 63) == 0) b = atomicAdd(counter, (u64)chunk);
+    b = uniform_u64(b);
+    beg = b;
+    end = (b + chunk < n) ? b + chunk : n;
+    return b < n;
+}
+
 template <u32 CHUNK = WQ_CHUNK, u32 MULT = 4>
 __device__ __forceinline__ bool wq_grab_multi(u64 *counter, u64 n, u64 &beg, u64 &end, u64 &gnext, u64 &gend)
 {
@@ -226,11 +243,56 @@
     }
 }
 
+#define BINX_COUNT0_BITS 8
+#define BINX_COUNT0_TILE 2048u
+#define BINX_COUNT0_WORDS (4u << BINX_COUNT0_BITS)
+struct BinxCount0 {
+    u32 *rec_hist = nullptr, *item_hist = nullptr;
+    u32 rec_shift = 0, rec_nb = 1, rec_tiles = 0;
+    u32 item_shift = 0, item_nb = 1, item_tiles = 0;
+};
+__device__ __forceinline__ void binx_count0_clear(u32 *s_h)
+{
+    for (u32 x = threadIdx.x; x < BINX_COUNT0_WORDS; x += blockDim.x) s_h[x] = 0;
+}
+__device__ __forceinline__ void binx_count0_add(const BinxCount0 &c0, u32 *s_h, u64 first, u64 i, u64 key_p, u64 key_s, u64 item)
+{
+    if (c0.rec_hist) {
+        u32 *h = s_h + (u32)((2 * i) / BINX_COUNT0_TILE - (2 * first) / BINX_COUNT0_TILE) * c0.rec_nb;
+        atomicAdd(&h[(u32)(key_p >> c0.rec_shift) & (c0.rec_nb - 1u)], 1u);
+        atomicAdd(&h[(u32)(key_s >> c0.rec_shift) & (c0.rec_nb - 1u)], 1u);
+    }
+    if (c0.item_hist) {
+        u32 *h = s_h + (2u << BINX_COUNT0_BITS) + (u32)(i / BINX_COUNT0_TILE - first / BINX_COUNT0_TILE) * c0.item_nb;
+        atomicAdd(&h[(u32)(item >> c0.item_shift) & (c0.item_nb - 1u)], 1u);
+    }
+}
+__device__ __forceinline__ void binx_count0_flush(const BinxCount0 &c0, const u32 *s_h, u64 first)
+{
+    for (u32 x = threadIdx.x; x < BINX_COUNT0_WORDS; x += blockDim.x) {
+        const u32 cnt = s_h[x];
+        if (!cnt) continue;
+        const bool it = x >= (2u << BINX_COUNT0_BITS);
+        const u32 y = x & ((2u << BINX_COUNT0_BITS) - 1u), nb = it ? c0.item_nb : c0.rec_nb, tiles = it ? c0.item_tiles : c0.rec_tiles;
+        const u32 tile = (u32)((it ? first : 2 * first) / BINX_COUNT0_TILE) + y / nb;
+        atomicAdd(&(it ? c0.item_hist : c0.rec_hist)[(u64)(y % nb) * tiles + tile], cnt);
+    }
+}
+
 template <bool COUNT, bool LONGK = false, bool LONGCLASS = false>
 __global__ void __launch_bounds__(256) index_count_kernel(DiscoView v, u32 *__restrict__ bkt, ulonglong2 *__restrict__ rec, u32 *__restrict__ okey, u64 lo, u64 hi,
                                                           u32 *__restrict__ ocnt, u32 *__restrict__ oslot, u64 *__restrict__ oitem, u32 oidbits, u32 oshift,
-                                                          const u64 *__restrict__ list = nullptr)
-{
+                                                          const u64 *__restrict__ list = nullptr, BinxCount0 c0 = BinxCount0())
+{
+    constexpr bool COUNT0 = !COUNT && !LONGCLASS;
+    __shared__ u32 s_h0[COUNT0 ? BINX_COUNT0_WORDS : 1u];
+    const bool counted0 = COUNT0 && (c0.rec_hist || c0.item_hist);
+    const u64 first = lo + (u64)blockIdx.x * 256u;
+    if (counted0) {
+        binx_count0_clear(s_h0);
+        __syncthreads();
+    }
+    auto one_read = [&]() {
     const u64 x = lo + (u64)blockIdx.x * 256u + threadIdx.x;
     if (x >= hi) return;
     const u64 i = LONGCLASS ? (u64)v.long_ids[x] : x;
@@ -304,6 +366,13 @@
     const u32 ss = COUNT ? atomicAdd(&bkt[bs], 1u) : 0u;
     rec[2 * (i - lo)] = make_ulonglong2((bp << 32) | sp, PAY_MAKE(kp, rid, tp, rp, 0, L));
     rec[2 * (i - lo) + 1] = make_ulonglong2((bs << 32) | ss, PAY_MAKE(ks, LONGCLASS ? v.n + x : rid, ts, rs, 1, L));
+    if (counted0) binx_count0_add(c0, s_h0, first, i, bp << 32, bs << 32, ORDER_ITEM(best, oshift, rid, L, oidbits));
+    };
+    one_read();
+    if (counted0) {
+        __syncthreads();
+        binx_count0_flush(c0, s_h0, first);
+    }
 }
 
 #define RUNS_M 23
@@ -357,14 +426,17 @@
 __global__ void __launch_bounds__(256) index_runs_kernel(DiscoView v, u32 *__restrict__ bkt, ulonglong2 *__restrict__ rec, u32 *__restrict__ okey, u64 lo, u64 hi,
                                                          u32 *__restrict__ runs, u32 *__restrict__ ocnt, u32 *__restrict__ oslot, u64 *__restrict__ oitem, u32 oidbits,
                                                          u32 oshift,
-                                                         const u64 *__restrict__ list = nullptr)
+                                                         const u64 *__restrict__ list = nullptr, BinxCount0 c0 = BinxCount0())
 {
     static_assert(NF == 0 || NF == NFMAX, "a specialised instantiation holds exactly its window");
     constexpr int CAP = 32 * NL;
     __shared__ u16 s_runs[256 * CAP];
     __shared__ u32 s_x[3 * 256];
+    __shared__ u32 s_h0[COUNT ? 1u : BINX_COUNT0_WORDS];
+    const bool counted0 = !COUNT && (c0.rec_hist || c0.item_hist);
     const u32 tid = threadIdx.x;
     for (u32 x = tid; x < 256u * CAP / 2u; x += 256u) ((u32 *)s_runs)[x] = 0xFFFFFFFFu;
+    if (counted0) binx_count0_clear(s_h0);
     __syncthreads();
     const u64 i = lo + (u64)blockIdx.x * 256u + tid;
     const u64 lw = (list && i < hi) ? list[i] : 0ull;
@@ -472,8 +544,10 @@
         const u32 ss = COUNT ? atomicAdd(&bkt[bs], 1u) : 0u;
         rec[2 * (i - lo)] = make_ulonglong2((bp << 32) | sp, PAY_MAKE(kp, rid, tp, rp, 0, L));
         rec[2 * (i - lo) + 1] = make_ulonglong2((bs << 32) | ss, PAY_MAKE(ks, rid, ts, rs, 1, L));
+        if (counted0) binx_count0_add(c0, s_h0, lo + (u64)blockIdx.x * 256u, i, bp << 32, bs << 32, ORDER_ITEM(best, oshift, rid, L, oidbits));
     }
     __syncthreads();
+    if (counted0) binx_count0_flush(c0, s_h0, lo + (u64)blockIdx.x * 256u);
 #if defined(INDEX_EXP_NORUNS)
     if (tid != 9999u) return;
 #endif
@@ -508,6 +582,7 @@
 #define BINX_TILE 2048u
 #define BINX_BLOCK 256u
 #define BINX_BUILD_BLOCK 1024u
+static_assert(BINX_COUNT0_BITS == BINX_MAX_BITS && BINX_COUNT0_TILE == BINX_TILE, "the count pass counts the first level's digits per tile of the level");
 
 __device__ __forceinline__ u32 binx_block_scan1024(u32 x, u32 *s_w, u32 *total)
 {
@@ -647,12 +722,54 @@
 
 __device__ __forceinline__ u64 binx_payload(const ulonglong2 &r, u32, u32) { return r.y; }
 __device__ __forceinline__ u64 binx_payload(u64 r, u32 kshift, u32 idbits) { return ORDER_MAKE(r & ((1ull << idbits) - 1ull), (r << (64u - kshift)) >> (64u - kshift + idbits)); }
+template <u32 PER, bool TABLE>
+__device__ __forceinline__ void binx_starts(u32 *s_c, u32 *s_w, u32 beg, u32 *__restrict__ bkt_part)
+{
+    const u32 tid = threadIdx.x;
+    u32 v[PER];
+    if constexpr (PER >= 4u) {
+#pragma unroll
+        for (u32 q = 0; q < PER / 4u; q++) {
+            const uint4 x = reinterpret_cast<const uint4 *>(s_c)[tid * (PER / 4u) + q];
+            v[4 * q] = x.x, v[4 * q + 1] = x.y, v[4 * q + 2] = x.z, v[4 * q + 3] = x.w;
+        }
+    } else {
+#pragma unroll
+        for (u32 j = 0; j < PER; j++) v[j] = s_c[tid * PER + j];
+    }
+    u32 mine = 0;
+#pragma unroll
+    for (u32 j = 0; j < PER; j++) {
+        const u32 t = v[j];
+        v[j] = mine;
+        mine += t;
+    }
+    u32 sum;
+    const u32 ex = beg + binx_block_scan1024(mine, s_w, &sum);
+#pragma unroll
+    for (u32 j = 0; j < PER; j++) v[j] += ex;
+    if constexpr (PER >= 4u) {
+#pragma unroll
+        for (u32 q = 0; q < PER / 4u; q++) {
+            const uint4 x = make_uint4(v[4 * q], v[4 * q + 1], v[4 * q + 2], v[4 * q + 3]);
+            reinterpret_cast<uint4 *>(s_c)[tid * (PER / 4u) + q] = x;
+            if (TABLE) reinterpret_cast<uint4 *>(bkt_part)[tid * (PER / 4u) + q] = x;
+        }
+    } else {
+#pragma unroll
+        for (u32 j = 0; j < PER; j++) {
+            s_c[tid * PER + j] = v[j];
+            if (TABLE) bkt_part[tid * PER + j] = v[j];
+        }
+    }
+}
 template <typename R>
 __global__ void __launch_bounds__(BINX_BUILD_BLOCK) binx_build_kernel(const R *__restrict__ rec, const u32 *__restrict__ part, u32 span, u32 kshift, u32 idbits, u32 total, u64 T,
                                                                       u32 *__restrict__ bkt, u64 *__restrict__ ent)
 {
     constexpr bool TABLE = sizeof(R) == sizeof(ulonglong2);
-    __shared__ u32 s_c[1u << BINX_SPAN_BITS];
+    static_assert(BINX_SPAN_BITS == 14 && BINX_BUILD_BLOCK == 1024u, "binx_starts is instantiated for 1, 2, 4, 8 and 16 counters per thread");
+    __shared__ __align__(16) u32 s_c[1u << BINX_SPAN_BITS];
     __shared__ u32 s_w[16];
     const u32 tid = threadIdx.x, p = blockIdx.x;
     const u32 nbk = 1u << span, mask = nbk - 1u;
@@ -661,14 +778,13 @@
     __syncthreads();
     for (u32 i = beg + tid; i < end; i += BINX_BUILD_BLOCK) atomicAdd(&s_c[(u32)(binx_key(rec[i]) >> kshift) & mask], 1u);
     __syncthreads();
-    u32 carry = beg;
-    for (u32 base = 0; base < nbk; base += BINX_BUILD_BLOCK) {
-        const u32 x = s_c[base + tid];
-        u32 sum;
-        const u32 ex = binx_block_scan1024(x, s_w, &sum);
-        s_c[base + tid] = carry + ex;
-        if (TABLE) bkt[(u64)p * nbk + base + tid] = carry + ex;
-        carry += sum;
+    u32 *const bp = TABLE ? bkt + (u64)p * nbk : nullptr;
+    switch (span) {
+    case 10: binx_starts<1, TABLE>(s_c, s_w, beg, bp); break;
+    case 11: binx_starts<2, TABLE>(s_c, s_w, beg, bp); break;
+    case 12: binx_starts<4, TABLE>(s_c, s_w, beg, bp); break;
+    case 13: binx_starts<8, TABLE>(s_c, s_w, beg, bp); break;
+    default: binx_starts<16, TABLE>(s_c, s_w, beg, bp); break;
     }
     if (TABLE && (u64)(p + 1u) * nbk == T && tid == 0) bkt[T] = total;
     __syncthreads();
@@ -814,7 +930,9 @@
     u64 cbeg = 0, cend = 0;
     u64 ord_chunk = 0;
     auto rid = [&](u64 it) { return readlane_u64(ord_chunk, (u32)(it - cbeg)); };
-    while (wq_grab(a.v.wq, n_items, cbeg, cend)) {
+    const u32 grab = LISTED ? wq_list_chunk(n_items) : (u32)WQ_CHUNK;
+    if (LISTED && (u64)blockIdx.x * grab >= n_items) return;
+    while (LISTED ? wq_grab_n(a.v.wq, n_items, grab, cbeg, cend) : wq_grab(a.v.wq, n_items, cbeg, cend)) {
     if (!LISTED) {
         const u64 i = min(cbeg + lane, cend - 1);
         ord_chunk = a.order ? a.order[i] : ORDER_MAKE(a.v.q_lo + i, a.v.len[a.v.q_lo + i]);
@@ -3361,6 +3479,7 @@
     const u64 n_items = (u64)min(*a.n_big, a.big_cap);
     u64 cbeg = 0, cend = 0;
     u64 gnext = 0, gend = 0;
+    if ((u64)blockIdx.x * 8u >= n_items) return;
     while (wq_grab_multi<1, 8>(a.v.wq, n_items, cbeg, cend, gnext, gend)) {
         const u64 A = a.big_list[cbeg];
         const u32 c = a.row_cnt[A];
@@ -4540,4 +4659,14 @@
     for (; i < n; i += (u64)gridDim.x * blockDim.x) p[i] = val;
 }
 
-#endif
+__global__ void __launch_bounds__(64) zero_words_kernel(u64 *__restrict__ ctr, u64 mask, u64 *__restrict__ w64, u32 *__restrict__ w32a, u32 *__restrict__ w32b)
+{
+    static_assert(CTR_COUNT <= 61, "a lane per counter, three lanes for the single words");
+    const u32 lane = threadIdx.x;
+    if ((mask >> lane) & 1ull) ctr[lane] = 0;
+    if (lane == 61 && w64) *w64 = 0;
+    if (lane == 62 && w32a) *w32a = 0;
+    if (lane == 63 && w32b) *w32b = 0;
+}
+
+#endif
diff --git a/include/disco_hip_inspect.h b/include/disco_hip_inspect.h
--- a/include/disco_hip_inspect.h
+++ b/include/disco_hip_inspect.h
@@ -13,6 +13,8 @@
 
 int disco_set_record_piece(disco_ctx *ctx, uint64_t records);
 
+int disco_last_pass_waits(disco_ctx *ctx, uint32_t *waits);
+
 #ifdef __cplusplus
 }
 #endif
```
